# ashiq24/UNO

Hardware: AMD Instinct MI355X
Metric: UNO training samples/s (421^2 Darcy) (higher is better)
Workload: dtype f32; 1 GPU; Darcy 2D 421x421, UNO_9(3,64,pad=5) 64ch, batch 16/GPU, train step (fwd+loss+bwd+allreduce+Adam); global_batch=16, parallelism=dp1

## Files before the change

### include/uno_spectral.h

```cpp
#ifndef UNO_SPECTRAL_H
#define UNO_SPECTRAL_H

#ifdef __cplusplus
extern "C" {
#endif

#define UNO_SPECTRAL_ABI_VERSION 14

int uno_abi_version(void);
void* uno_upload_table(const void* host, long long bytes);

const char* uno_last_error(void);

long long uno_spectral_conv2d_fwd_ws_bytes(int B, int Ci, int Co, int m1, int m2);
long long uno_spectral_conv2d_bwd_ws_bytes(int B, int Ci, int Co, int m1, int m2);

int uno_spectral_conv2d_forward(const float* x, const float* w1, const float* w2, float* y,
                                float* xtrunc, void* ws, int B, int Ci, int Co, int H, int W,
                                int Ho, int Wo, int m1, int m2, void* stream);

int uno_spectral_conv2d_backward(const float* gy, const float* xtrunc, const float* w1,
                                 const float* w2, float* gx, float* gw1, float* gw2, void* ws,
                                 int B, int Ci, int Co, int H, int W, int Ho, int Wo, int m1,
                                 int m2, void* stream);

int uno_spectral_conv2d_forward_bf16(const void* x, const float* w1, const float* w2, void* y,
                                     float* xtrunc, void* ws, int B, int Ci, int Co, int H, int W,
                                     int Ho, int Wo, int m1, int m2, void* stream);
int uno_spectral_conv2d_backward_bf16(const void* gy, const float* xtrunc, const float* w1,
                                      const float* w2, void* gx, float* gw1, float* gw2, void* ws,
                                      int B, int Ci, int Co, int H, int W, int Ho, int Wo, int m1,
                                      int m2, void* stream);

long long uno_fft_resample3d_ws_bytes(int n_vol, int D1, int M1, int J1, int J2, int m3);
int uno_fft_resample3d(const float* x, float* y, void* ws, int n_vol, int D1, int D2, int D3, int M1, int M2, int M3,
                       int J1, const int* f1_in, const int* f1_out, int J2, const int* f2_in, const int* f2_out, int m3,
                       float scale, int herm_in, int herm_out, void* stream);

int uno_fft_resample3d_acc(const float* x, float* y, float* y_act, void* ws, int n_vol, int D1, int D2, int D3, int M1, int M2, int M3,
                           int J1, const int* f1_in, const int* f1_out, int J2, const int* f2_in, const int* f2_out, int m3,
                           float scale, int herm_in, int herm_out, void* stream);

long long uno_fft_resample3d_any_ws_bytes(int n_vol, int D1, int M1, int J1, int J2, int m3);
int uno_fft_resample3d_any(const float* x, float* y, void* ws, int n_vol, int D1, int D2, int D3, int M1, int M2, int M3,
                           int J1, const int* f1_in, const int* f1_out, int J2, const int* f2_in, const int* f2_out, int m3,
                           float scale, int herm_in, int herm_out, void* stream);

int uno_fft_resample3d_any_acc(const float* x, float* y, float* y_act, void* ws, int n_vol, int D1, int D2, int D3, int M1, int M2, int M3,
                               int J1, const int* f1_in, const int* f1_out, int J2, const int* f2_in, const int* f2_out, int m3,
                               float scale, int herm_in, int herm_out, void* stream);

long long uno_spectral_conv3d_fwd_ws_bytes(int B, int Ci, int Co, int H, int Ho, int m1, int m2, int m3);
long long uno_spectral_conv3d_bwd_ws_bytes(int B, int Ci, int Co, int H, int Ho, int m1, int m2, int m3);
int uno_spectral_conv3d_forward(const float* x, const float* const* w, float* y, float* xtrunc, void* ws,
                                int B, int Ci, int Co, int H, int W, int T, int Ho, int Wo, int To,
                                int m1, int m2, int m3, void* stream);
int uno_spectral_conv3d_backward(const float* gy, const float* xtrunc, const float* const* w, float* gx,
                                 float* const* gw, void* ws, int B, int Ci, int Co, int H, int W, int T,
                                 int Ho, int Wo, int To, int m1, int m2, int m3, void* stream);

int uno_cdft_axis(const float* in, float* out, int inverse, int n_img, int H, int m1, int m2, int m3,
                  float scale, int mask_overlap, void* stream);


int uno_dft2d_forward(const float* images, float* spec, int n_img, int H, int W, int m1, int m2,
                      float scale, int hermitian_cols, int mask_overlap, void* stream);

int uno_dft2d_inverse(const float* spec, float* images, int n_img, int H, int W, int m1, int m2,
                      float scale, int hermitian_cols, int mask_overlap, void* stream);

int uno_reserve_cus(int n);

int uno_sweep_alternation(int enable);

int uno_dft2d_inverse_add_applies(int n_img, int H, int W, int m1, int m2, int Hs, int Ws);
int uno_dft2d_inverse_add(const float* spec, float* images, int n_img, int H, int W, int m1, int m2, float scale, int hermitian_cols,
                          int mask_overlap, const float* addend, int Hs, int Ws, const int* tile_p0, const float* row_op,
                          const int* col_v0, const float* col_op, void* stream);

int uno_dft2d_forward_bf16(const void* images, float* spec, int n_img, int H, int W, int m1, int m2,
                           float scale, int hermitian_cols, int mask_overlap, void* stream);
int uno_dft2d_inverse_bf16(const float* spec, void* images, int n_img, int H, int W, int m1, int m2,
                           float scale, int hermitian_cols, int mask_overlap, void* stream);

int uno_dft2d_forward_grouped(const float* images, float* spec, int n_img, int H, int W, int m1, int m2, float scale,
                              int hermitian_cols, int mask_overlap, int group, int stride, int offset, void* stream);
int uno_dft2d_inverse_grouped(const float* spec, float* images, int n_img, int H, int W, int m1, int m2, float scale,
                              int hermitian_cols, int mask_overlap, int group, int stride, int offset, void* stream);

int uno_mode_mix(const float* in, const float* const* w, float* out, int op, int B, int Ci, int Co,
                 int ncorner, int modes_per_corner, void* stream);

int uno_mode_wgrad(const float* xtrunc, const float* go, float* const* gw, int B, int Ci, int Co,
                   int ncorner, int modes_per_corner, void* stream);
int uno_mode_backward(const float* xtrunc, const float* go, const float* const* w, float* gx_spec, float* const* gw, int B, int Ci,
                      int Co, int ncorner, int modes_per_corner, int accumulate, void* stream);
int uno_mode_wgrad_acc(const float* xtrunc, const float* go, float* const* gw, int B, int Ci, int Co, int ncorner,
                       int modes_per_corner, int accumulate, void* stream);
int uno_spectral_conv2d_backward_acc(const void* gy, const float* xtrunc, const void* w1, const void* w2, void* gx,
                                     float* gw1, float* gw2, void* ws, int B, int Ci, int Co, int H, int W, int Ho, int Wo,
                                     int m1, int m2, int io_format, int accumulate_gw, void* stream);

int uno_resample2d(const float* in, float* out, float* tmp, int n_img, int H, int W, int Ho, int Wo,
                   const int* startH, const float* wtH, int KH, const int* startW, const float* wtW, int KW,
                   const int* tile_p0, const float* tile_w, int NP, int accumulate, void* stream);

int uno_channel_mix(const float* x, const float* w, const float* bias, float* y, int B, int Ci, int Co,
                    long long P, int transpose_w, int accumulate, int act_in, const float* dgelu_of, void* stream);

long long uno_channel_wgrad_ws_bytes(int B, int Ci, int Co, long long P);
int uno_channel_wgrad(const float* gy, const float* x, float* gw, float* gb, void* ws, int B, int Ci, int Co,
                      long long P, int act_x, void* stream);

int uno_channel_mix2(const float* x1, const float* x2, int C1, const float* w, const float* bias, float* y1, float* y2, int Co1,
                     float* y_act, int B, int Ci, int Co, long long P, int transpose_w, int accumulate, int act_in,
                     const float* dgelu_of, const float* proj_w, const float* proj_b, float* proj_out, void* stream);
int uno_channel_wgrad2(const float* gy, const float* x1, const float* x2, int C1, float* gw, float* gb, void* ws, int B, int Ci,
                       int Co, long long P, int act_x, int accumulate, void* stream);
int uno_channel_wgrad_finish(const void* parts, float* gw, float* gb, int Ci, int Co, long long nparts, int accumulate, void* stream);

int uno_gelu_project_forward(const float* pre, const float* w, const float* bias, float* out, int B, int C, long long P,
                             void* stream);
long long uno_gelu_project_bwd_ws_bytes(int B, int C, long long P);
int uno_gelu_project_backward(const float* pre, const float* w, const float* gout, float* gpre, float* gw, float* gb,
                              void* ws, int B, int C, long long P, void* stream);

int uno_gelu_project2_forward(const float* pre, const float* s, const float* w, const float* bias, float* out, int B, int C1, int C2,
                              long long P, int act2, void* stream);
long long uno_gelu_project2_bwd_ws_bytes(int B, int C1, int C2, long long P);
int uno_gelu_project2_backward(const float* pre, const float* s, const float* w, const float* gout, float* gpre, float* gs, float* gw,
                               float* gb, void* ws, int B, int C1, int C2, long long P, int act2, void* stream);

long long uno_rel_l2_steps_ws_bytes(int B, long long P, int T);
int uno_rel_l2_steps(const float* pred, const float* target, float* sums, float* rel, float* totals, void* ws, int B, long long P, int T,
                     void* stream);

long long uno_rollout_ws_bytes(int B, long long P, int T);
int uno_rollout_advance(float* window, const float* frame, const float* target, float* pred, void* ws, int B, int C, int T_in, long long P,
                        int T, int t, int shift, void* stream);
int uno_rollout_finish(const void* ws, float* sums, float* rel, float* totals, int B, long long P, int T, void* stream);

int uno_rollout_lift(const float* given, const float* pred, const float* feat, const float* w, const float* bias, float* h, int B, int T_in,
                     int F, int Cm, long long P, int T, int t, void* stream);
long long uno_rollout_lift_bwd_ws_bytes(int B, int T_in, int F, int Cm, long long P, int T);
int uno_rollout_lift_backward(const float* gh, const float* given, const float* pred, const float* target, const float* feat, const float* w,
                              const float* sums, const float* gL, float* gpred, float* gframe, void* parts, int B, int T_in, int F, int Cm,
                              long long P, int T, int t, void* stream);
int uno_rollout_loss_seed(const float* pred, const float* target, const float* sums, const float* gL, float* gframe, int B, long long P, int T,
                          void* stream);

int uno_channel_mix2_win(const float* x1, const float* x2, int C1, const float* w, const float* bias, float* y1, float* y2, int Co1,
                         float* y_act, int B, int Ci, int Co, int rows, int cols, int pitch, long long plane, int transpose_w,
                         int accumulate, int act_in, const float* dgelu_of, const float* proj_w, const float* proj_b, float* proj_out,
                         void* stream);
int uno_channel_wgrad2_win(const float* gy, const float* x1, const float* x2, int C1, float* gw, float* gb, void* ws, int B, int Ci,
                           int Co, int rows, int cols, int pitch, long long plane, int act_x, int accumulate, void* stream);
int uno_gelu_project_backward_win(const float* pre, const float* w, const float* gout, float* gpre, float* gw, float* gb, void* ws,
                                  int B, int C, int rows, int cols, int pitch, long long plane, void* stream);
int uno_project_backward_applies(int B, int C1, int Ci, int Co, int rows, int cols, int pitch, long long plane);
long long uno_project_backward_ws_bytes(int B, int Ci, int Co, long long P);
int uno_project_backward(const float* x1, const float* x2, int C1, const float* w, const float* pre, const float* w2, const float* gout,
                         float* g1, float* g2, float* gw, float* gb, float* gw2, float* gb2, void* ws, int B, int Ci, int Co, int rows,
                         int cols, int pitch, long long plane, int act_in, int accumulate_w, void* stream);
int uno_clear_border(float* t, long long n_planes, int Hp, int Wp, int rows, int cols, void* stream);
int uno_channel_mix_act_padded(const float* x, const float* w, const float* bias, float* y, float* y_act, int B, int Ci, int Co, int H,
                               int W, int Hp, int Wp, int act_in, void* stream);
int uno_channel_mix_dgelu_padded(const float* x, const float* w, const float* bias, const float* g_padded, float* gz, int B, int Ci,
                                 int Co, int H, int W, int Hp, int Wp, int act_in, void* stream);
int uno_lift_forward(const float* x, const float* w1, const float* b1, const float* w0, const float* b0, float* act, int B, int Cin,
                     int Cm, int Co, int H, int W, int Hp, int Wp, void* stream);
long long uno_lift_bwd_ws_bytes(int B, int Cin, int Cm, int Co, int H, int W);
int uno_lift_backward(const float* x, const float* w1, const float* b1, const float* w0, const float* b0, const float* g_act, float* gw1,
                      float* gb1, float* gw0, float* gb0, void* ws, int B, int Cin, int Cm, int Co, int H, int W, int Hp, int Wp,
                      void* stream);
int uno_lift_backward_takes_second(int B, int Cin, int Cm, int Co, int H, int W, int Hp, int Wp);
int uno_lift_backward2(const float* x, const float* w1, const float* b1, const float* w0, const float* b0, const float* g_act,
                       const float* g_act2, float* gw1, float* gb1, float* gw0, float* gb0, void* ws, int B, int Cin, int Cm, int Co,
                       int H, int W, int Hp, int Wp, void* stream);

int uno_gelu_pad(const float* s, const float* gy, float* out, int n_img, int H, int W, int Hp, int Wp, int backward,
                 void* stream);

int uno_instnorm_forward(const float* x, const float* gamma, const float* beta, float* y, float* mean, float* rstd, long long rows,
                         int C, long long N, float eps, int gelu, void* stream);
int uno_instnorm_backward(const float* x, const float* gy, const float* gamma, const float* beta, const float* mean,
                          const float* rstd, float* gx, float* s1, float* s2, long long rows, int C, long long N, int gelu,
                          void* stream);

int uno_adam_step(float* p, const float* g, float* m, float* v, long long n, int is_complex, double lr, double beta1,
                  double beta2, double eps, double weight_decay, int step, void* stream);

int uno_adam_step_multi(int n_tensors, float* const* p, const float* const* g, float* const* m, float* const* v,
                        const long long* n, const int* is_complex, double lr, double beta1, double beta2, double eps,
                        double weight_decay, int step, void* stream);

int uno_adam_step_multi_dev(int n_tensors, float* const* p, const float* const* g, float* const* m, float* const* v,
                            const long long* n, const int* is_complex, double lr, double beta1, double beta2, double eps,
                            double weight_decay, int* step_counter, float* scalars, const double* hyper, void* stream);

int uno_spectral_conv2d_forward_mixed(const void* x_bf16, const void* w1_f16, const void* w2_f16, void* y_bf16,
                                      float* xtrunc, void* ws, int B, int Ci, int Co, int H, int W, int Ho, int Wo,
                                      int modes1, int modes2, void* stream);
int uno_spectral_conv2d_backward_mixed(const void* gy_bf16, const float* xtrunc, const void* w1_f16, const void* w2_f16,
                                       void* gx_bf16, float* gw1, float* gw2, void* ws, int B, int Ci, int Co, int H, int W,
                                       int Ho, int Wo, int modes1, int modes2, void* stream);
int uno_mode_mix_f16w(const float* in, const void* const* w_f16, float* out, int op, int B, int Ci, int Co, int ncorner,
                      int modes_per_corner, void* stream);
int uno_dft2d_forward_grouped_bf16(const void* images, float* spec, int n_img, int H, int W, int m1, int m2, float scale,
                                   int hermitian_cols, int mask_overlap, int group, int stride, int offset, void* stream);
int uno_dft2d_inverse_grouped_bf16(const float* spec, void* images, int n_img, int H, int W, int m1, int m2, float scale,
                                   int hermitian_cols, int mask_overlap, int group, int stride, int offset, void* stream);
int uno_resample2d_bf16(const void* in, void* out, float* tmp, int n_img, int H, int W, int Ho, int Wo, const int* startH,
                        const float* wtH, int KH, const int* startW, const float* wtW, int KW, const int* tile_p0,
                        const float* tile_w, int NP, int accumulate, void* stream);
int uno_channel_mix_bf16(const void* x, const float* w, const float* bias, void* y, int B, int Ci, int Co, long long P,
                         int transpose_w, int accumulate, int act_in, const void* dgelu_of, void* stream);
int uno_channel_wgrad_bf16(const void* gy, const void* x, float* gw, float* gb, void* ws, int B, int Ci, int Co, long long P,
                           int act_x, void* stream);
int uno_channel_mix2_bf16(const void* x1, const void* x2, int C1, const float* w, const float* bias, void* y1, void* y2, int Co1,
                          void* y_act, int B, int Ci, int Co, long long P, int transpose_w, int accumulate, int act_in,
                          const void* dgelu_of, const float* proj_w, const float* proj_b, void* proj_out, void* stream);
int uno_channel_wgrad2_bf16(const void* gy, const void* x1, const void* x2, int C1, float* gw, float* gb, void* ws, int B, int Ci,
                            int Co, long long P, int act_x, int accumulate, void* stream);
int uno_gelu_project_forward_bf16(const void* pre, const float* w, const float* bias, void* out, int B, int C, long long P,
                                  void* stream);
int uno_gelu_project_backward_bf16(const void* pre, const float* w, const void* gout, void* gpre, float* gw, float* gb,
                                   void* ws, int B, int C, long long P, void* stream);
int uno_gelu_pad_bf16(const void* s, const void* gy, void* out, int n_img, int H, int W, int Hp, int Wp, int backward,
                      void* stream);
int uno_instnorm_forward_bf16(const void* x, const float* gamma, const float* beta, void* y, float* mean, float* rstd,
                              long long rows, int C, long long N, float eps, int gelu, void* stream);
int uno_instnorm_backward_bf16(const void* x, const void* gy, const float* gamma, const float* beta, const float* mean,
                               const float* rstd, void* gx, float* s1, float* s2, long long rows, int C, long long N,
                               int gelu, void* stream);

long long uno_dft2d_any_ws_bytes(int n_img, int H, int W, int m1, int m2);
int uno_scratch_provide(void* ptr, long long bytes);
long long uno_channel_mix_ws_bytes(int Ci, int Co, long long P, int bf16);

int uno_transpose_batched(const float* in, float* out, int B, long long R, int C, long long ld_in, long long sb_in,
                          long long ld_out, long long sb_out, void* stream);

int uno_profile_begin(int max_records);
int uno_profile_end(void);
int uno_profile_get(int index, char* name, int name_len, double* ms, double* bytes);

#ifdef __cplusplus
}
#endif
#endif
```

### uno_amd/_native.py

```python
from __future__ import annotations

import ctypes as C
import os
import threading

import torch

_HERE = os.path.dirname(os.path.abspath(__file__))
LIB_PATH = os.path.join(_HERE, "lib", "libuno_spectral.so")
ABI_VERSION = 14

_lib = None
_lock = threading.Lock()

_fp = C.c_void_p
_i = C.c_int
_SIGNATURES = {
    "uno_abi_version": (C.c_int, []),
    "uno_last_error": (C.c_char_p, []),
    "uno_dft2d_any_ws_bytes": (C.c_longlong, [_i] * 5),
    "uno_scratch_provide": (C.c_int, [_fp, C.c_longlong]),
    "uno_spectral_conv2d_fwd_ws_bytes": (C.c_longlong, [_i] * 5),
    "uno_spectral_conv2d_bwd_ws_bytes": (C.c_longlong, [_i] * 5),
    "uno_spectral_conv2d_forward": (C.c_int, [_fp] * 6 + [_i] * 9 + [_fp]),
    "uno_spectral_conv2d_backward": (C.c_int, [_fp] * 8 + [_i] * 9 + [_fp]),
    "uno_spectral_conv2d_forward_bf16": (C.c_int, [_fp] * 6 + [_i] * 9 + [_fp]),
    "uno_spectral_conv2d_backward_bf16": (C.c_int, [_fp] * 8 + [_i] * 9 + [_fp]),
    "uno_fft_resample3d_ws_bytes": (C.c_longlong, [_i] * 6),
    "uno_fft_resample3d": (C.c_int, [_fp] * 3 + [_i] * 8 + [_fp, _fp, _i, _fp, _fp, _i, C.c_float, _i, _i, _fp]),
    "uno_fft_resample3d_acc": (C.c_int, [_fp] * 4 + [_i] * 8 + [_fp, _fp, _i, _fp, _fp, _i, C.c_float, _i, _i, _fp]),
    "uno_fft_resample3d_any_ws_bytes": (C.c_longlong, [_i] * 6),
    "uno_fft_resample3d_any": (C.c_int, [_fp] * 3 + [_i] * 8 + [_fp, _fp, _i, _fp, _fp, _i, C.c_float, _i, _i, _fp]),
    "uno_fft_resample3d_any_acc": (C.c_int, [_fp] * 4 + [_i] * 8 + [_fp, _fp, _i, _fp, _fp, _i, C.c_float, _i, _i, _fp]),
    "uno_dft2d_forward": (C.c_int, [_fp, _fp] + [_i] * 5 + [C.c_float, _i, _i, _fp]),
    "uno_dft2d_forward_bf16": (C.c_int, [_fp, _fp] + [_i] * 5 + [C.c_float, _i, _i, _fp]),
    "uno_dft2d_inverse_bf16": (C.c_int, [_fp, _fp] + [_i] * 5 + [C.c_float, _i, _i, _fp]),
    "uno_dft2d_inverse": (C.c_int, [_fp, _fp] + [_i] * 5 + [C.c_float, _i, _i, _fp]),
    "uno_reserve_cus": (C.c_int, [_i]),
    "uno_sweep_alternation": (C.c_int, [_i]),
    "uno_dft2d_inverse_add_applies": (C.c_int, [_i] * 7),
    "uno_dft2d_inverse_add": (C.c_int, [_fp, _fp] + [_i] * 5 + [C.c_float, _i, _i, _fp, _i, _i, _fp, _fp, _fp, _fp, _fp]),
    "uno_dft2d_forward_grouped": (C.c_int, [_fp, _fp] + [_i] * 5 + [C.c_float] + [_i] * 5 + [_fp]),
    "uno_dft2d_inverse_grouped": (C.c_int, [_fp, _fp] + [_i] * 5 + [C.c_float] + [_i] * 5 + [_fp]),
    "uno_mode_mix": (C.c_int, [_fp, C.POINTER(_fp), _fp] + [_i] * 6 + [_fp]),
    "uno_mode_wgrad": (C.c_int, [_fp, _fp, C.POINTER(_fp)] + [_i] * 5 + [_fp]),
    "uno_mode_backward": (C.c_int, [_fp, _fp, C.POINTER(_fp), _fp, C.POINTER(_fp)] + [_i] * 6 + [_fp]),
    "uno_spectral_conv3d_fwd_ws_bytes": (C.c_longlong, [_i] * 8),
    "uno_spectral_conv3d_bwd_ws_bytes": (C.c_longlong, [_i] * 8),
    "uno_spectral_conv3d_forward": (C.c_int, [_fp, C.POINTER(_fp), _fp, _fp, _fp] + [_i] * 12 + [_fp]),
    "uno_spectral_conv3d_backward": (C.c_int, [_fp, _fp, C.POINTER(_fp), _fp, C.POINTER(_fp), _fp] + [_i] * 12 + [_fp]),
    "uno_cdft_axis": (C.c_int, [_fp, _fp] + [_i] * 6 + [C.c_float, _i, _fp]),
    "uno_resample2d": (C.c_int, [_fp, _fp, _fp] + [_i] * 5 + [_fp, _fp, _i, _fp, _fp, _i, _fp, _fp, _i, _i, _fp]),
    "uno_channel_mix": (C.c_int, [_fp, _fp, _fp, _fp, _i, _i, _i, C.c_longlong, _i, _i, _i, _fp, _fp]),
    "uno_channel_wgrad_ws_bytes": (C.c_longlong, [_i, _i, _i, C.c_longlong]),
    "uno_channel_wgrad": (C.c_int, [_fp, _fp, _fp, _fp, _fp, _i, _i, _i, C.c_longlong, _i, _fp]),
    "uno_channel_mix2": (C.c_int, [_fp, _fp, _i, _fp, _fp, _fp, _fp, _i, _fp, _i, _i, _i, C.c_longlong, _i, _i, _i, _fp, _fp, _fp, _fp, _fp]),
    "uno_channel_wgrad2": (C.c_int, [_fp, _fp, _fp, _i, _fp, _fp, _fp, _i, _i, _i, C.c_longlong, _i, _i, _fp]),
    "uno_channel_mix2_win": (C.c_int, [_fp, _fp, _i, _fp, _fp, _fp, _fp, _i, _fp, _i, _i, _i, _i, _i, _i, C.c_longlong, _i, _i, _i, _fp, _fp, _fp, _fp, _fp]),
    "uno_channel_mix_ws_bytes": (C.c_longlong, [_i, _i, C.c_longlong, _i]),
    "uno_clear_border": (C.c_int, [_fp, C.c_longlong, _i, _i, _i, _i, _fp]),
    "uno_channel_mix_act_padded": (C.c_int, [_fp, _fp, _fp, _fp, _fp, _i, _i, _i, _i, _i, _i, _i, _i, _fp]),
    "uno_lift_forward": (C.c_int, [_fp] * 6 + [_i] * 8 + [_fp]),
    "uno_lift_bwd_ws_bytes": (C.c_longlong, [_i] * 6),
    "uno_lift_backward": (C.c_int, [_fp] * 11 + [_i] * 8 + [_fp]),
    "uno_lift_backward2": (C.c_int, [_fp] * 12 + [_i] * 8 + [_fp]),
    "uno_lift_backward_takes_second": (C.c_int, [_i] * 8),
    "uno_channel_mix_dgelu_padded": (C.c_int, [_fp, _fp, _fp, _fp, _fp, _i, _i, _i, _i, _i, _i, _i, _i, _fp]),
    "uno_channel_wgrad2_win": (C.c_int, [_fp, _fp, _fp, _i, _fp, _fp, _fp, _i, _i, _i, _i, _i, _i, C.c_longlong, _i, _i, _fp]),
    "uno_gelu_project_backward_win": (C.c_int, [_fp] * 7 + [_i, _i, _i, _i, _i, C.c_longlong, _fp]),
    "uno_channel_wgrad_finish": (C.c_int, [_fp, _fp, _fp, _i, _i, C.c_longlong, _i, _fp]),
    "uno_mode_wgrad_acc": (C.c_int, [_fp, _fp, C.POINTER(_fp)] + [_i] * 6 + [_fp]),
    "uno_spectral_conv2d_backward_acc": (C.c_int, [_fp] * 8 + [_i] * 11 + [_fp]),
    "uno_upload_table": (C.c_void_p, [_fp, C.c_longlong]),
    "uno_project_backward_applies": (C.c_int, [_i] * 7 + [C.c_longlong]),
    "uno_project_backward_ws_bytes": (C.c_longlong, [_i, _i, _i, C.c_longlong]),
    "uno_project_backward": (C.c_int, [_fp, _fp, _i] + [_fp] * 11 + [_i] * 6 + [C.c_longlong, _i, _i, _fp]),
    "uno_gelu_project_forward": (C.c_int, [_fp, _fp, _fp, _fp, _i, _i, C.c_longlong, _fp]),
    "uno_gelu_project_bwd_ws_bytes": (C.c_longlong, [_i, _i, C.c_longlong]),
    "uno_gelu_project_backward": (C.c_int, [_fp] * 7 + [_i, _i, C.c_longlong, _fp]),
    "uno_gelu_project2_forward": (C.c_int, [_fp] * 5 + [_i, _i, _i, C.c_longlong, _i, _fp]),
    "uno_gelu_project2_bwd_ws_bytes": (C.c_longlong, [_i, _i, _i, C.c_longlong]),
    "uno_gelu_project2_backward": (C.c_int, [_fp] * 9 + [_i, _i, _i, C.c_longlong, _i, _fp]),
    "uno_rel_l2_steps_ws_bytes": (C.c_longlong, [_i, C.c_longlong, _i]),
    "uno_rel_l2_steps": (C.c_int, [_fp] * 6 + [_i, C.c_longlong, _i, _fp]),
    "uno_rollout_ws_bytes": (C.c_longlong, [_i, C.c_longlong, _i]),
    "uno_rollout_advance": (C.c_int, [_fp] * 5 + [_i, _i, _i, C.c_longlong, _i, _i, _i, _fp]),
    "uno_rollout_finish": (C.c_int, [_fp] * 4 + [_i, C.c_longlong, _i, _fp]),
    "uno_rollout_lift": (C.c_int, [_fp] * 6 + [_i, _i, _i, _i, C.c_longlong, _i, _i, _fp]),
    "uno_rollout_lift_bwd_ws_bytes": (C.c_longlong, [_i, _i, _i, _i, C.c_longlong, _i]),
    "uno_rollout_lift_backward": (C.c_int, [_fp] * 11 + [_i, _i, _i, _i, C.c_longlong, _i, _i, _fp]),
    "uno_rollout_loss_seed": (C.c_int, [_fp] * 5 + [_i, C.c_longlong, _i, _fp]),
    "uno_gelu_pad": (C.c_int, [_fp, _fp, _fp] + [_i] * 6 + [_fp]),
    "uno_transpose_batched": (C.c_int, [_fp, _fp, _i, C.c_longlong, _i] + [C.c_longlong] * 4 + [_fp]),
    "uno_instnorm_forward": (C.c_int, [_fp] * 6 + [C.c_longlong, _i, C.c_longlong, C.c_float, _i, _fp]),
    "uno_instnorm_backward": (C.c_int, [_fp] * 9 + [C.c_longlong, _i, C.c_longlong, _i, _fp]),
    "uno_adam_step": (C.c_int, [_fp, _fp, _fp, _fp, C.c_longlong, _i] + [C.c_double] * 5 + [_i, _fp]),
    "uno_adam_step_multi": (C.c_int, [_i, C.POINTER(_fp), C.POINTER(_fp), C.POINTER(_fp), C.POINTER(_fp), C.POINTER(C.c_longlong),
                                      C.POINTER(_i)] + [C.c_double] * 5 + [_i, _fp]),
    "uno_adam_step_multi_dev": (C.c_int, [_i, C.POINTER(_fp), C.POINTER(_fp), C.POINTER(_fp), C.POINTER(_fp), C.POINTER(C.c_longlong),
                                          C.POINTER(_i)] + [C.c_double] * 5 + [_fp, _fp, _fp, _fp]),
    "uno_spectral_conv2d_forward_mixed": (C.c_int, [_fp] * 6 + [_i] * 9 + [_fp]),
    "uno_spectral_conv2d_backward_mixed": (C.c_int, [_fp] * 8 + [_i] * 9 + [_fp]),
    "uno_mode_mix_f16w": (C.c_int, [_fp, C.POINTER(_fp), _fp] + [_i] * 6 + [_fp]),
    "uno_dft2d_forward_grouped_bf16": (C.c_int, [_fp, _fp] + [_i] * 5 + [C.c_float] + [_i] * 5 + [_fp]),
    "uno_dft2d_inverse_grouped_bf16": (C.c_int, [_fp, _fp] + [_i] * 5 + [C.c_float] + [_i] * 5 + [_fp]),
    "uno_resample2d_bf16": (C.c_int, [_fp, _fp, _fp] + [_i] * 5 + [_fp, _fp, _i, _fp, _fp, _i, _fp, _fp, _i, _i, _fp]),
    "uno_channel_mix_bf16": (C.c_int, [_fp, _fp, _fp, _fp, _i, _i, _i, C.c_longlong, _i, _i, _i, _fp, _fp]),
    "uno_channel_wgrad_bf16": (C.c_int, [_fp, _fp, _fp, _fp, _fp, _i, _i, _i, C.c_longlong, _i, _fp]),
    "uno_channel_mix2_bf16": (C.c_int, [_fp, _fp, _i, _fp, _fp, _fp, _fp, _i, _fp, _i, _i, _i, C.c_longlong, _i, _i, _i, _fp, _fp, _fp, _fp, _fp]),
    "uno_channel_wgrad2_bf16": (C.c_int, [_fp, _fp, _fp, _i, _fp, _fp, _fp, _i, _i, _i, C.c_longlong, _i, _i, _fp]),
    "uno_gelu_project_forward_bf16": (C.c_int, [_fp, _fp, _fp, _fp, _i, _i, C.c_longlong, _fp]),
    "uno_gelu_project_backward_bf16": (C.c_int, [_fp] * 7 + [_i, _i, C.c_longlong, _fp]),
    "uno_gelu_pad_bf16": (C.c_int, [_fp, _fp, _fp] + [_i] * 6 + [_fp]),
    "uno_instnorm_forward_bf16": (C.c_int, [_fp] * 6 + [C.c_longlong, _i, C.c_longlong, C.c_float, _i, _fp]),
    "uno_instnorm_backward_bf16": (C.c_int, [_fp] * 9 + [C.c_longlong, _i, C.c_longlong, _i, _fp]),
    "uno_profile_begin": (C.c_int, [_i]),
    "uno_profile_end": (C.c_int, []),
    "uno_profile_get": (C.c_int, [_i, C.c_char_p, _i, C.POINTER(C.c_double), C.POINTER(C.c_double)]),
}
EXPORTED_SYMBOLS = tuple(_SIGNATURES)


def lib():
    global _lib
    if _lib is None:
        with _lock:
            if _lib is None:
                if not os.path.exists(LIB_PATH):
                    raise RuntimeError(
                        f"uno_amd: native library {LIB_PATH} is missing - build it with "
                        "`python -m uno_amd.build` (hipcc, gfx950); there is no CPU fallback")
                h = C.CDLL(LIB_PATH)
                for name, (res, args) in _SIGNATURES.items():
                    fn = getattr(h, name)
                    fn.restype = res
                    fn.argtypes = args
                if h.uno_abi_version() != ABI_VERSION:
                    raise RuntimeError(f"uno_amd: ABI mismatch, library {h.uno_abi_version()} != binding {ABI_VERSION}")
                _lib = h
    return _lib


def _check(rc: int, what: str):
    if rc != 0:
        msg = lib().uno_last_error().decode(errors="replace")
        raise RuntimeError(f"{what} failed (code {rc}): {msg}")


def _ptr(t: torch.Tensor):
    return C.c_void_p(t.data_ptr())


def _opt(t):
    return _ptr(t) if t is not None else C.c_void_p(0)


def _count(lead) -> int:
    n = 1
    for d in lead:
        n *= d
    return n


def _stream(t: torch.Tensor):
    return C.c_void_p(torch.cuda.current_stream(t.device).cuda_stream)


class _scratch:

    def __init__(self, device, nbytes):
        self.bytes, self.device, self.buf = nbytes, device, None

    def __enter__(self):
        if self.bytes > 0:
            self.buf = torch.empty(self.bytes, dtype=torch.uint8, device=self.device)
            _check(lib().uno_scratch_provide(_ptr(self.buf), self.bytes), "uno_scratch_provide")
        return self

    def __exit__(self, *exc):
        if self.bytes > 0:
            lib().uno_scratch_provide(None, 0)
        return False


class _any_mode_scratch(_scratch):

    def __init__(self, device, *needs):
        L = lib()
        _scratch.__init__(self, device, max((int(L.uno_dft2d_any_ws_bytes(*[int(v) for v in n])) for n in needs), default=0))


class _mix_scratch(_scratch):

    def __init__(self, device, Ci, Co, P, bf16):
        _scratch.__init__(self, device, int(lib().uno_channel_mix_ws_bytes(int(Ci), int(Co), int(P), 1 if bf16 else 0)))


def _require(t: torch.Tensor, dtype, name: str, dense: bool = True):
    if not t.is_cuda:
        raise RuntimeError(f"uno_amd: {name} must live on a HIP device (got {t.device})"
                           + ("; the spectral convolution runs only on the MI355X kernels" if dense else ""))
    if t.dtype != dtype:
        raise RuntimeError(f"uno_amd: {name} must be {dtype} (got {t.dtype})")
    if dense and not t.is_contiguous():
        raise RuntimeError(f"uno_amd: {name} must be contiguous")


def _entry(name: str, bf16: bool):
    return getattr(lib(), name + "_bf16" if bf16 else name)


def _act_dtype(t, name):
    bf16 = t.dtype == torch.bfloat16
    _require(t, torch.bfloat16 if bf16 else torch.float32, name)
    return bf16


def _weights_half(w1, w2, bf16):
    if w1.dtype == torch.float16:
        if not bf16:
            raise RuntimeError("uno_amd: half-precision weight storage goes with bfloat16 activations")
        for w, name in ((w1, "weights1"), (w2, "weights2")):
            _require(w, torch.float16, name)
            if w.dim() != 5 or w.shape[-1] != 2:
                raise RuntimeError("uno_amd: half-precision weights are stored as (Ci, Co, m1, m2, 2) = (re, im)")
        return True
    _require(w1, torch.complex64, "weights1")
    _require(w2, torch.complex64, "weights2")
    return False


def _complex_grad_buffers(out, shape, n: int, device, accumulate: bool):
    if out is None:
        return [torch.empty(shape, dtype=torch.complex64, device=device) for _ in range(n)], False
    gws = list(out)
    for t in gws:
        _require(t, torch.complex64, "weight-gradient buffer")
        if tuple(t.shape) != tuple(shape):
            raise RuntimeError("uno_amd: weight-gradient buffer has the wrong shape")
    return gws, accumulate


def _real_grad_buffers(out_w, out_b, Ci: int, Co: int, need_bias: bool, device, accumulate: bool):
    if out_w is None:
        gw = torch.empty((Co, Ci), dtype=torch.float32, device=device)
        return gw, (torch.empty((Co,), dtype=torch.float32, device=device) if need_bias else None), False
    gw, gb = out_w, (out_b if need_bias else None)
    _require(gw, torch.float32, "weight-gradient buffer")
    if gw.numel() != Co * Ci or (need_bias and (gb is None or gb.numel() != Co)):
        raise RuntimeError("uno_amd: gradient buffers do not match the layer")
    if gb is not None:
        _require(gb, torch.float32, "bias-gradient buffer")
    return gw, gb, accumulate


def spectral_conv2d_forward(x, w1, w2, Ho: int, Wo: int, xt_out=None):
    bf16 = _act_dtype(x, "x")
    wh = _weights_half(w1, w2, bf16)
    B, Ci, H, W = x.shape
    Ci2, Co, m1, m2 = w1.shape[:4]
    if Ci2 != Ci or tuple(w2.shape) != tuple(w1.shape):
        raise RuntimeError(f"uno_amd: weight shapes {tuple(w1.shape)} / {tuple(w2.shape)} do not match input channels {Ci}")
    L = lib()
    with torch.cuda.device(x.device):
        y = torch.empty((B, Co, Ho, Wo), dtype=x.dtype, device=x.device)
        if xt_out is None:
            xt = torch.empty((B, Ci, 2 * m1, m2), dtype=torch.complex64, device=x.device)
        else:
            xt = xt_out
            _require(xt, torch.complex64, "xtrunc buffer")
            if tuple(xt.shape) != (B, Ci, 2 * m1, m2):
                raise RuntimeError("uno_amd: xtrunc buffer has the wrong shape")
        ws = torch.empty(max(1, L.uno_spectral_conv2d_fwd_ws_bytes(B, Ci, Co, m1, m2)), dtype=torch.uint8, device=x.device)
        fn = L.uno_spectral_conv2d_forward_mixed if wh else _entry("uno_spectral_conv2d_forward", bf16)
        with _any_mode_scratch(x.device, (B * Ci, H, W, m1, m2), (B * Co, Ho, Wo, m1, m2)):
            rc = fn(_ptr(x), _ptr(w1), _ptr(w2), _ptr(y), _ptr(xt), _ptr(ws), B, Ci, Co, H, W, Ho, Wo, m1, m2, _stream(x))
    _check(rc, "uno_spectral_conv2d_forward")
    return y, xt


def spectral_conv2d_backward(gy, xt, w1, w2, H: int, W: int, need_gx=True, need_gw=True, gw_out=None, accumulate_gw=False):
    bf16 = _act_dtype(gy, "grad_output")
    _require(xt, torch.complex64, "xtrunc")
    wh = _weights_half(w1, w2, bf16)
    B, Co, Ho, Wo = gy.shape
    Ci, Co2, m1, m2 = w1.shape[:4]
    if Co2 != Co:
        raise RuntimeError("uno_amd: grad_output channels do not match the weights")
    L = lib()
    with torch.cuda.device(gy.device):
        gx = torch.empty((B, Ci, H, W), dtype=gy.dtype, device=gy.device) if need_gx else None
        gw1, gw2, accumulate_gw = None, None, accumulate_gw and need_gw
        if need_gw:
            (gw1, gw2), accumulate_gw = _complex_grad_buffers(gw_out, (Ci, Co, m1, m2), 2, gy.device, accumulate_gw)
        ws = torch.empty(max(1, L.uno_spectral_conv2d_bwd_ws_bytes(B, Ci, Co, m1, m2)), dtype=torch.uint8, device=gy.device)
        with _any_mode_scratch(gy.device, (B * Co, Ho, Wo, m1, m2), (B * Ci, H, W, m1, m2)):
            rc = L.uno_spectral_conv2d_backward_acc(_ptr(gy), _ptr(xt), _ptr(w1), _ptr(w2), _opt(gx), _opt(gw1), _opt(gw2),
                                                    _ptr(ws), B, Ci, Co, H, W, Ho, Wo, m1, m2, 2 if wh else (1 if bf16 else 0),
                                                    1 if accumulate_gw else 0, _stream(gy))
    _check(rc, "uno_spectral_conv2d_backward")
    return gx, gw1, gw2


def _fft_resample3d(any_grid: bool, x, out_size, f1, f2, m3, scale, adjoint, out, act):
    name = "uno_fft_resample3d_any" if any_grid else "uno_fft_resample3d"
    _require(x, torch.float32, "x")
    *lead, D1, D2, D3 = x.shape
    M1, M2, M3 = (int(v) for v in out_size)
    n = _count(lead)
    for t in (*f1, *f2):
        if t.dtype != torch.int32 or not t.is_cuda or not t.is_contiguous():
            raise RuntimeError("uno_amd: frequency tables must be contiguous int32 device tensors")
    J1, J2 = f1[0].numel(), f2[0].numel()
    if any_grid and (f1[1].numel() != J1 or f2[1].numel() != J2):
        raise RuntimeError("uno_amd: the forward and inverse frequency tables of an axis must have the same length")
    L = lib()
    with torch.cuda.device(x.device):
        ws = torch.empty(max(1, getattr(L, name + "_ws_bytes")(n, D1, M1, J1, J2, int(m3))), dtype=torch.uint8, device=x.device)
        if out is not None:
            _require(out, torch.float32, "out")
            if tuple(out.shape) != (*lead, M1, M2, M3) or not out.is_contiguous():
                raise RuntimeError(f"uno_amd: out must be a contiguous {(*lead, M1, M2, M3)} tensor")
            ya = torch.empty_like(out) if act else None
            fn, dst, res = getattr(L, name + "_acc"), (_ptr(out), _opt(ya)), ((out, ya) if act else out)
        else:
            res = torch.empty((*lead, M1, M2, M3), dtype=torch.float32, device=x.device)
            fn, dst = getattr(L, name), (_ptr(res),)
        rc = fn(_ptr(x), *dst, _ptr(ws), n, D1, D2, D3, M1, M2, M3, J1, _ptr(f1[0]), _ptr(f1[1]), J2, _ptr(f2[0]), _ptr(f2[1]),
                int(m3), float(scale), int(adjoint), int(not adjoint), _stream(x))
    _check(rc, name + ("_acc" if out is not None else ""))
    return res


def fft_resample3d(x, out_size, f1, f2, m3: int, scale: float, adjoint: bool, out=None, act=False):
    return _fft_resample3d(False, x, out_size, f1, f2, m3, scale, adjoint, out, act)


def fft_resample3d_any(x, out_size, f1, f2, m3: int, scale: float, adjoint: bool, out=None, act=False):
    return _fft_resample3d(True, x, out_size, f1, f2, m3, scale, adjoint, out, act)


def dft2d_forward(images, m1, m2, scale=1.0, hermitian_cols=False, mask_overlap=False, out=None, channel_offset=0):
    bf16 = _act_dtype(images, "images")
    *lead, H, W = images.shape
    n = _count(lead)
    if out is None:
        spec = torch.empty((*lead, 2 * m1, m2), dtype=torch.complex64, device=images.device)
        with torch.cuda.device(images.device):
            fn = _entry("uno_dft2d_forward", bf16)
            with _any_mode_scratch(images.device, (n, H, W, m1, m2)):
                rc = fn(_ptr(images), _ptr(spec), n, H, W, m1, m2, float(scale), int(hermitian_cols), int(mask_overlap), _stream(images))
        _check(rc, "uno_dft2d_forward")
        return spec
    _require(out, torch.complex64, "out")
    if images.dim() != 4 or out.dim() != 4 or out.shape[0] != images.shape[0] or tuple(out.shape[2:]) != (2 * m1, m2) \
            or channel_offset < 0 or channel_offset + images.shape[1] > out.shape[1]:
        raise RuntimeError("uno_amd: out must be (B, Ctot, 2*m1, m2) with room for the image channels at channel_offset")
    with torch.cuda.device(images.device):
        fn = _entry("uno_dft2d_forward_grouped", bf16)
        with _any_mode_scratch(images.device, (n, H, W, m1, m2)):
            rc = fn(_ptr(images), _ptr(out), n, H, W, m1, m2, float(scale), int(hermitian_cols),
                    int(mask_overlap), images.shape[1], out.shape[1], int(channel_offset), _stream(images))
    _check(rc, "uno_dft2d_forward_grouped")
    return out


def reserve_cus(n: int) -> int:
    return int(lib().uno_reserve_cus(int(n)))


def sweep_alternation(enable: bool) -> bool:
    return bool(lib().uno_sweep_alternation(1 if enable else 0))


def sweep_direction(mode: str, mask: int = 255) -> int:
    if mode not in ("alternate", "forward", "reversed") or not 0 <= int(mask) <= 255:
        raise ValueError(f"uno_amd: sweep_direction({mode!r}, {mask!r}): mode is alternate | forward | reversed, mask 0 .. 255")
    value = {"alternate": int(mask), "forward": 0, "reversed": 256 | int(mask)}[mode]
    if value == 1:
        raise ValueError("uno_amd: sweep_direction('alternate', 1): the C entry point reads 1 as 'every family' (255)")
    return int(lib().uno_sweep_alternation(value))


def dft2d_inverse_add_applies(n_img, H, W, m1, m2, Hs, Ws) -> bool:
    return bool(lib().uno_dft2d_inverse_add_applies(int(n_img), int(H), int(W), int(m1), int(m2), int(Hs), int(Ws)))


def dft2d_inverse(spec, H, W, scale=1.0, hermitian_cols=True, mask_overlap=True, channels=None, channel_offset=0,
                  dtype=torch.float32, addend=None):
    _require(spec, torch.complex64, "spec")
    *lead, r2, m2 = spec.shape
    m1 = r2 // 2
    if addend is not None:
        t, (p0, rowop, v0, colop) = addend
        _require(t, torch.float32, "addend")
        if channels is not None or dtype != torch.float32 or tuple(t.shape[:-2]) != tuple(lead):
            raise RuntimeError("uno_amd: dft2d_inverse(addend=) takes the plain float32 form with one addend image per spectrum")
        n = _count(lead)
        img = torch.empty((*lead, H, W), dtype=torch.float32, device=spec.device)
        with torch.cuda.device(spec.device):
            rc = lib().uno_dft2d_inverse_add(_ptr(spec), _ptr(img), n, H, W, m1, m2, float(scale), int(hermitian_cols), int(mask_overlap),
                                             _ptr(t), t.shape[-2], t.shape[-1], _ptr(p0), _ptr(rowop), _ptr(v0), _ptr(colop), _stream(spec))
        _check(rc, "uno_dft2d_inverse_add")
        return img
    if channels is None:
        n = _count(lead)
        if dtype not in (torch.float32, torch.bfloat16):
            raise RuntimeError("uno_amd: images are float32 or bfloat16")
        img = torch.empty((*lead, H, W), dtype=dtype, device=spec.device)
        with torch.cuda.device(spec.device):
            fn = _entry("uno_dft2d_inverse", dtype == torch.bfloat16)
            with _any_mode_scratch(spec.device, (n, H, W, m1, m2)):
                rc = fn(_ptr(spec), _ptr(img), n, H, W, m1, m2, float(scale), int(hermitian_cols), int(mask_overlap), _stream(spec))
        _check(rc, "uno_dft2d_inverse")
        return img
    if dtype not in (torch.float32, torch.bfloat16):
        raise RuntimeError("uno_amd: images are float32 or bfloat16")
    if spec.dim() != 4 or channel_offset < 0 or channels < 1 or channel_offset + channels > spec.shape[1]:
        raise RuntimeError("uno_amd: spec must be (B, Ctot, 2*m1, m2) holding the requested channel range")
    B = spec.shape[0]
    img = torch.empty((B, channels, H, W), dtype=dtype, device=spec.device)
    with torch.cuda.device(spec.device):
        fn = _entry("uno_dft2d_inverse_grouped", dtype == torch.bfloat16)
        with _any_mode_scratch(spec.device, (B * channels, H, W, m1, m2)):
            rc = fn(_ptr(spec), _ptr(img), B * channels, H, W, m1, m2, float(scale), int(hermitian_cols),
                    int(mask_overlap), int(channels), spec.shape[1], int(channel_offset), _stream(spec))
    _check(rc, "uno_dft2d_inverse_grouped")
    return img


def _ptr_array(ts):
    return (C.c_void_p * len(ts))(*[t.data_ptr() for t in ts])


def mode_mix(inp, weights, op: int):
    _require(inp, torch.complex64, "spectrum")
    half = weights[0].dtype == torch.float16
    for w in weights:
        _require(w, torch.float16 if half else torch.complex64, "weights")
    B = inp.shape[0]
    Ci, Co = weights[0].shape[:2]
    nc = len(weights)
    Mc = weights[0][0, 0].numel() // (2 if half else 1)
    cout = Co if op == 0 else Ci
    out = torch.empty((B, cout, *inp.shape[2:]), dtype=torch.complex64, device=inp.device)
    with torch.cuda.device(inp.device):
        fn = lib().uno_mode_mix_f16w if half else lib().uno_mode_mix
        rc = fn(_ptr(inp), _ptr_array(weights), _ptr(out), op, B, Ci, Co, nc, Mc, _stream(inp))
    _check(rc, "uno_mode_mix")
    return out


def mode_wgrad(xt, go, weight_shape, ncorner: int, out=None, accumulate: bool = False):
    _require(xt, torch.complex64, "xtrunc")
    _require(go, torch.complex64, "grad spectrum")
    B, Ci = xt.shape[:2]
    Co = go.shape[1]
    gws, accumulate = _complex_grad_buffers(out, weight_shape, ncorner, xt.device, accumulate)
    Mc = gws[0][0, 0].numel()
    with torch.cuda.device(xt.device):
        rc = lib().uno_mode_wgrad_acc(_ptr(xt), _ptr(go), _ptr_array(gws), B, Ci, Co, ncorner, Mc, 1 if accumulate else 0, _stream(xt))
    _check(rc, "uno_mode_wgrad")
    return gws


def mode_backward(xt, go, weights, out=None, accumulate: bool = False):
    _require(xt, torch.complex64, "xtrunc")
    _require(go, torch.complex64, "grad spectrum")
    for w in weights:
        _require(w, torch.complex64, "weights")
    B, Ci = xt.shape[:2]
    Co = go.shape[1]
    nc = len(weights)
    Mc = weights[0][0, 0].numel()
    gws, accumulate = _complex_grad_buffers(out, weights[0].shape, nc, xt.device, accumulate)
    gX = torch.empty((B, Ci, nc * Mc), dtype=torch.complex64, device=xt.device)
    with torch.cuda.device(xt.device):
        rc = lib().uno_mode_backward(_ptr(xt), _ptr(go), _ptr_array(list(weights)), _ptr(gX), _ptr_array(gws), B, Ci, Co, nc, Mc,
                                     1 if accumulate else 0, _stream(xt))
    _check(rc, "uno_mode_backward")
    return gX, gws


def spectral_conv3d_forward(x, ws_, Ho: int, Wo: int, To: int):
    _require(x, torch.float32, "x")
    if len(ws_) != 4:
        raise RuntimeError("uno_amd: the 3-D spectral convolution takes four weight tensors")
    for w in ws_:
        _require(w, torch.complex64, "weights")
        if tuple(w.shape) != tuple(ws_[0].shape):
            raise RuntimeError("uno_amd: weights1..4 must have one shape")
    B, Ci, H, W, T = x.shape
    Ci2, Co, m1, m2, m3 = ws_[0].shape
    if Ci2 != Ci:
        raise RuntimeError(f"uno_amd: weight shape {tuple(ws_[0].shape)} does not match input channels {Ci}")
    L = lib()
    with torch.cuda.device(x.device):
        y = torch.empty((B, Co, Ho, Wo, To), dtype=torch.float32, device=x.device)
        xt = torch.empty((B, Ci, 4, m1, m2, m3), dtype=torch.complex64, device=x.device)
        scratch = torch.empty(max(1, L.uno_spectral_conv3d_fwd_ws_bytes(B, Ci, Co, H, Ho, m1, m2, m3)), dtype=torch.uint8,
                              device=x.device)
        with _any_mode_scratch(x.device, (B * Ci * H, W, T, m2, m3), (B * Co * Ho, Wo, To, m2, m3)):
            rc = L.uno_spectral_conv3d_forward(_ptr(x), _ptr_array(ws_), _ptr(y), _ptr(xt), _ptr(scratch), B, Ci, Co,
                                               H, W, T, Ho, Wo, To, m1, m2, m3, _stream(x))
    _check(rc, "uno_spectral_conv3d_forward")
    return y, xt


def spectral_conv3d_backward(gy, xt, ws_, H: int, W: int, T: int, need_gx=True, need_gw=True):
    _require(gy, torch.float32, "grad_output")
    _require(xt, torch.complex64, "xtrunc")
    for w in ws_:
        _require(w, torch.complex64, "weights")
    B, Co, Ho, Wo, To = gy.shape
    Ci, Co2, m1, m2, m3 = ws_[0].shape
    if Co2 != Co:
        raise RuntimeError("uno_amd: grad_output channels do not match the weights")
    L = lib()
    with torch.cuda.device(gy.device):
        gx = torch.empty((B, Ci, H, W, T), dtype=torch.float32, device=gy.device) if need_gx else None
        gws = [torch.empty_like(w) for w in ws_] if need_gw else None
        scratch = torch.empty(max(1, L.uno_spectral_conv3d_bwd_ws_bytes(B, Ci, Co, H, Ho, m1, m2, m3)), dtype=torch.uint8,
                              device=gy.device)
        with _any_mode_scratch(gy.device, (B * Co * Ho, Wo, To, m2, m3), (B * Ci * H, W, T, m2, m3)):
            rc = L.uno_spectral_conv3d_backward(_ptr(gy), _ptr(xt), _ptr_array(ws_), _opt(gx),
                                                _ptr_array(gws) if need_gw else None, _ptr(scratch), B, Ci, Co,
                                                H, W, T, Ho, Wo, To, m1, m2, m3, _stream(gy))
    _check(rc, "uno_spectral_conv3d_backward")
    return gx, gws


def resample2d(x, Ho: int, Wo: int, tabH, tabW, tilesH=None, out=None):
    bf16 = _act_dtype(x, "x")
    *lead, H, W = x.shape
    n = _count(lead)
    sH, wH = tabH
    sW, wW = tabW
    accumulate = out is not None
    if accumulate:
        _require(out, x.dtype, "out")
        if tuple(out.shape) != (*lead, Ho, Wo):
            raise RuntimeError(f"uno_amd: out has shape {tuple(out.shape)}, expected {(*lead, Ho, Wo)}")
    else:
        out = torch.empty((*lead, Ho, Wo), dtype=x.dtype, device=x.device)
    with torch.cuda.device(x.device):
        tmp = torch.empty(max(1, n * min(Ho * W, H * Wo)), dtype=torch.float32, device=x.device)
        if tilesH is not None:
            tp0, tw = tilesH
            targs = (_ptr(tp0), _ptr(tw), tw.shape[1])
        else:
            targs = (C.c_void_p(0), C.c_void_p(0), 0)
        fn = _entry("uno_resample2d", bf16)
        rc = fn(_ptr(x), _ptr(out), _ptr(tmp), n, H, W, Ho, Wo, _ptr(sH), _ptr(wH), wH.shape[1],
                _ptr(sW), _ptr(wW), wW.shape[1], *targs, 1 if accumulate else 0, _stream(x))
    _check(rc, "uno_resample2d")
    return out


def _window_fits(rows: int, cols: int, pitch: int, plane: int) -> bool:
    return not (rows < 1 or cols % 4 or cols < 260 or pitch < cols or (rows - 1) * pitch + cols > plane or rows * cols >= 1 << 24)


def _window_args(window, plane: int, bf16: bool):
    rows, cols, pitch = (int(v) for v in window)
    if bf16:
        raise RuntimeError("uno_amd: pixel windows are float32 only")
    if not _window_fits(rows, cols, pitch, plane):
        raise RuntimeError(f"uno_amd: window rows={rows} cols={cols} pitch={pitch} does not fit a plane of {plane} elements "
                           "(cols: a multiple of 4, 260 <= cols <= pitch; rows * cols < 2^24)")
    return rows, cols, pitch


def channel_mix(x, w, bias=None, transpose_w: bool = False, out=None, act_in: bool = False, dgelu_of=None, dgelu_total: bool = False,
                window=None):
    if window is not None:
        return channel_mix2(x, None, w, bias, transpose_w=transpose_w, out=out, act_in=act_in, dgelu_of=dgelu_of,
                            accumulate=(2 if (dgelu_total and dgelu_of is not None) else 1) if out is not None else 0, window=window)
    bf16 = _act_dtype(x, "x")
    _require(w, torch.float32, "weight")
    if bias is not None:
        _require(bias, torch.float32, "bias")
    B, Ci, P = x.shape
    Co = w.shape[1] if transpose_w else w.shape[0]
    if (w.shape[0] if transpose_w else w.shape[1]) != Ci:
        raise RuntimeError(f"uno_amd: weight {tuple(w.shape)} does not match {Ci} input channels")
    accumulate = out is not None
    if accumulate:
        _require(out, x.dtype, "out")
        if tuple(out.shape) != (B, Co, P):
            raise RuntimeError(f"uno_amd: out has shape {tuple(out.shape)}, expected {(B, Co, P)}")
        y = out
    else:
        y = torch.empty((B, Co, P), dtype=x.dtype, device=x.device)
    with torch.cuda.device(x.device), _mix_scratch(x.device, Ci, Co, P, bf16):
        if dgelu_of is not None:
            _require(dgelu_of, x.dtype, "dgelu_of")
            if tuple(dgelu_of.shape) != (B, Co, P):
                raise RuntimeError(f"uno_amd: dgelu_of has shape {tuple(dgelu_of.shape)}, expected {(B, Co, P)}")
        rc = _entry("uno_channel_mix", bf16)(_ptr(x), _ptr(w), _opt(bias), _ptr(y), B, Ci, Co, P, 1 if transpose_w else 0,
                                             (2 if (dgelu_total and dgelu_of is not None) else 1) if accumulate else 0,
                                             1 if act_in else 0, _opt(dgelu_of), _stream(x))
    _check(rc, "uno_channel_mix")
    return y


def clear_border(t, rows: int, cols: int):
    _require(t, torch.float32, "tensor")
    Hp, Wp = t.shape[-2:]
    n = t.numel() // max(1, Hp * Wp)
    with torch.cuda.device(t.device):
        rc = lib().uno_clear_border(_ptr(t), n, Hp, Wp, int(rows), int(cols), _stream(t))
    _check(rc, "uno_clear_border")
    return t


def channel_mix_act_padded_ok(x, Hp: int, Wp: int) -> bool:
    H, W = x.shape[-2:]
    return x.dtype == torch.float32 and 260 <= W <= Wp and H <= Hp and H * W < (1 << 24)


def channel_mix_act_padded(x, w, bias, Hp: int, Wp: int, act_in: bool = False, keep_y: bool = True):
    _require(x, torch.float32, "x")
    _require(w, torch.float32, "weight")
    if bias is not None:
        _require(bias, torch.float32, "bias")
    B, Ci, H, W = x.shape
    Co = w.shape[0]
    if w.shape[1] != Ci:
        raise RuntimeError(f"uno_amd: weight {tuple(w.shape)} does not match {Ci} input channels")
    y = torch.empty((B, Co, H, W), dtype=x.dtype, device=x.device) if keep_y else None
    act = torch.empty((B, Co, Hp, Wp), dtype=x.dtype, device=x.device)
    with torch.cuda.device(x.device):
        rc = lib().uno_channel_mix_act_padded(_ptr(x), _ptr(w), _opt(bias), _opt(y), _ptr(act),
                                              B, Ci, Co, H, W, int(Hp), int(Wp), 1 if act_in else 0, _stream(x))
    _check(rc, "uno_channel_mix_act_padded")
    return y, act


def lift_ok(x, w1, w0, Hp: int, Wp: int) -> bool:
    if x.dim() != 4 or x.dtype != torch.float32:
        return False
    H, W = x.shape[-2:]
    return (1 <= x.shape[1] <= 3 and w1.shape[0] in (16, 32) and w1.shape[1] == x.shape[1] and w0.shape[1] == w1.shape[0]
            and 260 <= W <= Wp and H <= Hp and H * W < (1 << 24))


def lift_forward(x, w1, b1, w0, b0, Hp: int, Wp: int):
    for t, n in ((x, "x"), (w1, "weight 1"), (w0, "weight 0")) + tuple((t, "bias") for t in (b1, b0) if t is not None):
        _require(t, torch.float32, n)
    B, Cin, H, W = x.shape
    Cm, Co = w1.shape[0], w0.shape[0]
    act = torch.empty((B, Co, Hp, Wp), dtype=x.dtype, device=x.device)
    with torch.cuda.device(x.device):
        rc = lib().uno_lift_forward(_ptr(x), _ptr(w1), _opt(b1), _ptr(w0), _opt(b0),
                                    _ptr(act), B, Cin, Cm, Co, H, W, int(Hp), int(Wp), _stream(x))
    _check(rc, "uno_lift_forward")
    return act


def lift_backward_takes_second(x, w1, w0, Hp: int, Wp: int) -> bool:
    B, Cin, H, W = x.shape
    return bool(lib().uno_lift_backward_takes_second(B, Cin, w1.shape[0], w0.shape[0], H, W, int(Hp), int(Wp)))


def lift_backward(x, w1, b1, w0, b0, g_act, g_act2=None):
    _require(g_act, torch.float32, "grad_output")
    B, Cin, H, W = x.shape
    Cm, Co = w1.shape[0], w0.shape[0]
    Hp, Wp = g_act.shape[-2:]
    if tuple(g_act.shape[:2]) != (B, Co):
        raise RuntimeError("uno_amd: grad_output does not match the lift")
    if g_act2 is not None:
        _require(g_act2, torch.float32, "second grad_output")
        if tuple(g_act2.shape) != tuple(g_act.shape):
            raise RuntimeError("uno_amd: the two gradients of the lift's output disagree in shape")
    dev = x.device
    gw1 = torch.empty((Cm, Cin), dtype=torch.float32, device=dev)
    gw0 = torch.empty((Co, Cm), dtype=torch.float32, device=dev)
    gb1 = torch.empty((Cm,), dtype=torch.float32, device=dev) if b1 is not None else None
    gb0 = torch.empty((Co,), dtype=torch.float32, device=dev) if b0 is not None else None
    with torch.cuda.device(dev):
        ws = torch.empty(max(1, lib().uno_lift_bwd_ws_bytes(B, Cin, Cm, Co, H, W)), dtype=torch.uint8, device=dev)
        rc = lib().uno_lift_backward2(_ptr(x), _ptr(w1), _opt(b1), _ptr(w0), _opt(b0),
                                     _ptr(g_act), _opt(g_act2), _ptr(gw1), _opt(gb1), _ptr(gw0),
                                     _opt(gb0), _ptr(ws), B, Cin, Cm, Co, H, W, int(Hp), int(Wp), _stream(x))
    _check(rc, "uno_lift_backward")
    return gw1, gb1, gw0, gb0


def channel_mix_dgelu_padded(x, w, bias, g_padded, act_in: bool = False):
# ... 641 lines not shown
```

### uno_amd/block2d.py

```python
import torch
import torch.nn.functional as F
from torch.autograd.function import once_differentiable

from . import _native
from ._param_grads import _grad_targets, _note_use, _stack_arrived, _stack_grad_slot, _stack_take, _stack_wanted
from .pointwise import _mix2_forward, _mix2_input_grads, _plain, _wgrad_into
from .resample import resample_adjoint, resample_forward, upsample_add_tables


def _half_weights(w1, w2):
    out = []
    capturing = w1.is_cuda and torch.cuda.is_current_stream_capturing()
    with torch.no_grad():
        for w in (w1, w2):
            cached = None if capturing else getattr(w, "_uno_half", None)
            if cached is None or cached[0] != w._version or cached[1].device != w.device or cached[2] != w.data_ptr():
                cached = (w._version, torch.view_as_real(w.detach()).half().contiguous(), w.data_ptr())
                if not capturing:
                    try:
                        w._uno_half = cached
                    except (AttributeError, RuntimeError):
                        pass
            out.append(cached[1])
    return out[0], out[1]


def _xt_slot(stack):
    return None if stack is None else stack.xt


def _xt_dest(stack, B, Ci, m1, m2, device):
    slot = _xt_slot(stack)
    return torch.empty((B, Ci, 2 * m1, m2), dtype=torch.complex64, device=device) if slot is None else slot


def _block_prologue(ctx, iw, x, Ci, w1, w2, cw, cb, Ho, Wo, half_weights):
    B, _, H, W = x.shape
    ctx.stack = _stack_take(w1, (B, Ci, 2 * w1.shape[2], w1.shape[3]), x.device, _stack_wanted(ctx, iw, x, half_weights))
    w1, w2 = _plain(w1), _plain(w2)
    if half_weights:
        w1, w2 = _half_weights(w1, w2)
    cwm = _plain(cw).reshape(cw.shape[0], Ci)
    cb = None if cb is None else _plain(cb)
    same = (H, W) == (Ho, Wo)
    return w1, w2, cwm, cb, same, same or Ho * Wo < H * W


def _pointwise_input_grads(g_src, w, C1, gx1, gx2, geom, dgelu_of=None, dgelu_total=False, g_act=None):
    H, W, Ho, Wo, same, mix_last = geom
    B = g_src.shape[0]
    direct = same or not mix_last

    def dest(gx):
        return gx.view(B, gx.shape[1], -1) if direct else None

    g1, g2 = g_act, None
    if gx1 is not None and gx2 is not None:
        g1, g2 = _mix2_input_grads(g_src, w, C1, out1=dest(gx1), out2=dest(gx2))
    else:
        if gx1 is not None and g1 is None:
            g1 = _native.channel_mix(g_src, w if C1 == w.shape[1] else w[:, :C1].contiguous(), None, transpose_w=True, out=dest(gx1),
                                     dgelu_of=dgelu_of, dgelu_total=dgelu_total)
        if gx2 is not None:
            g2 = _native.channel_mix(g_src, w[:, C1:].contiguous(), None, transpose_w=True, out=dest(gx2))
    if not direct:
        for g, gx in ((g1, gx1), (g2, gx2)):
            if gx is not None:
                resample_adjoint(g.view(B, gx.shape[1], Ho, Wo), H, W, out=gx)


class _SpectralConv2dFn(torch.autograd.Function):

    @staticmethod
    def forward(ctx, x, w1, w2, Ho, Wo, half_weights=False):
        ctx.params = (w1, w2)
        x = _plain(x)
        ctx.stack = _stack_take(w1, (x.shape[0], x.shape[1], 2 * w1.shape[2], w1.shape[3]), x.device, _stack_wanted(ctx, 1, x, half_weights))
        w1, w2 = _plain(w1), _plain(w2)
        if half_weights:
            w1, w2 = _half_weights(w1, w2)
        y, xt = _native.spectral_conv2d_forward(x, w1, w2, int(Ho), int(Wo), xt_out=_xt_slot(ctx.stack))
        ctx.save_for_backward(xt, w1, w2)
        ctx.in_hw = (x.shape[-2], x.shape[-1])
        return y

    @staticmethod
    @once_differentiable
    def backward(ctx, gy):
        xt, w1, w2 = ctx.saved_tensors
        gx, gw1, gw2, _ = _spectral_backward(_plain(gy), xt, w1, w2, ctx.in_hw[0], ctx.in_hw[1], ctx.needs_input_grad[0],
                                          ctx.needs_input_grad[1] or ctx.needs_input_grad[2],
                                          ctx.needs_input_grad[1] and ctx.needs_input_grad[2], ctx.params, ctx.stack)
        return gx, gw1, gw2, None, None, None


FUSE_UPSAMPLE_ADD = True


def _fused_addend(t, H, W, m1, m2, adjoint):
    if not FUSE_UPSAMPLE_ADD or t.dtype != torch.float32 or t.dim() != 4 or not t.is_cuda:
        return None
    Hs, Ws = t.shape[-2], t.shape[-1]
    if Hs * Ws >= H * W or not _native.dft2d_inverse_add_applies(t.shape[0] * t.shape[1], H, W, m1, m2, Hs, Ws):
        return None
    tabs = upsample_add_tables(Hs, Ws, H, W, str(t.device), bool(adjoint))
    return None if tabs is None else (t, tabs)


def _stage_wgrad(stack, gslot, xt, gO, w1, w2, leaves, both_gw, need_gx):
    if gslot is not None:
        return (None, *_stack_arrived(stack, leaves, w1.shape, both_gw))
    tg = _grad_targets(leaves) if both_gw else None
    _note_use(leaves[0])
    out, acc = (tg.dest, tg.accumulate) if tg else (None, False)
    gX = None
    if need_gx and w1.dtype == torch.complex64:
        gX, (gw1, gw2) = _native.mode_backward(xt, gO, [w1, w2], out=out, accumulate=acc)
        gX = gX.view(xt.shape)
    else:
        gw1, gw2 = _native.mode_wgrad(xt, gO, tuple(w1.shape[:4]), 2, out=out, accumulate=acc)
    if tg:
        gw1, gw2 = tg.returned
    return gX, gw1, gw2


def _spectral_backward(gs, xt, w1, w2, H, W, need_gx, need_gw, both_gw, leaves, stack, join=None, addend=None):
    B, Co = gs.shape[:2]
    Ci, _, m1, m2 = w1.shape[:4]
    gslot = _stack_grad_slot(stack, Co) if (stack is not None and need_gw) else None
    merging = join is not None and need_gx and bool(join.spectra)
    if addend is not None and not need_gx:
        raise RuntimeError("uno_amd: an addend for the input gradient needs the input gradient")
    if gslot is None and not merging and addend is None and not (need_gx and need_gw and w1.dtype == torch.complex64):
        tg = _grad_targets(leaves) if (need_gw and both_gw) else None
        if need_gw:
            _note_use(leaves[0])
        gx, gw1, gw2 = _native.spectral_conv2d_backward(gs, xt, w1, w2, H, W, need_gx=need_gx, need_gw=need_gw,
                                                        gw_out=tg.dest if tg else None, accumulate_gw=bool(tg and tg.accumulate))
        if tg:
            gw1, gw2 = tg.returned
        return gx, gw1, gw2, False
    gO = _native.dft2d_forward(gs, m1, m2, 1.0, True, True, out=gslot)
    gX, gw1, gw2 = _stage_wgrad(stack, gslot, xt, gO, w1, w2, leaves, both_gw, need_gx) if need_gw else (None, None, None)
    gx = None
    if need_gx:
        if gX is None:
            gX = _native.mode_mix(gO.view(B, Co, 2, m1 * m2), [w1, w2], 1).view(B, Ci, 2 * m1, m2)
        if merging:
            gX = join.merge(gX, (H, W))
        gx = _native.dft2d_inverse(gX, H, W, 1.0 / (H * W), False, False, dtype=gs.dtype, addend=addend)
    return gx, gw1, gw2, gslot is not None


class _OperatorBlock2dFn(torch.autograd.Function):

    @staticmethod
    def forward(ctx, x, w1, w2, cw, cb, Ho, Wo, half_weights=False, fuse_gelu=False, join=None, out_join=None):
        ctx.leaves = (w1, w2, cw, cb)
        ctx.join = None
        if join is not None:
            join.reset()
            if ctx.needs_input_grad[0]:
                join.owner = True
                ctx.join = join
        x = _plain(x)
        B, Ci, H, W = x.shape
        Co = cw.shape[0]
        w1, w2, cwm, cb, same, mix_last = _block_prologue(ctx, 1, x, Ci, w1, w2, cw, cb, Ho, Wo, half_weights)
        t = fused = None
        if not mix_last and not half_weights and x.dtype == torch.float32:
            t = _native.channel_mix(x.view(B, Ci, -1), cwm, cb).view(B, Co, H, W)
            fused = _fused_addend(t, Ho, Wo, w1.shape[2], w1.shape[3], False)
        if fused is not None:
            m1, m2 = w1.shape[2], w1.shape[3]
            xt = _xt_dest(ctx.stack, B, Ci, m1, m2, x.device)
            _native.dft2d_forward(x, m1, m2, 1.0 / (H * W), out=xt, channel_offset=0)
            O = _native.mode_mix(xt.view(B, Ci, 2, m1 * m2), [w1, w2], 0)
            s = _native.dft2d_inverse(O.view(B, Co, 2 * m1, m2), Ho, Wo, 1.0, True, True, addend=fused)
        else:
            pre_act = None
            if mix_last and not same:
                pre_act = resample_forward(x, Ho, Wo)
            s, xt = _native.spectral_conv2d_forward(x, w1, w2, Ho, Wo, xt_out=_xt_slot(ctx.stack))
        out = s
        if fused is not None:
            act = x
            if fuse_gelu:
                out = F.gelu(s)
        elif mix_last:
            act = x if same else pre_act
            if fuse_gelu:
                _, out = _native.channel_mix2(act.view(B, Ci, -1), None, cwm, cb, out=s.view(B, Co, -1), accumulate=True, y_act=True)
                out = out.view(B, Co, Ho, Wo)
            else:
                _native.channel_mix(act.view(B, Ci, -1), cwm, cb, out=s.view(B, Co, -1))
        else:
            act = x
            if t is None:
                t = _native.channel_mix(x.view(B, Ci, -1), cwm, cb).view(B, Co, H, W)
            resample_forward(t, Ho, Wo, out=s)
            if fuse_gelu:
                out = F.gelu(s)
        ctx.save_for_backward(xt, w1, w2, cwm, act, s if fuse_gelu else None)
        ctx.geom = (H, W, same, mix_last, cb is not None, tuple(cw.shape))
        ctx.out_join = None
        if fuse_gelu and out_join is not None:
            out_join.pre, out_join.dgelu_applied = s, False
            ctx.out_join = out_join
        return out

    @staticmethod
    @once_differentiable
    def backward(ctx, gs):
        xt, w1, w2, cwm, act, pre = ctx.saved_tensors
        H, W, same, mix_last, has_bias, cw_shape = ctx.geom
        gs = _plain(gs)
        if pre is not None:
            oj = ctx.out_join
            if oj is not None and oj.dgelu_applied and oj.pre is not None and oj.pre.data_ptr() == pre.data_ptr():
                oj.dgelu_applied = False
            else:
                gs = torch.ops.aten.gelu_backward(gs, pre)
            if oj is not None:
                oj.pre = None
        B, Co, Ho, Wo = gs.shape
        Ci = cwm.shape[1]
        need_gx = ctx.needs_input_grad[0]
        need_gw = ctx.needs_input_grad[1] or ctx.needs_input_grad[2]
        need_gc = ctx.needs_input_grad[3] or (has_bias and ctx.needs_input_grad[4])
        join = ctx.join
        lw1, lw2, lcw, lcb = ctx.leaves
        g_act = addend = g_t = None
        if not mix_last:
            g_t = resample_adjoint(gs, H, W).view(B, Co, -1)
        if mix_last and not same and need_gx and gs.dtype == torch.float32:
            g_act = _native.channel_mix(gs.view(B, Co, -1), cwm, None, transpose_w=True).view(B, Ci, Ho, Wo)
            addend = _fused_addend(g_act, H, W, w1.shape[2], w1.shape[3], True)
        gx, gw1, gw2, stacked = _spectral_backward(gs, xt, w1, w2, H, W, need_gx, need_gw, ctx.needs_input_grad[1] and ctx.needs_input_grad[2],
                                                   (lw1, lw2), ctx.stack, join, addend)
        pstack = ctx.stack if stacked else None
        gcw = gcb = None
        xpre = join.pre if (join is not None and need_gx) else None
        own_last = xpre is not None and not join.pending
        dg_view = xpre.view(B, Ci, -1) if own_last else None
        direct = same or not mix_last
        g_src = gs.view(B, Co, -1) if mix_last else g_t
        if need_gx and (direct or addend is None):
            _pointwise_input_grads(g_src, cwm, Ci, gx, None, (H, W, Ho, Wo, same, mix_last), dgelu_of=dg_view if direct else None,
                                   dgelu_total=own_last and direct, g_act=g_act)
        dg_done = own_last and direct
        if need_gc:
            gcw, gcb = _wgrad_into((lcw, lcb), g_src, act.view(B, Ci, -1), None, ctx.needs_input_grad[3],
                                   has_bias and ctx.needs_input_grad[4], stack=pstack)
            gcw = None if gcw is None else gcw.view(cw_shape)
        if join is not None:
            if need_gx:
                dg_done = join.apply(gx, xpre if not dg_done else None) or dg_done
                if xpre is not None:
                    if not dg_done:
                        gx = torch.ops.aten.gelu_backward(gx, xpre)
                    join.dgelu_applied = True
            join.reset()
        return gx, gw1, gw2, gcw, gcb, None, None, None, None, None, None


class _OperatorBlock2dCatFn(torch.autograd.Function):

    @staticmethod
    def forward(ctx, x1, x2, w1, w2, cw, cb, Ho, Wo, half_weights=False, defer=None):
        ctx.leaves = (w1, w2, cw, cb)
        ctx.defer = defer if (defer is not None and defer.owner and ctx.needs_input_grad[1]) else None
        x1, x2 = _plain(x1), _plain(x2)
        B, C1, H, W = x1.shape
        C2 = x2.shape[1]
        Ci, Co, m1, m2 = w1.shape
        w1, w2, cwm, cb, same, mix_last = _block_prologue(ctx, 2, x1, Ci, w1, w2, cw, cb, Ho, Wo, half_weights)
        xt = _xt_dest(ctx.stack, B, Ci, m1, m2, x1.device)
        _native.dft2d_forward(x1, m1, m2, 1.0 / (H * W), out=xt, channel_offset=0)
        _native.dft2d_forward(x2, m1, m2, 1.0 / (H * W), out=xt, channel_offset=C1)
        O = _native.mode_mix(xt.view(B, Ci, 2, m1 * m2), [w1, w2], 0)
        t = fused = None
        if not mix_last and not half_weights and x1.dtype == torch.float32:
            t = _mix2_forward(x1.view(B, C1, -1), x2.view(B, C2, -1), cwm, cb).view(B, Co, H, W)
            fused = _fused_addend(t, Ho, Wo, m1, m2, False)
        s = _native.dft2d_inverse(O.view(B, Co, 2 * m1, m2), Ho, Wo, 1.0, True, True, dtype=x1.dtype, addend=fused)
        if fused is not None:
            a1, a2 = x1, x2
        elif mix_last:
            a1 = x1 if same else resample_forward(x1, Ho, Wo)
            a2 = x2 if same else resample_forward(x2, Ho, Wo)
            _mix2_forward(a1.view(B, C1, -1), a2.view(B, C2, -1), cwm, cb, out=s.view(B, Co, -1), accumulate=True)
        else:
            a1, a2 = x1, x2
            if t is None:
                t = _mix2_forward(x1.view(B, C1, -1), x2.view(B, C2, -1), cwm, cb).view(B, Co, H, W)
            resample_forward(t, Ho, Wo, out=s)
        ctx.save_for_backward(xt, w1, w2, cwm, a1, a2)
        ctx.geom = (H, W, same, mix_last, cb is not None, tuple(cw.shape))
        return s

    @staticmethod
    @once_differentiable
    def backward(ctx, gs):
        xt, w1, w2, cwm, a1, a2 = ctx.saved_tensors
        H, W, same, mix_last, has_bias, cw_shape = ctx.geom
        gs = _plain(gs)
        B, Co, Ho, Wo = gs.shape
        Ci, _, m1, m2 = w1.shape[:4]
        C1, C2 = a1.shape[1], a2.shape[1]
        need1, need2 = ctx.needs_input_grad[0], ctx.needs_input_grad[1]
        need_gw = ctx.needs_input_grad[2] or ctx.needs_input_grad[3]
        need_gc = ctx.needs_input_grad[4] or (has_bias and ctx.needs_input_grad[5])
        lw1, lw2, lcw, lcb = ctx.leaves
        both_gw = ctx.needs_input_grad[2] and ctx.needs_input_grad[3]
        gslot = _stack_grad_slot(ctx.stack, Co) if (ctx.stack is not None and need_gw) else None
        g_src = gs.view(B, Co, -1) if mix_last else resample_adjoint(gs, H, W).view(B, Co, -1)
        gO = _native.dft2d_forward(gs, m1, m2, 1.0, True, True, out=gslot)
        gXp, gw1, gw2 = _stage_wgrad(ctx.stack, gslot, xt, gO, w1, w2, (lw1, lw2), both_gw, need1 or need2) if need_gw else (None, None, None)
        gx1 = gx2 = None
        defer = ctx.defer if (need2 and ctx.defer is not None and ctx.defer.owner) else None
        if need1 or need2:
            gX = gXp if gXp is not None else _native.mode_mix(gO.view(B, Co, 2, m1 * m2), [w1, w2], 1).view(B, Ci, 2 * m1, m2)
            if need1:
                gx1 = _native.dft2d_inverse(gX, H, W, 1.0 / (H * W), False, False, channels=C1, channel_offset=0, dtype=gs.dtype)
            if defer is not None:
                defer.spectra.append((gX[:, C1:].contiguous(), (H, W)))
            elif need2:
                gx2 = _native.dft2d_inverse(gX, H, W, 1.0 / (H * W), False, False, channels=C2, channel_offset=C1, dtype=gs.dtype)
        gcw = gcb = None
        geom = (H, W, Ho, Wo, same, mix_last)
        if defer is not None:
            cw2 = cwm[:, C1:].contiguous()

            def x2_part(out, dg=None):
                _pointwise_input_grads(g_src, cw2, C2, out, None, geom, dgelu_of=None if dg is None else dg.view(B, C2, -1),
                                       dgelu_total=dg is not None)
            defer.pending.append((x2_part, same or not mix_last))
            _pointwise_input_grads(g_src, cwm, C1, gx1, None, geom)
        else:
            _pointwise_input_grads(g_src, cwm, C1, gx1, gx2, geom)
        if need_gc:
            gcw, gcb = _wgrad_into((lcw, lcb), g_src, a1.view(B, C1, -1), a2.view(B, C2, -1), ctx.needs_input_grad[4],
                                   has_bias and ctx.needs_input_grad[5])
            gcw = None if gcw is None else gcw.view(cw_shape)
        if ctx.defer is not None and gx2 is not None:
            gx2 = ctx.defer.late(gx2)
        return gx1, gx2, gw1, gw2, gcw, gcb, None, None, None, None


def spectral_conv2d(x, weights1, weights2, dim1, dim2):
    return _SpectralConv2dFn.apply(x, weights1, weights2, dim1, dim2)


def spectral_conv2d_mixed(x, weights1, weights2, dim1, dim2):
    if x.dtype != torch.bfloat16:
        raise RuntimeError(f"spectral_conv2d_mixed: input must be bfloat16 (got {x.dtype})")
    for w in (weights1, weights2):
        if w.dtype == torch.float16 and w.shape[-1] != 2:
            raise RuntimeError("spectral_conv2d_mixed: half-precision weights are stored as (..., 2) = (re, im)")
    if weights1.dtype == torch.float16:
        return _SpectralConv2dHalfFn.apply(x, weights1, weights2, dim1, dim2)
    return _SpectralConv2dFn.apply(x, weights1, weights2, dim1, dim2)


class _SpectralConv2dHalfFn(torch.autograd.Function):

    @staticmethod
    def forward(ctx, x, w1h, w2h, Ho, Wo):
        x, w1h, w2h = _plain(x), _plain(w1h), _plain(w2h)
        y, xt = _native.spectral_conv2d_forward(x, w1h, w2h, int(Ho), int(Wo))
        ctx.save_for_backward(xt, w1h, w2h)
        ctx.in_hw = (x.shape[-2], x.shape[-1])
        return y

    @staticmethod
    @once_differentiable
    def backward(ctx, gy):
        xt, w1h, w2h = ctx.saved_tensors
        need_gx = ctx.needs_input_grad[0]
        need_gw = ctx.needs_input_grad[1] or ctx.needs_input_grad[2]
        gx, gw1, gw2 = _native.spectral_conv2d_backward(_plain(gy), xt, w1h, w2h, ctx.in_hw[0], ctx.in_hw[1],
                                                        need_gx=need_gx, need_gw=need_gw)
        if need_gw:
            gw1, gw2 = torch.view_as_real(gw1).half(), torch.view_as_real(gw2).half()
        return gx, gw1, gw2, None, None
```

### uno_amd/build.py

```python
from __future__ import annotations

import argparse
import concurrent.futures as cf
import hashlib
import os
import shutil
import subprocess
import sys

HERE = os.path.dirname(os.path.abspath(__file__))
CSRC = os.path.join(HERE, "csrc")
LIBDIR = os.path.join(HERE, "lib")
LIB = os.path.join(LIBDIR, "libuno_spectral.so")
STAMP = os.path.join(LIBDIR, "libuno_spectral.stamp")
SOURCES = ["capi.hip", "capi_spectral.hip", "capi_pointwise.hip", "dft2d_fwd.hip", "dft2d_fwd_r4.hip", "dft2d_inv.hip", "dft2d_inv_b.hip", "dft2d_inv_c.hip", "dft2d_inv_add.hip", "dft2d_plane.hip", "dft2d_b16.hip", "mode_gemm.hip", "cdft_axis.hip", "dft3d_volume.hip", "dft_generic.hip", "resample3d_any.hip", "resample2d.hip", "channel_mix.hip", "channel_wgrad.hip", "adam.hip", "pointwise_fused.hip", "instnorm.hip", "lift_bwd.hip", "rel_l2_steps.hip", "rollout.hip", "rollout_train.hip"]
HEADERS = ["uno_common.h", "channel_mix_common.h", "dft2d_fwd_common.h", "dft2d_fwd_kernel.h", "dft2d_fwd_ft_kernel.h", "dft2d_fwd_ht_kernel.h", "dft2d_inv_kernel.h", "dft2d_inv_add_kernel.h", os.path.join("..", "..", "include", "uno_spectral.h")]
ARCH = "gfx950"
FLAGS = ["-O3", "-std=c++17", "-fPIC", f"--offload-arch={ARCH}", "-fno-gpu-rdc", "-Wall", "-Wno-unused-function"]
EXTRA_FLAGS = {"mode_gemm.hip": ["-mllvm", "-amdgpu-mfma-vgpr-form"], "dft2d_inv_add.hip": ["-mllvm", "-amdgpu-mfma-vgpr-form"]}


def _hipcc() -> str:
    for cand in (os.environ.get("HIPCC"), shutil.which("hipcc"), "/opt/rocm/bin/hipcc"):
        if cand and os.path.exists(cand):
            return cand
    raise RuntimeError("hipcc not found (set HIPCC or install ROCm)")


def _digest() -> str:
    h = hashlib.sha256()
    for f in SOURCES + HEADERS:
        with open(os.path.join(CSRC, f), "rb") as fh:
            h.update(fh.read())
    h.update(" ".join(FLAGS).encode())
    h.update(repr(sorted(EXTRA_FLAGS.items())).encode())
    return h.hexdigest()


def build(force: bool = False, verbose: bool = False) -> str:
    os.makedirs(LIBDIR, exist_ok=True)
    digest = _digest()
    if not force and os.path.exists(LIB) and os.path.exists(STAMP) and open(STAMP).read().strip() == digest:
        return LIB
    hipcc = _hipcc()
    objdir = os.path.join(LIBDIR, "obj")
    os.makedirs(objdir, exist_ok=True)

    def compile_one(src):
        obj = os.path.join(objdir, os.path.splitext(src)[0] + ".o")
        cmd = [hipcc, *FLAGS, *EXTRA_FLAGS.get(src, []), "-c", os.path.join(CSRC, src), "-o", obj]
        if verbose:
            print(" ".join(cmd), flush=True)
        r = subprocess.run(cmd, capture_output=True, text=True)
        if r.returncode != 0:
            raise RuntimeError(f"hipcc failed on {src}:\n{r.stdout}\n{r.stderr}")
        if verbose and r.stderr.strip():
            print(r.stderr)
        return obj

    jobs = min(len(SOURCES), os.cpu_count() or 1, int(os.environ.get("MAX_JOBS", 16)))
    with cf.ThreadPoolExecutor(max_workers=max(1, jobs)) as ex:
        objs = list(ex.map(compile_one, SOURCES))
    cmd = [hipcc, "-shared", "-fPIC", f"--offload-arch={ARCH}", "-fno-gpu-rdc", *objs, "-o", LIB]
    r = subprocess.run(cmd, capture_output=True, text=True)
    if r.returncode != 0:
        raise RuntimeError(f"link failed:\n{r.stdout}\n{r.stderr}")
    with open(STAMP, "w") as fh:
        fh.write(digest)
    return LIB


if __name__ == "__main__":
    ap = argparse.ArgumentParser()
    ap.add_argument("--force", action="store_true")
    ap.add_argument("--verbose", action="store_true")
    a = ap.parse_args()
    print(build(a.force, a.verbose))
```

### uno_amd/csrc/capi_spectral.hip

```cpp
#include "../../include/uno_spectral.h"
#include "uno_common.h"

#include <cstdlib>
#include <map>
#include <mutex>

namespace uno {

static int check_modes2d(const char* who, int H, int W, int Ho, int Wo, int m1, int m2) {
    if (H < 1 || W < 1 || Ho < 1 || Wo < 1) { set_error("%s: empty grid %dx%d -> %dx%d", who, H, W, Ho, Wo); return -1; }
    if (m1 < 1 || m1 > H || m1 > Ho) {
        set_error("%s: modes1=%d incompatible with grid rows %d -> %d (need 1 <= modes1 <= min rows)", who, m1, H, Ho);
        return -1;
    }
    if (m2 < 1 || m2 > W / 2 + 1 || m2 > Wo / 2 + 1) {
        set_error("%s: modes2=%d incompatible with grid cols %d -> %d (need modes2 <= cols/2+1)", who, m2, W, Wo);
        return -1;
    }
    return 0;
}

static int dft2d(bool inverse, const float* in, float* out, int n_img, int H, int W, int m1, int m2, float scale,
                 int herm, int mask, hipStream_t s, int sp_group = 0, int sp_stride = 0, int sp_offset = 0, int bf16 = 0) {
    const char* who = inverse ? "uno_dft2d_inverse" : "uno_dft2d_forward";
    if (n_img < 0) { set_error("%s: negative image count", who); return -1; }
    if (n_img > 0 && (!in || !out)) { set_error("%s: null pointer", who); return -1; }
    if (int rc = check_modes2d(who, H, W, H, W, m1, m2)) return rc;
    if (n_img == 0) return 0;
    Dft2dParams p;
    p.in = in; p.out = out; p.n_img = n_img; p.H = H; p.W = W; p.m1 = m1; p.m2 = m2;
    p.scale = scale; p.herm = herm ? 1 : 0; p.mask = mask ? 1 : 0; p.bf16 = bf16 ? 1 : 0;
    if (sp_group <= 0) { sp_group = n_img; sp_stride = 0; sp_offset = 0; }
    if (sp_offset < 0 || sp_stride < sp_offset + sp_group || n_img % sp_group) {
        if (!(sp_stride == 0 && sp_offset == 0 && sp_group == n_img)) {
            set_error("%s: bad spectrum grouping (group %d, stride %d, offset %d, images %d)", who, sp_group, sp_stride, sp_offset, n_img);
            return -1;
        }
    }
    p.sp_group = sp_group; p.sp_stride = sp_stride; p.sp_offset = sp_offset;
    p.twH = twiddle_table(H);
    p.twW = twiddle_table(W);
    if (!p.twH || !p.twW) return -6;
    if (m1 > 40 || m2 > 48) return launch_dft2d_generic(p, inverse, thread_scratch().ptr, thread_scratch().bytes, s);
    if (inverse ? dft2d_inv_plane_applies(p) : dft2d_fwd_plane_applies(p))
        return inverse ? launch_dft2d_inv_plane(p, s) : launch_dft2d_fwd_plane(p, s);
    if (dft2d_b16_applies(p)) {
        const int rc = inverse ? launch_dft2d_inv_b16(p, s) : launch_dft2d_fwd_b16(p, s);
        if (rc != -3) return rc;
    }
    return inverse ? launch_dft2d_inv(p, s) : launch_dft2d_fwd(p, s);
}

static int mode_gemm_params(ModeGemmParams& p, int op, const float2* act, const float2* const* w, const float2* go, float2* out_act,
                            float2* const* out_w, int B, int Ci, int Co, int nc, int Mc, hipStream_t s, int w_half, int accumulate) {
    if (B < 0 || Ci < 1 || Co < 1 || nc < 1 || nc > 4 || Mc < 1) {
        set_error("mode gemm: bad sizes B=%d Ci=%d Co=%d corners=%d modes=%d", B, Ci, Co, nc, Mc);
        return -1;
    }
    if (B == 0 && op != 2) return 1;
    const long long P = (long long)nc * Mc;
    p.ncorner = nc; p.Mc = Mc; p.accumulate = (op == 2 && accumulate) ? 1 : 0;
    p.A.half = 0; p.B.half = (op != 2 && w_half) ? 1 : 0;
    for (int c = 0; c < 4; ++c) { p.A.base[c] = nullptr; p.B.base[c] = nullptr; p.out[c] = nullptr; }
    if (op == 0) {
        p.M = B; p.N = Co; p.K = Ci;
        p.A.s0 = (long long)Ci * P; p.A.s1 = P; p.A.conj = 0;
        p.B.s0 = (long long)Co * Mc; p.B.s1 = Mc; p.B.conj = 0;
        p.o_sm = (long long)Co * P; p.o_sn = P;
        for (int c = 0; c < nc; ++c) { p.A.base[c] = act + (long long)c * Mc; p.B.base[c] = w[c]; p.out[c] = out_act + (long long)c * Mc; }
    } else if (op == 1) {
        p.M = B; p.N = Ci; p.K = Co;
        p.A.s0 = (long long)Co * P; p.A.s1 = P; p.A.conj = 0;
        p.B.s0 = Mc; p.B.s1 = (long long)Co * Mc; p.B.conj = 1;
        p.o_sm = (long long)Ci * P; p.o_sn = P;
        for (int c = 0; c < nc; ++c) { p.A.base[c] = act + (long long)c * Mc; p.B.base[c] = w[c]; p.out[c] = out_act + (long long)c * Mc; }
    } else {
        p.M = Ci; p.N = Co; p.K = B;
        p.A.s0 = P; p.A.s1 = (long long)Ci * P; p.A.conj = 1;
        p.B.s0 = (long long)Co * P; p.B.s1 = P; p.B.conj = 0;
        p.o_sm = (long long)Co * Mc; p.o_sn = Mc;
        for (int c = 0; c < nc; ++c) { p.A.base[c] = act + (long long)c * Mc; p.B.base[c] = go + (long long)c * Mc; p.out[c] = out_w[c]; }
        if (B == 0) {
            if (accumulate) return 1;
            for (int c = 0; c < nc; ++c)
                if (hipMemsetAsync(out_w[c], 0, sizeof(float2) * (size_t)Ci * Co * Mc, s) != hipSuccess) { set_error("memset failed"); return -5; }
            return 1;
        }
    }
    return 0;
}

static int mode_gemm(int op, const float2* act, const float2* const* w, const float2* go, float2* out_act,
                     float2* const* out_w, int B, int Ci, int Co, int nc, int Mc, hipStream_t s, int w_half = 0, int accumulate = 0) {
    ModeGemmParams p;
    const int rc = mode_gemm_params(p, op, act, w, go, out_act, out_w, B, Ci, Co, nc, Mc, s, w_half, accumulate);
    if (rc != 0) return rc < 0 ? rc : 0;
    return launch_mode_gemm(p, s);
}

static int mode_backward(const float2* xtrunc, const float2* go, const float2* const* w, float2* gx_spec, float2* const* gw, int B, int Ci,
                         int Co, int nc, int Mc, hipStream_t s, int accumulate) {
    ModeGemmParams pa, pb;
    const int ra = mode_gemm_params(pa, 1, go, w, nullptr, gx_spec, nullptr, B, Ci, Co, nc, Mc, s, 0, 0);
    if (ra < 0) return ra;
    const int rb = mode_gemm_params(pb, 2, xtrunc, nullptr, go, nullptr, gw, B, Ci, Co, nc, Mc, s, 0, accumulate);
    if (rb < 0) return rb;
    if (ra == 0 && rb == 0) return launch_mode_gemm_pair(pa, pb, s);
    if (rb == 0) if (int rc = launch_mode_gemm(pb, s)) return rc;
    if (ra == 0) return launch_mode_gemm(pa, s);
    return 0;
}

}

using namespace uno;


namespace {
struct SideStream {
    hipStream_t s = nullptr;
    hipEvent_t fork_ev = nullptr, join_ev = nullptr;
    std::mutex mu;
    bool ok = false;
};
SideStream* side_stream_of_current_device() {
    static std::mutex mu;
    static std::map<int, SideStream*> table;
    int dev = 0;
    if (hipGetDevice(&dev) != hipSuccess) return nullptr;
    std::lock_guard<std::mutex> g(mu);
    auto it = table.find(dev);
    if (it != table.end()) return it->second->ok ? it->second : nullptr;
    SideStream* ss = new SideStream();
    ss->ok = hipStreamCreateWithFlags(&ss->s, hipStreamNonBlocking) == hipSuccess &&
             hipEventCreateWithFlags(&ss->fork_ev, hipEventDisableTiming) == hipSuccess &&
             hipEventCreateWithFlags(&ss->join_ev, hipEventDisableTiming) == hipSuccess;
    table[dev] = ss;
    return ss->ok ? ss : nullptr;
}
}

extern "C" {

long long uno_dft2d_any_ws_bytes(int n_img, int H, int W, int m1, int m2) {
    (void)W;
    if (n_img <= 0 || H <= 0 || m2 <= 0) return 0;
    return (m1 > 40 || m2 > 48) ? 8LL * n_img * H * m2 : 0;
}

long long uno_spectral_conv2d_fwd_ws_bytes(int B, int Ci, int Co, int m1, int m2) {
    (void)Ci;
    return 8LL * B * Co * 2 * m1 * m2;
}

long long uno_spectral_conv2d_bwd_ws_bytes(int B, int Ci, int Co, int m1, int m2) {
    return 8LL * B * (Ci + Co) * 2 * m1 * m2;
}

int uno_dft2d_forward(const float* images, float* spec, int n_img, int H, int W, int m1, int m2, float scale,
                      int hermitian_cols, int mask_overlap, void* stream) {
    return dft2d(false, images, spec, n_img, H, W, m1, m2, scale, hermitian_cols, mask_overlap, (hipStream_t)stream);
}

int uno_dft2d_inverse(const float* spec, float* images, int n_img, int H, int W, int m1, int m2, float scale,
                      int hermitian_cols, int mask_overlap, void* stream) {
    return dft2d(true, spec, images, n_img, H, W, m1, m2, scale, hermitian_cols, mask_overlap, (hipStream_t)stream);
}

int uno_dft2d_inverse_add_applies(int n_img, int H, int W, int m1, int m2, int Hs, int Ws) {
    if (n_img < 1 || H < 1 || W < 1 || m1 < 1 || m2 < 1 || Hs < 1 || Ws < 1 || m1 > H || m2 > W / 2 + 1 || m1 > 40 || m2 > 48) return 0;
    Dft2dParams p;
    p.n_img = n_img; p.H = H; p.W = W; p.m1 = m1; p.m2 = m2; p.herm = 1; p.mask = 1;
    p.sp_group = n_img; p.sp_stride = 0;
    p.add_Hs = Hs; p.add_Ws = Ws;
    if (dft2d_inv_plane_applies(p)) return 0;
    return dft2d_inv_add_applies(p) ? 1 : 0;
}

int uno_dft2d_inverse_add(const float* spec, float* images, int n_img, int H, int W, int m1, int m2, float scale, int hermitian_cols,
                          int mask_overlap, const float* addend, int Hs, int Ws, const int* tile_p0, const float* row_op,
                          const int* col_v0, const float* col_op, void* stream) {
    const char* who = "uno_dft2d_inverse_add";
    if (n_img < 0) { set_error("%s: negative image count", who); return -1; }
    if (n_img > 0 && (!spec || !images || !addend || !tile_p0 || !row_op || !col_v0 || !col_op)) { set_error("%s: null pointer", who); return -1; }
    if (int rc = check_modes2d(who, H, W, H, W, m1, m2)) return rc;
    if (Hs < 1 || Ws < 12 || (long long)Hs * Ws * 4 > 0x7fffffffLL) { set_error("%s: bad addend grid %dx%d", who, Hs, Ws); return -1; }
    if (n_img == 0) return 0;
    if (!uno_dft2d_inverse_add_applies(n_img, H, W, m1, m2, Hs, Ws)) {
        set_error("%s: the fused form does not apply to %d images of %dx%d, modes (%d, %d) (query uno_dft2d_inverse_add_applies)", who, n_img, H, W, m1, m2);
        return -3;
    }
    Dft2dParams p;
    p.in = spec; p.out = images; p.n_img = n_img; p.H = H; p.W = W; p.m1 = m1; p.m2 = m2;
    p.scale = scale; p.herm = hermitian_cols ? 1 : 0; p.mask = mask_overlap ? 1 : 0;
    p.sp_group = n_img; p.sp_stride = 0;
    p.twH = twiddle_table(H);
    p.twW = twiddle_table(W);
    if (!p.twH || !p.twW) return -6;
    p.add_src = addend; p.add_Hs = Hs; p.add_Ws = Ws; p.add_p0 = tile_p0; p.add_rowop = row_op; p.add_v0 = col_v0; p.add_colop = col_op;
#ifdef UNO_K3A_DEV
    { static const int dev_exp = getenv("UNO_K3A_STAGGER") ? atoi(getenv("UNO_K3A_STAGGER")) : 0; p.exp = dev_exp; }
#endif
    return launch_dft2d_inv_add(p, (hipStream_t)stream);
}

int uno_dft2d_forward_bf16(const void* images, float* spec, int n_img, int H, int W, int m1, int m2, float scale,
                           int hermitian_cols, int mask_overlap, void* stream) {
    return dft2d(false, static_cast<const float*>(images), spec, n_img, H, W, m1, m2, scale, hermitian_cols, mask_overlap,
                 (hipStream_t)stream, 0, 0, 0, 1);
}

int uno_dft2d_inverse_bf16(const float* spec, void* images, int n_img, int H, int W, int m1, int m2, float scale,
                           int hermitian_cols, int mask_overlap, void* stream) {
    return dft2d(true, spec, static_cast<float*>(images), n_img, H, W, m1, m2, scale, hermitian_cols, mask_overlap,
                 (hipStream_t)stream, 0, 0, 0, 1);
}

int uno_dft2d_forward_grouped(const float* images, float* spec, int n_img, int H, int W, int m1, int m2, float scale,
                              int hermitian_cols, int mask_overlap, int group, int stride, int offset, void* stream) {
    if (group < 1) { set_error("uno_dft2d_forward_grouped: group must be positive"); return -1; }
    return dft2d(false, images, spec, n_img, H, W, m1, m2, scale, hermitian_cols, mask_overlap, (hipStream_t)stream, group, stride, offset);
}

int uno_dft2d_forward_grouped_bf16(const void* images, float* spec, int n_img, int H, int W, int m1, int m2, float scale,
                                   int hermitian_cols, int mask_overlap, int group, int stride, int offset, void* stream) {
    if (group < 1) { set_error("uno_dft2d_forward_grouped_bf16: group must be positive"); return -1; }
    return dft2d(false, static_cast<const float*>(images), spec, n_img, H, W, m1, m2, scale, hermitian_cols, mask_overlap,
                 (hipStream_t)stream, group, stride, offset, 1);
}

int uno_dft2d_inverse_grouped_bf16(const float* spec, void* images, int n_img, int H, int W, int m1, int m2, float scale,
                                   int hermitian_cols, int mask_overlap, int group, int stride, int offset, void* stream) {
    if (group < 1) { set_error("uno_dft2d_inverse_grouped_bf16: group must be positive"); return -1; }
    return dft2d(true, spec, static_cast<float*>(images), n_img, H, W, m1, m2, scale, hermitian_cols, mask_overlap,
                 (hipStream_t)stream, group, stride, offset, 1);
}

int uno_dft2d_inverse_grouped(const float* spec, float* images, int n_img, int H, int W, int m1, int m2, float scale,
                              int hermitian_cols, int mask_overlap, int group, int stride, int offset, void* stream) {
    if (group < 1) { set_error("uno_dft2d_inverse_grouped: group must be positive"); return -1; }
    return dft2d(true, spec, images, n_img, H, W, m1, m2, scale, hermitian_cols, mask_overlap, (hipStream_t)stream, group, stride, offset);
}

static int mode_mix_impl(const float* in, const float* const* w, float* out, int op, int B, int Ci, int Co, int ncorner,
                         int modes_per_corner, void* stream, int w_half) {
    if (!w || (B > 0 && (!in || !out))) { set_error("uno_mode_mix: null pointer"); return -1; }
    if (op != 0 && op != 1) { set_error("uno_mode_mix: op must be 0 or 1"); return -1; }
    if (ncorner < 1 || ncorner > 4) { set_error("uno_mode_mix: ncorner=%d out of range", ncorner); return -1; }
    for (int c = 0; c < ncorner; ++c)
        if (!w[c]) { set_error("uno_mode_mix: null weight pointer %d", c); return -1; }
    return mode_gemm(op, reinterpret_cast<const float2*>(in), reinterpret_cast<const float2* const*>(w), nullptr,
                     reinterpret_cast<float2*>(out), nullptr, B, Ci, Co, ncorner, modes_per_corner, (hipStream_t)stream, w_half);
}

int uno_mode_mix(const float* in, const float* const* w, float* out, int op, int B, int Ci, int Co, int ncorner,
                 int modes_per_corner, void* stream) {
    return mode_mix_impl(in, w, out, op, B, Ci, Co, ncorner, modes_per_corner, stream, 0);
}

int uno_mode_mix_f16w(const float* in, const void* const* w, float* out, int op, int B, int Ci, int Co, int ncorner,
                      int modes_per_corner, void* stream) {
    return mode_mix_impl(in, reinterpret_cast<const float* const*>(w), out, op, B, Ci, Co, ncorner, modes_per_corner, stream, 1);
}

static int mode_wgrad_impl(const float* xtrunc, const float* go, float* const* gw, int B, int Ci, int Co, int ncorner,
                           int modes_per_corner, int accumulate, void* stream) {
    if (!gw || (B > 0 && (!xtrunc || !go))) { set_error("uno_mode_wgrad: null pointer"); return -1; }
    if (ncorner < 1 || ncorner > 4) { set_error("uno_mode_wgrad: ncorner=%d out of range", ncorner); return -1; }
    for (int c = 0; c < ncorner; ++c)
        if (!gw[c]) { set_error("uno_mode_wgrad: null output pointer %d", c); return -1; }
    return mode_gemm(2, reinterpret_cast<const float2*>(xtrunc), nullptr, reinterpret_cast<const float2*>(go), nullptr,
                     reinterpret_cast<float2* const*>(gw), B, Ci, Co, ncorner, modes_per_corner, (hipStream_t)stream, 0, accumulate);
}

int uno_mode_wgrad(const float* xtrunc, const float* go, float* const* gw, int B, int Ci, int Co, int ncorner,
                   int modes_per_corner, void* stream) {
    return mode_wgrad_impl(xtrunc, go, gw, B, Ci, Co, ncorner, modes_per_corner, 0, stream);
}

int uno_mode_backward(const float* xtrunc, const float* go, const float* const* w, float* gx_spec, float* const* gw, int B, int Ci, int Co,
                      int ncorner, int modes_per_corner, int accumulate, void* stream) {
    if (!w || !gw || (B > 0 && (!xtrunc || !go || !gx_spec))) { set_error("uno_mode_backward: null pointer"); return -1; }
    if (ncorner < 1 || ncorner > 4) { set_error("uno_mode_backward: ncorner=%d out of range", ncorner); return -1; }
    for (int c = 0; c < ncorner; ++c)
        if (!w[c] || !gw[c]) { set_error("uno_mode_backward: null weight / gradient pointer %d", c); return -1; }
    return mode_backward(reinterpret_cast<const float2*>(xtrunc), reinterpret_cast<const float2*>(go), reinterpret_cast<const float2* const*>(w),
                         reinterpret_cast<float2*>(gx_spec), reinterpret_cast<float2* const*>(gw), B, Ci, Co, ncorner, modes_per_corner,
                         (hipStream_t)stream, accumulate);
}

int uno_mode_wgrad_acc(const float* xtrunc, const float* go, float* const* gw, int B, int Ci, int Co, int ncorner,
                       int modes_per_corner, int accumulate, void* stream) {
    return mode_wgrad_impl(xtrunc, go, gw, B, Ci, Co, ncorner, modes_per_corner, accumulate, stream);
}

int uno_cdft_axis(const float* in, float* out, int inverse, int n_img, int H, int m1, int m2, int m3, float scale,
                  int mask_overlap, void* stream) {
    if (n_img < 0 || H < 1 || m1 < 1 || m1 > H || m2 < 1 || m3 < 1) {
        set_error("uno_cdft_axis: bad sizes n_img=%d H=%d modes=(%d,%d,%d)", n_img, H, m1, m2, m3);
        return -1;
    }
    if (n_img == 0) return 0;
    if (!in || !out) { set_error("uno_cdft_axis: null pointer"); return -1; }
    CdftParams p;
    p.in = in; p.out = out; p.n_img = n_img; p.H = H; p.C = 2 * m2 * m3; p.m1 = m1; p.m2 = m2; p.m3 = m3;
    p.scale = scale; p.mask = mask_overlap ? 1 : 0;
    p.tw = twiddle_table(H);
    if (!p.tw) return -6;
    if (m1 > 40) return launch_cdft_generic(p, inverse != 0, (hipStream_t)stream);
    return launch_cdft(p, inverse != 0, (hipStream_t)stream);
}

long long uno_fft_resample3d_ws_bytes(int n_vol, int D1, int M1, int J1, int J2, int m3) {
    const long long C = (long long)J2 * m3;
    return 8LL * n_vol * ((long long)D1 * C + (long long)M1 * C + (long long)J1 * C);
}

static int fft_resample3d_impl(const float* x, float* y, void* ws, int n_vol, int D1, int D2, int D3, int M1, int M2, int M3,
                               int J1, const int* f1_in, const int* f1_out, int J2, const int* f2_in, const int* f2_out, int m3,
                               float scale, int herm_in, int herm_out, int accumulate, float* act_out, void* stream) {
    const char* who = "uno_fft_resample3d";
    if (n_vol < 0 || D1 < 1 || D2 < 1 || D3 < 1 || M1 < 1 || M2 < 1 || M3 < 1) { set_error("%s: bad sizes", who); return -1; }
    if (J1 < 2 || (J1 & 1) || J2 < 2 || (J2 & 1) || J1 > 80 || J2 > 48 || m3 < 1 || m3 > D3 / 2 + 1 || m3 > M3 / 2 + 1) {
        set_error("%s: row counts must be even (J1=%d <= 80, J2=%d <= 48) and 1 <= modes3=%d <= n/2+1", who, J1, J2, m3);
        return -1;
    }
    if (n_vol == 0) return 0;
    if (!x || !y || !ws || !f1_in || !f1_out || !f2_in || !f2_out) { set_error("%s: null pointer", who); return -1; }
    hipStream_t s = (hipStream_t)stream;
    const long long C = (long long)J2 * m3;
    float* Z1 = static_cast<float*>(ws);
    float* Z2 = Z1 + 2LL * n_vol * D1 * C;
    float* S = Z2 + 2LL * n_vol * M1 * C;
    Dft2dParams p;
    p.n_img = n_vol * D1; p.H = D2; p.W = D3; p.m1 = J2 / 2; p.m2 = m3; p.herm = herm_in ? 1 : 0;
    p.sp_group = p.n_img; p.sp_stride = 0;
    p.in = x; p.out = Z1; p.rowfreq = f2_in;
    p.twH = twiddle_table(D2); p.twW = twiddle_table(D3);
    if (!p.twH || !p.twW) return -6;
    if (!dft2d_fwd_plane_applies(p)) { set_error("%s: input planes %d x %d (%d of them) are outside the plane-batched kernels' range", who, D2, D3, p.n_img); return -2; }
    if (int rc = launch_dft2d_fwd_plane(p, s)) return rc;
    CdftParams c;
    c.n_img = n_vol; c.C = (int)C; c.m1 = J1 / 2; c.m2 = J2 / 2; c.m3 = m3;
    c.in = Z1; c.out = S; c.H = D1; c.rowfreq = f1_in; c.tw = twiddle_table(D1);
    if (!c.tw) return -6;
    if (int rc = launch_cdft(c, false, s)) return rc;
    c.in = S; c.out = Z2; c.H = M1; c.rowfreq = f1_out; c.tw = twiddle_table(M1);
    if (!c.tw) return -6;
    if (int rc = launch_cdft(c, true, s)) return rc;
    p.n_img = n_vol * M1; p.H = M2; p.W = M3; p.scale = scale; p.herm = herm_out ? 1 : 0;
    p.sp_group = p.n_img;
    p.in = Z2; p.out = y; p.rowfreq = f2_out;
    p.twH = twiddle_table(M2); p.twW = twiddle_table(M3);
    if (!p.twH || !p.twW) return -6;
    if (!dft2d_inv_plane_applies(p)) { set_error("%s: output planes %d x %d (%d of them) are outside the plane-batched kernels' range", who, M2, M3, p.n_img); return -2; }
    p.accumulate = accumulate ? 1 : 0; p.act_out = act_out;
    return launch_dft2d_inv_plane(p, s);
}

int uno_fft_resample3d(const float* x, float* y, void* ws, int n_vol, int D1, int D2, int D3, int M1, int M2, int M3,
                       int J1, const int* f1_in, const int* f1_out, int J2, const int* f2_in, const int* f2_out, int m3,
                       float scale, int herm_in, int herm_out, void* stream) {
    return fft_resample3d_impl(x, y, ws, n_vol, D1, D2, D3, M1, M2, M3, J1, f1_in, f1_out, J2, f2_in, f2_out, m3, scale, herm_in, herm_out,
                               0, nullptr, stream);
}

int uno_fft_resample3d_acc(const float* x, float* y, float* y_act, void* ws, int n_vol, int D1, int D2, int D3, int M1, int M2, int M3,
                           int J1, const int* f1_in, const int* f1_out, int J2, const int* f2_in, const int* f2_out, int m3,
                           float scale, int herm_in, int herm_out, void* stream) {
    return fft_resample3d_impl(x, y, ws, n_vol, D1, D2, D3, M1, M2, M3, J1, f1_in, f1_out, J2, f2_in, f2_out, m3, scale, herm_in, herm_out,
                               1, y_act, stream);
}

long long uno_fft_resample3d_any_ws_bytes(int n_vol, int D1, int M1, int J1, int J2, int m3) {
    (void)J1;
    return 8LL * n_vol * ((long long)D1 + M1) * J2 * m3;
}

static int fft_resample3d_any_impl(const char* who, const float* x, float* y, float* y_act, int accumulate, void* ws, int n_vol, int D1,
                                   int D2, int D3, int M1, int M2, int M3, int J1, const int* f1_in, const int* f1_out, int J2,
                                   const int* f2_in, const int* f2_out, int m3, float scale, int herm_in, int herm_out, void* stream) {
    const int dims[6] = {D1, D2, D3, M1, M2, M3};
    for (int d : dims)
        if (d < 2 || d > 128) {
            set_error("%s: grid (%d,%d,%d) -> (%d,%d,%d): every axis length must be in 2 ... 128", who, D1, D2, D3, M1, M2, M3);
            return -1;
        }
    if (J1 < 1 || J1 > 128 || J2 < 1 || J2 > 128) { set_error("%s: kept-row counts J1=%d, J2=%d must be in 1 ... 128", who, J1, J2); return -1; }
    if (m3 < 1 || m3 > D3 / 2 + 1 || m3 > M3 / 2 + 1) {
        set_error("%s: need 1 <= modes3=%d <= n/2+1 on the last axis %d -> %d", who, m3, D3, M3);
        return -1;
    }
    if (n_vol < 0 || (long long)n_vol * 128 > 0x7fffffffLL) { set_error("%s: bad volume count %d (0 ... 2^24 - 1)", who, n_vol); return -1; }
    if (accumulate) {
        if (y_act && y_act == y) { set_error("%s: y_act must not alias y", who); return -1; }
        if (x && x == y) { set_error("%s: x must not alias y", who); return -1; }
        if (x && x == y_act) { set_error("%s: x must not alias y_act", who); return -1; }
    }
    if (n_vol == 0) return 0;
    if (!x || !y || !ws || !f1_in || !f1_out || !f2_in || !f2_out) { set_error("%s: null pointer", who); return -1; }
    return launch_resample3d_any(x, y, y_act, accumulate, ws, n_vol, D1, D2, D3, M1, M2, M3, J1, f1_in, f1_out, J2, f2_in, f2_out, m3, scale,
                                 herm_in, herm_out, (hipStream_t)stream);
}

int uno_fft_resample3d_any(const float* x, float* y, void* ws, int n_vol, int D1, int D2, int D3, int M1, int M2, int M3,
                           int J1, const int* f1_in, const int* f1_out, int J2, const int* f2_in, const int* f2_out, int m3,
                           float scale, int herm_in, int herm_out, void* stream) {
    return fft_resample3d_any_impl("uno_fft_resample3d_any", x, y, nullptr, 0, ws, n_vol, D1, D2, D3, M1, M2, M3, J1, f1_in, f1_out, J2, f2_in,
                                   f2_out, m3, scale, herm_in, herm_out, stream);
}

int uno_fft_resample3d_any_acc(const float* x, float* y, float* y_act, void* ws, int n_vol, int D1, int D2, int D3, int M1, int M2, int M3,
                               int J1, const int* f1_in, const int* f1_out, int J2, const int* f2_in, const int* f2_out, int m3,
                               float scale, int herm_in, int herm_out, void* stream) {
    return fft_resample3d_any_impl("uno_fft_resample3d_any_acc", x, y, y_act, 1, ws, n_vol, D1, D2, D3, M1, M2, M3, J1, f1_in, f1_out, J2,
                                   f2_in, f2_out, m3, scale, herm_in, herm_out, stream);
}

static int check_modes3d(const char* who, int H, int W, int T, int Ho, int Wo, int To, int m1, int m2, int m3) {
    if (H < 1 || W < 1 || T < 1 || Ho < 1 || Wo < 1 || To < 1) { set_error("%s: empty grid", who); return -1; }
    if (m1 < 1 || m1 > H || m1 > Ho) { set_error("%s: modes1=%d incompatible with axis %d -> %d", who, m1, H, Ho); return -1; }
    if (m2 < 1 || m2 > W || m2 > Wo) { set_error("%s: modes2=%d incompatible with axis %d -> %d", who, m2, W, Wo); return -1; }
    if (m3 < 1 || m3 > T / 2 + 1 || m3 > To / 2 + 1) {
        set_error("%s: modes3=%d incompatible with axis %d -> %d (need modes3 <= n/2+1)", who, m3, T, To);
        return -1;
    }
    return 0;
}

static int fwd_transform3d(const float* x, float* spec, float* Z, int n_vol, int D1, int D2, int D3, int m1, int m2, int m3, float scale,
                           int adjoint, hipStream_t s) {
    if (vol3d_fwd_applies(n_vol, D1, D2, D3, m1, m2, m3)) {
        Vol3dParams v;
        v.in = x; v.out = spec; v.n_vol = n_vol; v.D1 = D1; v.D2 = D2; v.D3 = D3; v.m1 = m1; v.m2 = m2; v.m3 = m3;
        v.scale = scale; v.herm = adjoint;
        v.tw1 = twiddle_table(2 * D1); v.tw2 = twiddle_table(2 * D2); v.tw3 = twiddle_table(D3);
        if (!v.tw1 || !v.tw2 || !v.tw3) return -6;
        return launch_dft3d_fwd_volume(v, s);
    }
    if (int rc = dft2d(false, x, Z, n_vol * D1, D2, D3, m2, m3, scale, adjoint, adjoint, s)) return rc;
    return uno_cdft_axis(Z, spec, 0, n_vol, D1, m1, m2, m3, 1.0f, adjoint, (void*)s);
}

static int inv_transform3d(const float* spec, float* y, float* Z, int n_vol, int D1, int D2, int D3, int m1, int m2, int m3, float scale,
                           int weighted, hipStream_t s) {
    if (vol3d_inv_applies(n_vol, D1, D2, D3, m1, m2, m3)) {
        Vol3dParams v;
        v.in = spec; v.out = y; v.n_vol = n_vol; v.D1 = D1; v.D2 = D2; v.D3 = D3; v.m1 = m1; v.m2 = m2; v.m3 = m3;
        v.scale = scale; v.herm = weighted;
        v.tw1 = twiddle_table(2 * D1); v.tw2 = twiddle_table(2 * D2); v.tw3 = twiddle_table(D3);
        if (!v.tw1 || !v.tw2 || !v.tw3) return -6;
        return launch_dft3d_inv_volume(v, s);
    }
    if (int rc = uno_cdft_axis(spec, Z, 1, n_vol, D1, m1, m2, m3, 1.0f, weighted, (void*)s)) return rc;
    return dft2d(true, Z, y, n_vol * D1, D2, D3, m2, m3, scale, weighted, weighted, s);
}

long long uno_spectral_conv3d_fwd_ws_bytes(int B, int Ci, int Co, int H, int Ho, int m1, int m2, int m3) {
    const long long C = 2LL * m2 * m3;
    return 8LL * B * ((long long)Ci * H * C + (long long)Co * Ho * C + 4LL * Co * m1 * m2 * m3);
}

long long uno_spectral_conv3d_bwd_ws_bytes(int B, int Ci, int Co, int H, int Ho, int m1, int m2, int m3) {
    const long long C = 2LL * m2 * m3;
    return 8LL * B * ((long long)Ci * H * C + (long long)Co * Ho * C + 4LL * (Ci + Co) * m1 * m2 * m3);
}

int uno_spectral_conv3d_forward(const float* x, const float* const* w, float* y, float* xtrunc, void* ws, int B, int Ci,
                                int Co, int H, int W, int T, int Ho, int Wo, int To, int m1, int m2, int m3, void* stream) {
    const char* who = "uno_spectral_conv3d_forward";
    if (B < 0 || Ci < 1 || Co < 1) { set_error("%s: bad sizes B=%d Ci=%d Co=%d", who, B, Ci, Co); return -1; }
    if (int rc = check_modes3d(who, H, W, T, Ho, Wo, To, m1, m2, m3)) return rc;
    if (B == 0) return 0;
    if (!x || !w || !y || !xtrunc || !ws) { set_error("%s: null pointer", who); return -1; }
    hipStream_t s = (hipStream_t)stream;
    const long long C = 2LL * m2 * m3, Mc = (long long)m1 * m2 * m3;
    float* Z1 = static_cast<float*>(ws);
    float* Z2 = Z1 + 2LL * B * Ci * H * C;
    float* O5 = Z2 + 2LL * B * Co * Ho * C;
    const float inv_n = 1.0f / ((float)H * (float)W * (float)T);
    if (int rc = fwd_transform3d(x, xtrunc, Z1, B * Ci, H, W, T, m1, m2, m3, inv_n, 0, s)) return rc;
    if (int rc = uno_mode_mix(xtrunc, w, O5, 0, B, Ci, Co, 4, (int)Mc, stream)) return rc;
    return inv_transform3d(O5, y, Z2, B * Co, Ho, Wo, To, m1, m2, m3, 1.0f, 1, s);
}

int uno_spectral_conv3d_backward(const float* gy, const float* xtrunc, const float* const* w, float* gx, float* const* gw,
                                 void* ws, int B, int Ci, int Co, int H, int W, int T, int Ho, int Wo, int To, int m1,
                                 int m2, int m3, void* stream) {
    const char* who = "uno_spectral_conv3d_backward";
    if (B < 0 || Ci < 1 || Co < 1) { set_error("%s: bad sizes B=%d Ci=%d Co=%d", who, B, Ci, Co); return -1; }
    if (int rc = check_modes3d(who, H, W, T, Ho, Wo, To, m1, m2, m3)) return rc;
    hipStream_t s = (hipStream_t)stream;
    const long long C = 2LL * m2 * m3, Mc = (long long)m1 * m2 * m3;
    if (B == 0) {
        if (gw)
            for (int c = 0; c < 4; ++c)
                if (hipMemsetAsync(gw[c], 0, 8ULL * Ci * Co * Mc, s) != hipSuccess) { set_error("memset failed"); return -5; }
        return 0;
    }
    if (!gy || !xtrunc || !w || !ws) { set_error("%s: null pointer", who); return -1; }
    float* Z1 = static_cast<float*>(ws);
    float* Z2 = Z1 + 2LL * B * Ci * H * C;
    float* gO = Z2 + 2LL * B * Co * Ho * C;
    float* gX = gO + 2LL * B * Co * 4 * Mc;
    if (int rc = fwd_transform3d(gy, gO, Z2, B * Co, Ho, Wo, To, m1, m2, m3, 1.0f, 1, s)) return rc;
    if (gw)
// ... 118 lines not shown
```

### uno_amd/csrc/dft2d_fwd_ft_kernel.h

```cpp
#pragma once
#include "dft2d_fwd_common.h"

namespace uno {

constexpr size_t FT_LDS_BUDGET = 160 * 1024 - 2048;
constexpr int FT_AUX = 2;
constexpr int FT_MAXW = 160;

template <int NT, int MT, int R4>
__global__ __launch_bounds__(256) void dft2d_fwd_ft_kernel(Dft2dParams p) {
    constexpr int NTF = R4 > 0 ? NT - 1 : NT;
    constexpr int NQ = R4 > 0 ? R4 : 1;
    constexpr int NTFA = NTF > 0 ? NTF : 1;
    extern __shared__ __attribute__((aligned(16))) char smem[];
    const int H = p.H, W = p.W, m1 = p.m1, m2 = p.m2;
    const int tid = threadIdx.x;
    const int nthreads = blockDim.x;
    const int NWT = nthreads >> 6;
    const int NW = p.nw;
    const int wave = __builtin_amdgcn_readfirstlane(tid >> 6);
    const int lane = tid & 63;
    const int r16 = lane & 15;
    const int kk = lane >> 4;
    const unsigned H8 = 8u * H;
    UNO_FWD_COLUMN_PAIRS(W);
    const int nk = 4 * nfull + tailsteps;

    const int tile_stride = (16 * W + 32 + 3) & ~3;
    float* sTile = reinterpret_cast<float*>(smem);
    float2* sTabF = reinterpret_cast<float2*>(sTile + (size_t)NWT * tile_stride);
    const int nka = UNO_FWD_TABLE_STEPS(nfull);
    float2* sTab4 = sTabF + (size_t)nka * NTF * 64;
    float2* sTwH = sTab4 + (size_t)nka * R4 * 16;
    int* sTailW = reinterpret_cast<int*>(sTwH + H);

    const int slot = wave / NW, wsub = wave - slot * NW;
    const int image = sweep_x(p.rev) * (NWT / NW) + slot;
    const bool active = image < p.n_img;
    const int nrt = (H + 15) >> 4;
    float* buf = sTile + (size_t)wave * tile_stride;

    int a0;
    const __amdgpu_buffer_rsrc_t rsrc = image_rsrc(p.in, p.n_img, H, W, active ? image : 0, &a0);
    auto request_tile = [&](int rt) {
        const int toff = a0 + rt * 16 * W;
        const int rows = min(16, H - 16 * rt);
        const int total = (toff & 31) + rows * W;
        const int npiece = (total + 255) >> 8;
        const unsigned v0 = (unsigned)(((toff & ~31) + 4 * lane) * 4);
        for (int i = 0; i < npiece; ++i)
            if (256 * i + 4 * lane < total)
                __builtin_amdgcn_raw_ptr_buffer_load_lds(rsrc, (lds_ptr_t)(buf + 256 * i), 16, v0 + 1024u * (unsigned)i, 0, 0, FT_AUX);
    };
    if (active && wsub < nrt) request_tile(wsub);

    for (int n = tid; n < H; n += nthreads) sTwH[n] = p.twH[n];
    for (int e = tid; e < FWD_TAILMAX * 64; e += nthreads) { UNO_FWD_PUT_TAIL_COLUMNS(e); }
    UNO_FWD_BUILD_OPERAND_TABLES();
    __syncthreads();

    UNO_FWD_ACCUMULATORS(false, MT);

    const float2* tabF = sTabF + lane;
    const float2* tab4 = sTab4 + 4 * kk + (lane & 3);

    if (active) {
        for (int rt = wsub; rt < nrt; rt += NW) {
            const int toff = a0 + rt * 16 * W;
            const int phase = toff & 31;
            const int rows = min(16, H - 16 * rt);
            const float* row = buf + phase + r16 * W;
            asm volatile("s_waitcnt vmcnt(0)" ::: "memory");
            if (rows < 16) {
                for (int i = phase + rows * W + lane; i < phase + 16 * W; i += 64) buf[i] = 0.f;
            }

            f32x4 Tr[NT], Tn[NT];
            f32x4 Qr[NQ], Qn[NQ];
#pragma unroll
            for (int t = 0; t < NT; ++t) { Tr[t] = f32x4{0, 0, 0, 0}; Tn[t] = f32x4{0, 0, 0, 0}; }
#pragma unroll
            for (int g = 0; g < NQ; ++g) { Qr[g] = f32x4{0, 0, 0, 0}; Qn[g] = f32x4{0, 0, 0, 0}; }
#define UNO_FT_MFMA(E_, D_, TWF_, TW4_)                                                   \
    do {                                                                                  \
        _Pragma("unroll") for (int t = 0; t < NTF; ++t) {                                 \
            Tr[t] = mfma16((E_), (TWF_)[t].x, Tr[t]);                                     \
            Tn[t] = mfma16((D_), (TWF_)[t].y, Tn[t]);                                     \
        }                                                                                 \
        _Pragma("unroll") for (int g = 0; g < R4; ++g) {                                  \
            Qr[g] = mfma4((E_), (TW4_)[g].x, Qr[g]);                                   \
            Qn[g] = mfma4((D_), (TW4_)[g].y, Qn[g]);                                   \
        }                                                                                 \
    } while (0)

            struct RowOps { float xl[4], xr[4]; float2 twF[4][NTFA], tw4[4][NQ]; };
            RowOps opA, opB;
            const float* pl = row + 1 + 4 * kk;
            const float* pr = row + W - 4 - 4 * kk;
            auto load_ops = [&](RowOps& o, int c) {
                const int cn = min(c, max(nfull - 1, 0));
                const float2* tf = tabF + (size_t)(4 * c) * (NTF * 64);
                const float2* t4 = tab4 + (size_t)(4 * c) * (R4 * 16);
#pragma unroll
                for (int s = 0; s < 4; ++s) {
                    o.xl[s] = pl[16 * cn + s]; o.xr[s] = pr[-16 * cn + s];
#pragma unroll
                    for (int t = 0; t < NTF; ++t) o.twF[s][t] = tf[(s * NTF + t) * 64];
#pragma unroll
                    for (int g = 0; g < R4; ++g) o.tw4[s][g] = t4[(s * R4 + g) * 16];
                }
            };
            auto chunk = [&](RowOps& cur, RowOps& nxt, int c) {
                load_ops(nxt, c + 1);
                __builtin_amdgcn_sched_barrier(0);
#pragma unroll
                for (int s = 0; s < 4; ++s) {
                    const float E = cur.xl[s] + cur.xr[3 - s];
                    const float D = cur.xl[s] - cur.xr[3 - s];
                    UNO_FT_MFMA(E, D, cur.twF[s], cur.tw4[s]);
                }
                __builtin_amdgcn_sched_barrier(0);
            };
            load_ops(opA, 0);
            {
                int c = 0;
                for (; c + 2 <= nfull; c += 2) { chunk(opA, opB, c); chunk(opB, opA, c + 1); }
                if (c < nfull) { chunk(opA, opB, c); opA = opB; }
            }
            float2 (&twF)[4][NTFA] = opA.twF;
            float2 (&tw4)[4][NQ] = opA.tw4;
            {
                const float2* tf = tabF + (size_t)(4 * nfull) * (NTF * 64);
                const float2* t4 = tab4 + (size_t)(4 * nfull) * (R4 * 16);
                float TL[FWD_TAILMAX], TR[FWD_TAILMAX];
#pragma unroll
                for (int s = 0; s < FWD_TAILMAX; ++s) {
                    const int wl = sTailW[(s * 2 + 0) * 64 + lane], wr = sTailW[(s * 2 + 1) * 64 + lane];
                    const float vl = row[max(wl, 0)], vr = row[max(wr, 0)];
                    TL[s] = wl >= 0 ? vl : 0.f; TR[s] = wr >= 0 ? vr : 0.f;
                }
                float2 twF5[NTFA], tw45[NQ];
#pragma unroll
                for (int t = 0; t < NTF; ++t) twF5[t] = tf[(4 * NTF + t) * 64];
#pragma unroll
                for (int g = 0; g < R4; ++g) tw45[g] = t4[(4 * R4 + g) * 16];
#pragma unroll
                for (int s = 0; s < FWD_TAILMAX; ++s) {
                    if (s < tailsteps) {
                        const float E = TL[s] + TR[s];
                        const float D = TL[s] - TR[s];
                        if (s < 4) UNO_FT_MFMA(E, D, twF[s], tw4[s]);
                        else UNO_FT_MFMA(E, D, twF5, tw45);
                    }
                }
            }
#undef UNO_FT_MFMA
            if (rt + NW < nrt) {
                asm volatile("s_waitcnt lgkmcnt(0)" ::: "memory");
                request_tile(rt + NW);
            }

            UNO_FWD_REGROUP_4X4();
            UNO_FWD_STAGE_B(false, MT);
        }
    }

    if (NW > 1) __syncthreads();
    for (int stride = 2; stride >= 1; stride >>= 1) {
        if (stride >= NW) continue;
        UNO_FWD_REDUCE_STEP(Xr, Xi, MT, buf, sTile + (size_t)(wave - stride) * tile_stride, wsub, stride);
    }
    if (active && wsub == 0) UNO_FWD_STORE_SPECTRUM(false, MT, image);
}

static size_t fwd_ft_lds_bytes(const Dft2dParams& p, int NTF, int R4, int waves) {
    const size_t tile_stride = (size_t)((16 * p.W + 32 + 3) & ~3);
    return (size_t)waves * tile_stride * 4 + fwd_table_bytes(p.W, NTF, R4) + (size_t)p.H * 8 + FWD_TAILMAX * 2 * 64 * 4;
}

static bool fwd_ft_geometry(const Dft2dParams& p, int NT, int MT, int R4, FwdFtGeometry* out) {
    const int NTF = R4 > 0 ? NT - 1 : NT;
    if (p.bf16 || p.rowfreq || p.W % 8 == 0 || ((p.W - 1) >> 1) < 16) return false;
    if (p.W > FT_MAXW) return false;
    if ((size_t)MT * NT * 8 * 64 > (size_t)16 * p.W) return false;
    return fwd_tile_geometry(p, NTF, R4, FwdTileForm{4, FT_LDS_BUDGET, 3, fwd_ft_lds_bytes}, out);
}

template <int NT, int MT, int R4>
static int launch_fwd_ft(const Dft2dParams& p, const FwdFtGeometry& g, hipStream_t s) {
    char name[64];
    snprintf(name, sizeof(name), "uno::dft2d_fwd_ft_kernel<%d, %d, %d>", NT, MT, R4);
    return launch_fwd_tile<dft2d_fwd_ft_kernel<NT, MT, R4>>(name, p, g, next_sweep_reversed(SWEEP_K1), s);
}

}
```

### uno_amd/csrc/uno_common.h

```cpp
#pragma once
#include <hip/hip_runtime.h>
#include <stdint.h>

namespace uno {

typedef float f32x4 __attribute__((ext_vector_type(4)));

__device__ __forceinline__ f32x4 mfma16(float a, float b, f32x4 c) {
    return __builtin_amdgcn_mfma_f32_16x16x4f32(a, b, c, 0, 0, 0);
}

__device__ __forceinline__ float uno_erf(float x) {
    x = __builtin_fminf(__builtin_fmaxf(x, -4.f), 4.f);
    const float t = x * x;
    float p = -2.72614225801306e-10f;
    p = fmaf(p, t, 2.77068142495902e-08f);
    p = fmaf(p, t, -2.10102402082508e-06f);
    p = fmaf(p, t, -5.69250639462346e-05f);
    p = fmaf(p, t, -7.34990630326855e-04f);
    p = fmaf(p, t, -2.95459980854025e-03f);
    p = fmaf(p, t, -1.60960333262415e-02f);
    p *= x;
    float q = -1.45660718464996e-05f;
    q = fmaf(q, t, -2.13374055278905e-04f);
    q = fmaf(q, t, -1.68282697438203e-03f);
    q = fmaf(q, t, -7.37332916720468e-03f);
    q = fmaf(q, t, -1.42647390514189e-02f);
    float r = __builtin_amdgcn_rcpf(q);
    r = r * fmaf(-q, r, 2.f);
    return p * r;
}
__device__ __forceinline__ float uno_gelu(float x) { return 0.5f * x * (1.f + uno_erf(x * 0.70710678118654752440f)); }
__device__ __forceinline__ float uno_dgelu(float x) {
    const float cdf = 0.5f * (1.f + uno_erf(x * 0.70710678118654752440f));
    const float pdf = 0.39894228040143267794f * __expf(-0.5f * x * x);
    return fmaf(x, pdf, cdf);
}

struct PixelWindow { long long plane = 0; int cols = 0, pitch = 0; };
struct PixMap {
    int PS; int rl, skip; unsigned magic;
};
inline PixMap pix_map(const PixelWindow& w, long long P) {
    if (!w.cols) return PixMap{(int)P, 0, 0, 0u};
    return PixMap{(int)w.plane, w.cols, w.pitch - w.cols, (unsigned)(((1ULL << 40) + w.cols - 1) / (unsigned long long)w.cols)};
}
inline const char* pix_window_error(const PixelWindow& w, long long P) {
    if (!w.cols) return nullptr;
    if (w.cols % 4 || w.cols < 260 || w.pitch < w.cols) return "window: cols must be a multiple of 4, >= 260 and <= pitch";
    if (P % w.cols || P >= (1LL << 24)) return "window: the pixel count must be rows * cols, below 2^24";
    if (w.plane < (P / w.cols - 1) * (long long)w.pitch + w.cols || w.plane > 0x7fffffffLL) return "window: the plane does not hold rows * pitch elements";
    return nullptr;
}
struct PixRun {
    int base, bound, skip;
    __device__ __forceinline__ int operator()(int q) const { return q + base + (q >= bound ? skip : 0); }
};
__device__ __forceinline__ PixRun pix_run(const PixMap& m, int q0) {
    if (m.rl == 0) return PixRun{0, 0x7fffffff, 0};
    const int r = (int)(((unsigned long long)(unsigned)q0 * m.magic) >> 40);
    return PixRun{r * m.skip, (r + 1) * m.rl, m.skip};
}
__device__ __forceinline__ int pix_phys(const PixMap& m, int q) {
    if (m.rl == 0) return q;
    return q + (int)(((unsigned long long)(unsigned)q * m.magic) >> 40) * m.skip;
}

__device__ __forceinline__ unsigned wrap_add(unsigned idx, unsigned inc, unsigned lim) {
    unsigned t = idx + inc;
    return min(t, t - lim);
}
__device__ __forceinline__ unsigned wrap_sub(unsigned idx, unsigned dec, unsigned lim) {
    unsigned t = idx - dec;
    return min(t, t + lim);
}

struct __attribute__((packed, aligned(4))) f4u { float v[4]; };

struct __attribute__((packed, aligned(2))) h4u { unsigned short v[4]; };
template <bool BF16> struct IoElem { typedef float type; typedef f4u vec4; };
template <> struct IoElem<true> { typedef unsigned short type; typedef h4u vec4; };
__device__ __forceinline__ float io_widen(float v) { return v; }
__device__ __forceinline__ float io_widen(unsigned short v) { return __uint_as_float((unsigned)v << 16); }
typedef __bf16 bf16x2_t __attribute__((ext_vector_type(2)));
typedef float f32x2_t __attribute__((ext_vector_type(2)));
__device__ __forceinline__ unsigned bf16_pack2(float lo, float hi) {
    return __builtin_bit_cast(unsigned, __builtin_convertvector(f32x2_t{lo, hi}, bf16x2_t));
}
__device__ __forceinline__ unsigned short bf16_rne(float f) { return (unsigned short)(bf16_pack2(f, 0.f) & 0xffffu); }
struct __attribute__((packed, aligned(2))) h8u { unsigned w[4]; };
__device__ __forceinline__ void io_store4(float* dst, float a, float b, float c, float d) {
    *reinterpret_cast<f4u*>(dst) = f4u{{a, b, c, d}};
}
__device__ __forceinline__ void io_store4(unsigned short* dst, float a, float b, float c, float d) {
    struct __attribute__((packed, aligned(2))) h4w { unsigned w[2]; };
    *reinterpret_cast<h4w*>(dst) = h4w{{bf16_pack2(a, b), bf16_pack2(c, d)}};
}
__device__ __forceinline__ void io_store8(unsigned short* dst, const f32x4& a, const f32x4& b) {
    *reinterpret_cast<h8u*>(dst) = h8u{{bf16_pack2(a[0], a[1]), bf16_pack2(a[2], a[3]), bf16_pack2(b[0], b[1]), bf16_pack2(b[2], b[3])}};
}
__device__ __forceinline__ float4 io_ld4(const float* p) {
    const f4u v = *reinterpret_cast<const f4u*>(p);
    return make_float4(v.v[0], v.v[1], v.v[2], v.v[3]);
}
__device__ __forceinline__ float4 io_ld4(const unsigned short* p) {
    const h4u v = *reinterpret_cast<const h4u*>(p);
    return make_float4(io_widen(v.v[0]), io_widen(v.v[1]), io_widen(v.v[2]), io_widen(v.v[3]));
}
__device__ __forceinline__ void io_store1(float* dst, float a) { *dst = a; }
__device__ __forceinline__ void io_store1(unsigned short* dst, float a) { *dst = bf16_rne(a); }

__device__ __forceinline__ float2 lds_tw(const float2* tab, unsigned byte_off) {
    return *reinterpret_cast<const float2*>(reinterpret_cast<const char*>(tab) + byte_off);
}

__device__ __forceinline__ float herm_weight(int l, int N) {
    return (l == 0 || 2 * l == N) ? 1.0f : 2.0f;
}

__host__ __device__ __forceinline__ int corner_freq(int j, int m, int N) { return j < m ? j : N - 2 * m + j; }

__host__ __device__ __forceinline__ bool row_survives(int j, int m, int N) { return j >= m || j < N - m; }

inline int pick_waves_per_image(int n_row_tiles) {
    int best = 1, best_waste = 1 << 30;
    for (int nw = 4; nw >= 1; --nw) {
        if (nw > n_row_tiles) continue;
        const int per = (n_row_tiles + nw - 1) / nw;
        const int waste = (per * nw - n_row_tiles) * 12 / nw;
        if (waste < best_waste) { best_waste = waste; best = nw; }
    }
    return best;
}

__device__ __forceinline__ int sweep_x(int rev) { return rev ? (int)(gridDim.x - 1 - blockIdx.x) : (int)blockIdx.x; }
__device__ __forceinline__ int sweep_y(int rev) { return rev ? (int)(gridDim.y - 1 - blockIdx.y) : (int)blockIdx.y; }

struct Dft2dParams {
    const float* in = nullptr;
    float* out = nullptr;
    const float2* twH = nullptr;
    const float2* twW = nullptr;
    int n_img = 0, H = 0, W = 0, m1 = 0, m2 = 0;
    float scale = 1.f;
    int herm = 0;
    int mask = 0;
    int sp_group = 1, sp_stride = 1, sp_offset = 0;
    int bf16 = 0;
    const int* rowfreq = nullptr;
    int nw = 1;
    int exp = 0;
    int accumulate = 0;
    float* act_out = nullptr;
    int rev = 0;
    const float* add_src = nullptr;
    int add_Hs = 0, add_Ws = 0;
    const int* add_p0 = nullptr;
    const float* add_rowop = nullptr;
    const int* add_v0 = nullptr;
    const float* add_colop = nullptr;
};

__device__ __forceinline__ size_t spectrum_index(const Dft2dParams& p, int img) {
    return (size_t)(img / p.sp_group) * p.sp_stride + p.sp_offset + img % p.sp_group;
}

struct ModeOperand {
    const float2* base[4];
    long long s0, s1;
    int conj;
    int half;
};
struct ModeGemmParams {
    ModeOperand A, B;
    float2* out[4];
    long long o_sm, o_sn;
    int M, N, K, ncorner, Mc;
    int accumulate;
};

struct CdftParams {
    const float* in = nullptr;
    float* out = nullptr;
    const float2* tw = nullptr;
    int n_img = 0, H = 0, C = 0, m1 = 0, m2 = 0, m3 = 0;
    float scale = 1.f;
    int mask = 0;
    const int* rowfreq = nullptr;
};

struct Vol3dParams {
    const float* in = nullptr;
    float* out = nullptr;
    const float2* tw1 = nullptr;
    const float2* tw2 = nullptr;
    const float2* tw3 = nullptr;
    int n_vol = 0, D1 = 0, D2 = 0, D3 = 0, m1 = 0, m2 = 0, m3 = 0;
    float scale = 1.f;
    int herm = 0;
    const float* ctab = nullptr;
};

const float2* twiddle_table(int N);
void* upload_table(const void* host, size_t bytes);
float2 twiddle_value(long long n, int N);

inline bool ensure_dynamic_lds(const void* kernel, size_t bytes, int* slot) {
    if (bytes <= 64 * 1024) return true;
    int dev = 0;
    if (hipGetDevice(&dev) != hipSuccess || dev < 0 || dev >= 64) dev = 0;
    if ((size_t)__atomic_load_n(&slot[dev], __ATOMIC_RELAXED) >= bytes) return true;
    const int want = 160 * 1024;
    if (hipFuncSetAttribute(kernel, hipFuncAttributeMaxDynamicSharedMemorySize, want) != hipSuccess) return false;
    __atomic_store_n(&slot[dev], want, __ATOMIC_RELAXED);
    return true;
}
void set_error(const char* fmt, ...);
struct Scratch { void* ptr; size_t bytes; };
const Scratch& thread_scratch();
int reserved_cus();
int next_sweep_reversed(int family);
enum { SWEEP_K1 = 1, SWEEP_K3 = 2, SWEEP_K7 = 4, SWEEP_K8 = 8, SWEEP_K9 = 16, SWEEP_NORM = 32, SWEEP_PROJ = 64, SWEEP_LIFT = 128 };
inline int usable_cus(int device_cus) { const int r = reserved_cus(); return device_cus - r >= 8 ? device_cus - r : (device_cus < 8 ? device_cus : 8); }

struct ProfScope {
    int slot;
    hipStream_t stream;
    ProfScope(const char* name, double bytes, hipStream_t s);
    ~ProfScope();
};

int launch_dft2d_fwd(const Dft2dParams& p, hipStream_t s);
int launch_dft2d_inv(const Dft2dParams& p, hipStream_t s);
bool dft2d_inv_add_applies(const Dft2dParams& p);
int launch_dft2d_inv_add(const Dft2dParams& p, hipStream_t s);
bool dft2d_fwd_plane_applies(const Dft2dParams& p);
bool dft2d_inv_plane_applies(const Dft2dParams& p);
bool dft2d_b16_applies(const Dft2dParams& p);
int launch_dft2d_fwd_b16(const Dft2dParams& p, hipStream_t s);
int launch_dft2d_inv_b16(const Dft2dParams& p, hipStream_t s);
int launch_dft2d_fwd_plane(const Dft2dParams& p, hipStream_t s);
int launch_dft2d_inv_plane(const Dft2dParams& p, hipStream_t s);
bool vol3d_fwd_applies(int n_vol, int D1, int D2, int D3, int m1, int m2, int m3);
bool vol3d_inv_applies(int n_vol, int D1, int D2, int D3, int m1, int m2, int m3);
int launch_dft3d_fwd_volume(const Vol3dParams& p, hipStream_t s);
int launch_dft3d_inv_volume(const Vol3dParams& p, hipStream_t s);
int launch_mode_gemm(const ModeGemmParams& p, hipStream_t s);
int launch_mode_gemm_pair(const ModeGemmParams& input_grad, const ModeGemmParams& weight_grad, hipStream_t s);
int launch_cdft(const CdftParams& p, bool inverse, hipStream_t s);
int launch_dft2d_generic(const Dft2dParams& p, bool inverse, void* ws, size_t ws_bytes, hipStream_t s);
int launch_cdft_generic(const CdftParams& p, bool inverse, hipStream_t s);
int launch_resample3d_any(const float* x, float* y, float* y_act, int accumulate, void* ws, int n_vol, int D1, int D2, int D3, int M1, int M2, int M3, int J1,
                          const int* f1_in, const int* f1_out, int J2, const int* f2_in, const int* f2_out, int m3, float scale,
                          int herm_in, int herm_out, hipStream_t s);
int launch_resample2d(const void* in, void* out, float* tmp, int n_img, int H, int W, int Ho, int Wo, const int* startH,
                      const float* wtH, int KH, const int* startW, const float* wtW, int KW, const int* tile_p0,
                      const float* tile_w, int NP, int accumulate, int bf16, hipStream_t s);
struct ChannelMixArgs {
    const void* x; const void* x2; const float* w; const float* bias; void* y; void* y2; void* y_act; const void* dgelu_of;
    const float* proj_w; const float* proj_b; void* proj_out;
    int B, Ci, Co, C1, Co1; long long P; int transpose_w, accumulate, act_in, bf16;
    PixelWindow win;
    void* ws = nullptr; size_t ws_bytes = 0;
    const float* vh_x = nullptr; const float* vh_w = nullptr; const float* vh_b = nullptr; int vh_ci = 0, vh_mode = 0;
    const void* gmul = nullptr;
    const float* pb_w2 = nullptr; const float* pb_g = nullptr;
    int act_cols = 0, act_pitch = 0; long long act_plane = 0;
};
int launch_clear_border(float* t, long long n_planes, int Hp, int Wp, int rows, int cols, hipStream_t s);
int launch_channel_mix2(const ChannelMixArgs& a, hipStream_t s);
int launch_channel_mix(const void* x, const float* w, const float* bias, void* y, int B, int Ci, int Co, long long P,
                       int transpose_w, int accumulate, int act_in, const void* dgelu_of, int bf16, hipStream_t s, void* ws = nullptr,
                       size_t ws_bytes = 0);
long long channel_mix_ws_bytes(int Ci, int Co, long long P, int bf16);
int launch_adam_multi(int n_tensors, float* const* p, const float* const* g, float* const* m, float* const* v, const long long* n,
                      const int* is_complex, double lr, double beta1, double beta2, double eps, double wd, int step, hipStream_t s,
                      const float* dev_scalars = nullptr);
int launch_adam_advance(int* step, float* scalars, const double* hyper, double lr, double eps, double wd, double beta1, double beta2,
                        hipStream_t s);
int launch_adam(float* p, const float* g, float* m, float* v, long long n, int is_complex, double lr, double beta1, double beta2,
                double eps, double wd, int step, hipStream_t s);
struct GeluProjectSecond { const void* s = nullptr; void* gs = nullptr; int C1 = 0, act = 0; };
int launch_gelu_project_fwd(const void* pre, const float* w, const float* bias, void* out, int B, int C, long long P, int bf16, hipStream_t s,
                            const GeluProjectSecond* two = nullptr);
long long gelu_project_ws_floats(int B, int C, long long P);
int launch_gelu_project_bwd(const void* pre, const float* w, const void* gout, void* gpre, float* gw, float* gb, float* ws, int B,
                            int C, long long P, int bf16, hipStream_t s, const PixelWindow& win = PixelWindow(),
                            const GeluProjectSecond* two = nullptr);
int launch_gelu_pad(const void* s, const void* gy, void* out, int n_img, int H, int W, int Hp, int Wp, int backward, int bf16, hipStream_t st);
int launch_transpose_batched(const float* in, float* out, int B, long long R, int C, long long ld_in, long long sb_in, long long ld_out,
                             long long sb_out, hipStream_t st);
int launch_instnorm_fwd(const void* x, const float* gamma, const float* beta, void* y, float* mean, float* rstd, long long rows, int C,
                        long long N, float eps, int gelu, int bf16, hipStream_t s);
int launch_instnorm_bwd(const void* x, const void* gy, const float* gamma, const float* beta, const float* mean, const float* rstd,
                        void* gx, float* s1, float* s2, long long rows, int C, long long N, int gelu, int bf16, hipStream_t s);
long long channel_wgrad_ws_floats(int B, int Ci, int Co, long long P, int* nsplit_out);
int launch_channel_wgrad(const void* gy, const void* x, float* gw, float* gb, float* ws, int B, int Ci, int Co, long long P,
                         int act_x, int bf16, hipStream_t s);
struct WgradProjectedBack { const float* w2 = nullptr; const float* g = nullptr; float* gw2 = nullptr; float* gb2 = nullptr; };
bool channel_wgrad_pb_applies(int B, int Ci, int Co, int C1, long long P);
long long channel_wgrad_pb_ws_floats(int B, int Ci, int Co, long long P);
int launch_channel_wgrad2(const void* gy, const void* x, const void* x2, int C1, float* gw, float* gb, float* ws, int B, int Ci, int Co,
                          long long P, int act_x, int accumulate, int bf16, hipStream_t s, const PixelWindow& win = PixelWindow(),
                          const WgradProjectedBack& pb = WgradProjectedBack());
int launch_channel_wgrad_vh(const void* gy, const float* vh_x, const float* vh_w, const float* vh_b, int vh_ci, float* gw, float* gb, float* ws,
                            int B, int Ci, int Co, long long P, int act_x, hipStream_t s, int accumulate = 0);
bool lift_bwd_fused_applies(int Cin, int Cm, int Co, int W, long long P);
long long lift_bwd_fused_parts(int B, int H, int W);
int launch_lift_forward_fused(const float* x, const float* w1, const float* b1, const float* w0, const float* b0, float* act, int B, int Cin,
                              int H, int W, int Hp, int Wp, hipStream_t s);
int launch_lift_backward_fused(const float* x, const float* w1, const float* b1, const float* w0, const float* b0, const float* g, float* part,
                               float* part1, int B, int Cin, int H, int W, int Hp, int Wp, hipStream_t s, const float* g2 = nullptr);
int launch_channel_wgrad_finish(const float* parts, float* gw, float* gb, int Ci, int Co, long long nparts, int accumulate, hipStream_t s);
long long rel_l2_steps_chunks(long long P, int T, long long* chunk_pixels);
long long rel_l2_steps_ws_floats(int B, long long P, int T);
int launch_rel_l2_steps(const float* pred, const float* target, float* sums, float* rel, float* totals, float* ws, int B, long long P, int T,
                        hipStream_t s);
int launch_rel_l2_steps_finish(const float* ws, float* sums, float* rel, float* totals, int B, int T, long long nc, hipStream_t s);
long long rollout_chunks(long long P, long long* chunk_pixels);
long long rollout_ws_floats(int B, long long P, int T);
int launch_rollout_advance(float* window, const float* frame, const float* target, float* pred, float* ws, int B, int C, int T_in, long long P,
                           int T, int t, int shift, hipStream_t s);
long long rollout_lift_bwd_ws_floats(int B, int C, int Cm, long long P, int T);
int launch_rollout_lift(const float* given, const float* pred, const float* feat, const float* w, const float* bias, float* h, int B, int T_in,
                        int F, int Cm, long long P, int T, int t, hipStream_t s);
int launch_rollout_lift_backward(const float* gh, const float* given, const float* pred, const float* target, const float* feat, const float* w,
                                 const float* sums, const float* gL, float* gpred, float* gframe, float* parts, int B, int T_in, int F, int Cm,
                                 long long P, int T, int t, hipStream_t s);
int launch_rollout_loss_seed(const float* pred, const float* target, const float* sums, const float* gL, float* gframe, int B, long long P, int T,
                             hipStream_t s);

}
```

### uno_amd/resample.py

```python
from __future__ import annotations

import functools

import torch
import torch.nn.functional as F
from torch.autograd.function import once_differentiable

from . import _native


@functools.lru_cache(maxsize=None)
def _matrix(n_in: int, n_out: int, mode: str = "bicubic_aa") -> torch.Tensor:
    eye = torch.eye(n_in, dtype=torch.float32).view(1, n_in, n_in, 1).expand(1, n_in, n_in, 2).contiguous()
    if mode == "bicubic_aa":
        r = F.interpolate(eye, size=(n_out, 2), mode="bicubic", align_corners=True, antialias=True)
    elif mode == "linear":
        r = F.interpolate(eye, size=(n_out, 2), mode="bilinear", align_corners=True)
    else:
        raise ValueError(mode)
    return r[0, :, :, 0].t().contiguous()


def _band(mat: torch.Tensor):
    nz = mat != 0
    n_out, n_in = mat.shape
    first = torch.where(nz.any(1), nz.float().argmax(1), torch.zeros(n_out, dtype=torch.long))
    last = torch.where(nz.any(1), n_in - 1 - nz.flip(1).float().argmax(1), torch.zeros(n_out, dtype=torch.long))
    K = int((last - first + 1).max())
    cols = first[:, None] + torch.arange(K)[None, :]
    w = torch.where(cols < n_in, mat.gather(1, cols.clamp(max=n_in - 1)), torch.zeros((), dtype=mat.dtype))
    return first.to(torch.int32), w.to(torch.float32), K


TILE_ROWS = 16


def _row_tiles(mat: torch.Tensor):
    n_out, n_in = mat.shape
    first, w, K = _band(mat)
    ntiles = (n_out + TILE_ROWS - 1) // TILE_ROWS
    p0 = torch.zeros(ntiles, dtype=torch.int32)
    spans = []
    for k in range(ntiles):
        rows = range(TILE_ROWS * k, min(TILE_ROWS * (k + 1), n_out))
        lo = min(int(first[i]) for i in rows)
        hi = max(min(int(first[i]) + K, n_in) for i in rows)
        p0[k] = lo
        spans.append(hi - lo)
    NP = max(spans)
    tw = torch.zeros(ntiles, NP, TILE_ROWS, dtype=torch.float32)
    for k in range(ntiles):
        for r in range(TILE_ROWS):
            i = TILE_ROWS * k + r
            if i >= n_out:
                break
            lo = int(p0[k])
            seg = mat[i, lo:min(lo + NP, n_in)].to(torch.float32)
            tw[k, :seg.numel(), r] = seg
    return p0, tw


@functools.lru_cache(maxsize=None)
def _tables(n_in: int, n_out: int, device_str: str, mode: str = "bicubic_aa"):
    R = _matrix(n_in, n_out, mode)
    dev = torch.device(device_str)
    out = []
    for M in (R, R.t().contiguous()):
        s, w, _ = _band(M)
        p0, tw = _row_tiles(M)
        up = lambda t: _native.table_to_device(t.contiguous(), dev)
        out.append(((up(s), up(w)), (up(p0), up(tw))))
    return tuple(out)


ADD_KE = 3


def _add_operands(Rh: torch.Tensor, Rw: torch.Tensor):
    H, Hs = Rh.shape
    W, Ws = Rw.shape
    span = 4 * ADD_KE
    if Hs < 1 or Ws < span:
        return None
    lane = torch.arange(64)
    r16, kk = lane % 16, lane // 16

    def band(M, rows):
        rows = [r for r in rows if 0 <= r < M.shape[0]]
        if not rows:
            return 0, -1
        nz = (M[rows] != 0).any(0).nonzero().flatten()
        return (int(nz[0]), int(nz[-1])) if nz.numel() else (0, -1)

    nrt = (H + 15) // 16
    p0 = torch.zeros(nrt, dtype=torch.int32)
    rowop = torch.zeros(nrt, ADD_KE, 64, dtype=torch.float32)
    Rh_pad = torch.zeros(16 * nrt, Hs + span, dtype=torch.float32)
    Rh_pad[:H, :Hs] = Rh
    for rt in range(nrt):
        lo, hi = band(Rh, range(16 * rt, 16 * rt + 16))
        if hi - lo + 1 > span:
            return None
        p0[rt] = lo
        for e in range(ADD_KE):
            rowop[rt, e] = Rh_pad[16 * rt + r16, lo + ADD_KE * kk + e]
    nwt = ((W // 2) + 16) // 16
    v0 = torch.zeros(nwt, 2, dtype=torch.int32)
    colop = torch.zeros(nwt, 2, ADD_KE, 64, dtype=torch.float32)
    Rw_pad = torch.zeros(W + 1, Ws + span, dtype=torch.float32)
    Rw_pad[:W, :Ws] = Rw
    for wt in range(nwt):
        for side in range(2):
            cols = [16 * wt + i if side == 0 else W - 16 * wt - i for i in range(16)]
            lo, hi = band(Rw, cols)
            lo = max(min(lo, Ws - span), 0)
            if hi - lo + 1 > span:
                return None
            v0[wt, side] = lo
            w = torch.tensor([c if 0 <= c < W else W for c in cols])[r16]
            for ks in range(ADD_KE):
                colop[wt, side, ks] = Rw_pad[w, lo + ADD_KE * kk + ks]
    return p0, rowop.contiguous(), v0.contiguous(), colop.contiguous()


@functools.lru_cache(maxsize=None)
def upsample_add_tables(Hs: int, Ws: int, H: int, W: int, device_str: str, adjoint: bool = False, mode: str = "bicubic_aa"):
    if adjoint:
        Rh, Rw = _matrix(H, Hs, mode).t().contiguous(), _matrix(W, Ws, mode).t().contiguous()
    else:
        Rh, Rw = _matrix(Hs, H, mode), _matrix(Ws, W, mode)
    ops = _add_operands(Rh, Rw)
    if ops is None:
        return None
    dev = torch.device(device_str)
    return tuple(_native.table_to_device(t, dev) for t in ops)


def resample_forward(x: torch.Tensor, Ho: int, Wo: int, out: torch.Tensor | None = None) -> torch.Tensor:
    H, W = x.shape[-2:]
    (fh, th), _ = _tables(H, Ho, str(x.device))
    (fw, _), _ = _tables(W, Wo, str(x.device))
    return _native.resample2d(x, Ho, Wo, fh, fw, th, out=out)


def resample_adjoint(gy: torch.Tensor, H: int, W: int, out: torch.Tensor | None = None) -> torch.Tensor:
    Ho, Wo = gy.shape[-2:]
    _, (bh, th) = _tables(H, Ho, str(gy.device))
    _, (bw, _) = _tables(W, Wo, str(gy.device))
    return _native.resample2d(gy, H, W, bh, bw, th, out=out)


class _Resample2dFn(torch.autograd.Function):
    @staticmethod
    def forward(ctx, x, Ho, Wo):
        x = x.contiguous()
        ctx.in_hw = tuple(x.shape[-2:])
        return resample_forward(x, Ho, Wo)

    @staticmethod
    @once_differentiable
    def backward(ctx, gy):
        return resample_adjoint(gy.contiguous(), *ctx.in_hw), None, None


def resample2d_bicubic_aa(x: torch.Tensor, Ho: int, Wo: int) -> torch.Tensor:
    if x.shape[-2] == Ho and x.shape[-1] == Wo:
        return x
    return _Resample2dFn.apply(x, int(Ho), int(Wo))


def _apply3d(x: torch.Tensor, sizes, adjoint: bool) -> torch.Tensor:
    dev = str(x.device)
    B, C = x.shape[:2]
    (i1, i2, i3), (o1, o2, o3) = sizes
    k = 1 if adjoint else 0
    src, dst = ((o1, o2, o3), (i1, i2, i3)) if adjoint else ((i1, i2, i3), (o1, o2, o3))

    def tabs(n_in, n_out):
        return _tables(n_in, n_out, dev, "linear")[k]

    def last_two(t, d1):
        if (src[1], src[2]) == (dst[1], dst[2]):
            return t
        (bh, th), (bw, _) = tabs(i2, o2), tabs(i3, o3)
        return _native.resample2d(t.reshape(B * C * d1, src[1], src[2]), dst[1], dst[2], bh, bw, th).view(B, C, d1, dst[1], dst[2])

    def first(t, d2, d3):
        if src[0] == dst[0]:
            return t
        (bh, th) = tabs(i1, o1)
        (bw, _) = _tables(d2 * d3, d2 * d3, dev, "linear")[0]
        return _native.resample2d(t.reshape(B * C, src[0], d2 * d3), dst[0], d2 * d3, bh, bw, th).view(B, C, dst[0], d2, d3)

    if src[0] * dst[1] * dst[2] <= dst[0] * src[1] * src[2]:
        return first(last_two(x, src[0]), dst[1], dst[2])
    return last_two(first(x, src[1], src[2]), dst[0])


class _Trilinear3dFn(torch.autograd.Function):
    @staticmethod
    def forward(ctx, x, size):
        x = x.contiguous()
        ctx.sizes = (tuple(x.shape[2:]), tuple(size))
        return _apply3d(x, ctx.sizes, adjoint=False)

    @staticmethod
    @once_differentiable
    def backward(ctx, gy):
        return _apply3d(gy.contiguous(), ctx.sizes, adjoint=True), None


def resample3d_trilinear(x: torch.Tensor, size) -> torch.Tensor:
    size = tuple(int(v) for v in size)
    if tuple(x.shape[2:]) == size:
        return x
    if x.is_cuda and x.dtype == torch.float32 and x.dim() == 5 and min(x.shape[2:]) > 1 and min(size) > 1:
        return _Trilinear3dFn.apply(x, size)
    return F.interpolate(x, size=size, mode="trilinear", align_corners=True)
```

Baseline: 1496 samples/s.

## Fuse downsampling resample into forward DFT kernel

Adds a new forward-DFT kernel that, while streaming image tiles for the truncated 2D DFT, also computes a banded bicubic resample to a smaller grid. It is used in the block forward when mixing happens last and the grid shrinks, and in backward for the resample adjoint of the gradient. The goal is to avoid a separate resample kernel that re-reads the full-resolution tensor. In exchange it adds register- and LDS-heavy kernel complexity, a closure-based hook in the backward path, and shape-restricted applicability checks.

```diff
diff --git a/include/uno_spectral.h b/include/uno_spectral.h
--- a/include/uno_spectral.h
+++ b/include/uno_spectral.h
@@ -77,6 +77,11 @@
 int uno_dft2d_inverse_add(const float* spec, float* images, int n_img, int H, int W, int m1, int m2, float scale, int hermitian_cols,
                           int mask_overlap, const float* addend, int Hs, int Ws, const int* tile_p0, const float* row_op,
                           const int* col_v0, const float* col_op, void* stream);
+
+int uno_dft2d_forward_resample_applies(int n_img, int H, int W, int m1, int m2, int Ho, int Wo, int KW);
+int uno_dft2d_forward_resample(const float* images, float* spec, int n_img, int H, int W, int m1, int m2, float scale, int hermitian_cols,
+                               int mask_overlap, int group, int stride, int offset, float* resampled, int Ho, int Wo, const int* col_start,
+                               const float* col_wt, int KW, const int* row_tiles, const float* row_op, void* stream);
 
 int uno_dft2d_forward_bf16(const void* images, float* spec, int n_img, int H, int W, int m1, int m2,
                            float scale, int hermitian_cols, int mask_overlap, void* stream);
diff --git a/uno_amd/_native.py b/uno_amd/_native.py
--- a/uno_amd/_native.py
+++ b/uno_amd/_native.py
@@ -39,6 +39,8 @@
     "uno_reserve_cus": (C.c_int, [_i]),
     "uno_sweep_alternation": (C.c_int, [_i]),
     "uno_dft2d_inverse_add_applies": (C.c_int, [_i] * 7),
+    "uno_dft2d_forward_resample_applies": (C.c_int, [_i] * 8),
+    "uno_dft2d_forward_resample": (C.c_int, [_fp, _fp] + [_i] * 5 + [C.c_float] + [_i] * 5 + [_fp, _i, _i, _fp, _fp, _i, _fp, _fp, _fp]),
     "uno_dft2d_inverse_add": (C.c_int, [_fp, _fp] + [_i] * 5 + [C.c_float, _i, _i, _fp, _i, _i, _fp, _fp, _fp, _fp, _fp]),
     "uno_dft2d_forward_grouped": (C.c_int, [_fp, _fp] + [_i] * 5 + [C.c_float] + [_i] * 5 + [_fp]),
     "uno_dft2d_inverse_grouped": (C.c_int, [_fp, _fp] + [_i] * 5 + [C.c_float] + [_i] * 5 + [_fp]),
@@ -386,6 +388,33 @@
     return bool(lib().uno_dft2d_inverse_add_applies(int(n_img), int(H), int(W), int(m1), int(m2), int(Hs), int(Ws)))
 
 
+def dft2d_forward_resample_applies(n_img, H, W, m1, m2, Ho, Wo, KW) -> bool:
+    return bool(lib().uno_dft2d_forward_resample_applies(int(n_img), int(H), int(W), int(m1), int(m2), int(Ho), int(Wo), int(KW)))
+
+
+def dft2d_forward_resample(images, m1, m2, Ho, Wo, tables, scale=1.0, hermitian_cols=False, mask_overlap=False, out=None, channel_offset=0):
+    _require(images, torch.float32, "images")
+    col_start, col_wt, row_tiles, row_op = tables
+    *lead, H, W = images.shape
+    n = _count(lead)
+    group = stride = 0
+    if out is None:
+        spec = torch.empty((*lead, 2 * m1, m2), dtype=torch.complex64, device=images.device)
+    else:
+        _require(out, torch.complex64, "out")
+        if images.dim() != 4 or out.dim() != 4 or out.shape[0] != images.shape[0] or tuple(out.shape[2:]) != (2 * m1, m2) \
+                or channel_offset < 0 or channel_offset + images.shape[1] > out.shape[1]:
+            raise RuntimeError("uno_amd: out must be (B, Ctot, 2*m1, m2) with room for the image channels at channel_offset")
+        spec, group, stride = out, images.shape[1], out.shape[1]
+    res = torch.empty((*lead, Ho, Wo), dtype=torch.float32, device=images.device)
+    with torch.cuda.device(images.device):
+        rc = lib().uno_dft2d_forward_resample(_ptr(images), _ptr(spec), n, H, W, m1, m2, float(scale), int(hermitian_cols), int(mask_overlap),
+                                              int(group), int(stride), int(channel_offset), _ptr(res), int(Ho), int(Wo), _ptr(col_start),
+                                              _ptr(col_wt), int(col_wt.shape[1]), _ptr(row_tiles), _ptr(row_op), _stream(images))
+    _check(rc, "uno_dft2d_forward_resample")
+    return spec, res
+
+
 def dft2d_inverse(spec, H, W, scale=1.0, hermitian_cols=True, mask_overlap=True, channels=None, channel_offset=0,
                   dtype=torch.float32, addend=None):
     _require(spec, torch.complex64, "spec")
diff --git a/uno_amd/block2d.py b/uno_amd/block2d.py
--- a/uno_amd/block2d.py
+++ b/uno_amd/block2d.py
@@ -5,7 +5,7 @@
 from . import _native
 from ._param_grads import _grad_targets, _note_use, _stack_arrived, _stack_grad_slot, _stack_take, _stack_wanted
 from .pointwise import _mix2_forward, _mix2_input_grads, _plain, _wgrad_into
-from .resample import resample_adjoint, resample_forward, upsample_add_tables
+from .resample import fused_resample_tables, resample_adjoint, resample_forward, upsample_add_tables
 
 
 def _half_weights(w1, w2):
@@ -107,6 +107,22 @@
     return None if tabs is None else (t, tabs)
 
 
+FUSE_FORWARD_RESAMPLE = True
+
+
+def _fused_resample(x, m1, m2, Ho, Wo, adjoint):
+    if not FUSE_FORWARD_RESAMPLE or x.dtype != torch.float32 or x.dim() != 4 or not x.is_cuda:
+        return None
+    H, W = x.shape[-2], x.shape[-1]
+    n = x.shape[0] * x.shape[1]
+    if Ho * Wo >= H * W or not _native.dft2d_forward_resample_applies(n, H, W, m1, m2, Ho, Wo, 1):
+        return None
+    tabs = fused_resample_tables(H, W, Ho, Wo, str(x.device), bool(adjoint))
+    if tabs is None or not _native.dft2d_forward_resample_applies(n, H, W, m1, m2, Ho, Wo, tabs[1].shape[1]):
+        return None
+    return tabs
+
+
 def _stage_wgrad(stack, gslot, xt, gO, w1, w2, leaves, both_gw, need_gx):
     if gslot is not None:
         return (None, *_stack_arrived(stack, leaves, w1.shape, both_gw))
@@ -124,14 +140,14 @@
     return gX, gw1, gw2
 
 
-def _spectral_backward(gs, xt, w1, w2, H, W, need_gx, need_gw, both_gw, leaves, stack, join=None, addend=None):
+def _spectral_backward(gs, xt, w1, w2, H, W, need_gx, need_gw, both_gw, leaves, stack, join=None, addend=None, k1=None):
     B, Co = gs.shape[:2]
     Ci, _, m1, m2 = w1.shape[:4]
     gslot = _stack_grad_slot(stack, Co) if (stack is not None and need_gw) else None
     merging = join is not None and need_gx and bool(join.spectra)
     if addend is not None and not need_gx:
         raise RuntimeError("uno_amd: an addend for the input gradient needs the input gradient")
-    if gslot is None and not merging and addend is None and not (need_gx and need_gw and w1.dtype == torch.complex64):
+    if gslot is None and not merging and addend is None and k1 is None and not (need_gx and need_gw and w1.dtype == torch.complex64):
         tg = _grad_targets(leaves) if (need_gw and both_gw) else None
         if need_gw:
             _note_use(leaves[0])
@@ -140,7 +156,7 @@
         if tg:
             gw1, gw2 = tg.returned
         return gx, gw1, gw2, False
-    gO = _native.dft2d_forward(gs, m1, m2, 1.0, True, True, out=gslot)
+    gO = _native.dft2d_forward(gs, m1, m2, 1.0, True, True, out=gslot) if k1 is None else k1(gslot)
     gX, gw1, gw2 = _stage_wgrad(stack, gslot, xt, gO, w1, w2, leaves, both_gw, need_gx) if need_gw else (None, None, None)
     gx = None
     if need_gx:
@@ -177,6 +193,12 @@
             _native.dft2d_forward(x, m1, m2, 1.0 / (H * W), out=xt, channel_offset=0)
             O = _native.mode_mix(xt.view(B, Ci, 2, m1 * m2), [w1, w2], 0)
             s = _native.dft2d_inverse(O.view(B, Co, 2 * m1, m2), Ho, Wo, 1.0, True, True, addend=fused)
+        elif mix_last and not same and not half_weights and (rs := _fused_resample(x, w1.shape[2], w1.shape[3], Ho, Wo, False)) is not None:
+            m1, m2 = w1.shape[2], w1.shape[3]
+            xt = _xt_dest(ctx.stack, B, Ci, m1, m2, x.device)
+            _, pre_act = _native.dft2d_forward_resample(x, m1, m2, Ho, Wo, rs, 1.0 / (H * W), out=xt, channel_offset=0)
+            O = _native.mode_mix(xt.view(B, Ci, 2, m1 * m2), [w1, w2], 0)
+            s = _native.dft2d_inverse(O.view(B, Co, 2 * m1, m2), Ho, Wo, 1.0, True, True)
         else:
             pre_act = None
             if mix_last and not same:
@@ -230,14 +252,24 @@
         need_gc = ctx.needs_input_grad[3] or (has_bias and ctx.needs_input_grad[4])
         join = ctx.join
         lw1, lw2, lcw, lcb = ctx.leaves
-        g_act = addend = g_t = None
+        g_act = addend = g_t = k1 = None
         if not mix_last:
-            g_t = resample_adjoint(gs, H, W).view(B, Co, -1)
+            rs = _fused_resample(gs, w1.shape[2], w1.shape[3], H, W, True) if w1.dtype == torch.complex64 else None
+            if rs is None:
+                g_t = resample_adjoint(gs, H, W).view(B, Co, -1)
+            else:
+                both = []
+
+                def k1(out):
+                    both.extend(_native.dft2d_forward_resample(gs, w1.shape[2], w1.shape[3], H, W, rs, 1.0, True, True, out=out))
+                    return both[0]
         if mix_last and not same and need_gx and gs.dtype == torch.float32:
             g_act = _native.channel_mix(gs.view(B, Co, -1), cwm, None, transpose_w=True).view(B, Ci, Ho, Wo)
             addend = _fused_addend(g_act, H, W, w1.shape[2], w1.shape[3], True)
         gx, gw1, gw2, stacked = _spectral_backward(gs, xt, w1, w2, H, W, need_gx, need_gw, ctx.needs_input_grad[1] and ctx.needs_input_grad[2],
-                                                   (lw1, lw2), ctx.stack, join, addend)
+                                                   (lw1, lw2), ctx.stack, join, addend, k1)
+        if k1 is not None:
+            g_t = both[1].view(B, Co, -1)
         pstack = ctx.stack if stacked else None
         gcw = gcb = None
         xpre = join.pre if (join is not None and need_gx) else None
@@ -314,8 +346,13 @@
         lw1, lw2, lcw, lcb = ctx.leaves
         both_gw = ctx.needs_input_grad[2] and ctx.needs_input_grad[3]
         gslot = _stack_grad_slot(ctx.stack, Co) if (ctx.stack is not None and need_gw) else None
-        g_src = gs.view(B, Co, -1) if mix_last else resample_adjoint(gs, H, W).view(B, Co, -1)
-        gO = _native.dft2d_forward(gs, m1, m2, 1.0, True, True, out=gslot)
+        rs = _fused_resample(gs, m1, m2, H, W, True) if (not mix_last and w1.dtype == torch.complex64) else None
+        if rs is not None:
+            gO, g_src = _native.dft2d_forward_resample(gs, m1, m2, H, W, rs, 1.0, True, True, out=gslot)
+            g_src = g_src.view(B, Co, -1)
+        else:
+            g_src = gs.view(B, Co, -1) if mix_last else resample_adjoint(gs, H, W).view(B, Co, -1)
+            gO = _native.dft2d_forward(gs, m1, m2, 1.0, True, True, out=gslot)
         gXp, gw1, gw2 = _stage_wgrad(ctx.stack, gslot, xt, gO, w1, w2, (lw1, lw2), both_gw, need1 or need2) if need_gw else (None, None, None)
         gx1 = gx2 = None
         defer = ctx.defer if (need2 and ctx.defer is not None and ctx.defer.owner) else None
diff --git a/uno_amd/build.py b/uno_amd/build.py
--- a/uno_amd/build.py
+++ b/uno_amd/build.py
@@ -13,8 +13,8 @@
 LIBDIR = os.path.join(HERE, "lib")
 LIB = os.path.join(LIBDIR, "libuno_spectral.so")
 STAMP = os.path.join(LIBDIR, "libuno_spectral.stamp")
-SOURCES = ["capi.hip", "capi_spectral.hip", "capi_pointwise.hip", "dft2d_fwd.hip", "dft2d_fwd_r4.hip", "dft2d_inv.hip", "dft2d_inv_b.hip", "dft2d_inv_c.hip", "dft2d_inv_add.hip", "dft2d_plane.hip", "dft2d_b16.hip", "mode_gemm.hip", "cdft_axis.hip", "dft3d_volume.hip", "dft_generic.hip", "resample3d_any.hip", "resample2d.hip", "channel_mix.hip", "channel_wgrad.hip", "adam.hip", "pointwise_fused.hip", "instnorm.hip", "lift_bwd.hip", "rel_l2_steps.hip", "rollout.hip", "rollout_train.hip"]
-HEADERS = ["uno_common.h", "channel_mix_common.h", "dft2d_fwd_common.h", "dft2d_fwd_kernel.h", "dft2d_fwd_ft_kernel.h", "dft2d_fwd_ht_kernel.h", "dft2d_inv_kernel.h", "dft2d_inv_add_kernel.h", os.path.join("..", "..", "include", "uno_spectral.h")]
+SOURCES = ["capi.hip", "capi_spectral.hip", "capi_pointwise.hip", "dft2d_fwd.hip", "dft2d_fwd_r4.hip", "dft2d_fwd_fd.hip", "dft2d_inv.hip", "dft2d_inv_b.hip", "dft2d_inv_c.hip", "dft2d_inv_add.hip", "dft2d_plane.hip", "dft2d_b16.hip", "mode_gemm.hip", "cdft_axis.hip", "dft3d_volume.hip", "dft_generic.hip", "resample3d_any.hip", "resample2d.hip", "channel_mix.hip", "channel_wgrad.hip", "adam.hip", "pointwise_fused.hip", "instnorm.hip", "lift_bwd.hip", "rel_l2_steps.hip", "rollout.hip", "rollout_train.hip"]
+HEADERS = ["uno_common.h", "channel_mix_common.h", "dft2d_fwd_common.h", "dft2d_fwd_kernel.h", "dft2d_fwd_ft_kernel.h", "dft2d_fwd_ht_kernel.h", "dft2d_fwd_fd_kernel.h", "dft2d_inv_kernel.h", "dft2d_inv_add_kernel.h", os.path.join("..", "..", "include", "uno_spectral.h")]
 ARCH = "gfx950"
 FLAGS = ["-O3", "-std=c++17", "-fPIC", f"--offload-arch={ARCH}", "-fno-gpu-rdc", "-Wall", "-Wno-unused-function"]
 EXTRA_FLAGS = {"mode_gemm.hip": ["-mllvm", "-amdgpu-mfma-vgpr-form"], "dft2d_inv_add.hip": ["-mllvm", "-amdgpu-mfma-vgpr-form"]}
diff --git a/uno_amd/csrc/capi_spectral.hip b/uno_amd/csrc/capi_spectral.hip
--- a/uno_amd/csrc/capi_spectral.hip
+++ b/uno_amd/csrc/capi_spectral.hip
@@ -202,6 +202,48 @@
     { static const int dev_exp = getenv("UNO_K3A_STAGGER") ? atoi(getenv("UNO_K3A_STAGGER")) : 0; p.exp = dev_exp; }
 #endif
     return launch_dft2d_inv_add(p, (hipStream_t)stream);
+}
+
+static void fwd_resample_shape(Dft2dParams& p, int n_img, int H, int W, int m1, int m2, int Ho, int Wo, int KW) {
+    p.n_img = n_img; p.H = H; p.W = W; p.m1 = m1; p.m2 = m2;
+    p.fd_Ho = Ho; p.fd_Wo = Wo; p.fd_KW = KW;
+}
+
+int uno_dft2d_forward_resample_applies(int n_img, int H, int W, int m1, int m2, int Ho, int Wo, int KW) {
+    if (n_img < 1 || H < 1 || W < 1 || m1 < 1 || m2 < 1 || Ho < 1 || Wo < 1 || KW < 1 || m1 > H || m2 > W / 2 + 1 || m1 > 40 || m2 > 48) return 0;
+    Dft2dParams p;
+    fwd_resample_shape(p, n_img, H, W, m1, m2, Ho, Wo, KW);
+    return dft2d_fwd_fd_applies(p) ? 1 : 0;
+}
+
+int uno_dft2d_forward_resample(const float* images, float* spec, int n_img, int H, int W, int m1, int m2, float scale, int hermitian_cols,
+                               int mask_overlap, int group, int stride, int offset, float* resampled, int Ho, int Wo, const int* col_start,
+                               const float* col_wt, int KW, const int* row_tiles, const float* row_op, void* stream) {
+    const char* who = "uno_dft2d_forward_resample";
+    if (n_img < 0) { set_error("%s: negative image count", who); return -1; }
+    if (n_img > 0 && (!images || !spec || !resampled || !col_start || !col_wt || !row_tiles || !row_op)) { set_error("%s: null pointer", who); return -1; }
+    if (int rc = check_modes2d(who, H, W, H, W, m1, m2)) return rc;
+    if (Ho < 1 || Wo < 1 || KW < 1) { set_error("%s: bad output grid %dx%d or band (%d taps)", who, Ho, Wo, KW); return -1; }
+    if (n_img == 0) return 0;
+    if (group <= 0) { group = n_img; stride = 0; offset = 0; }
+    else if (offset < 0 || stride < offset + group || n_img % group) {
+        set_error("%s: bad spectrum grouping (group %d, stride %d, offset %d, images %d)", who, group, stride, offset, n_img);
+        return -1;
+    }
+    if (!uno_dft2d_forward_resample_applies(n_img, H, W, m1, m2, Ho, Wo, KW)) {
+        set_error("%s: the fused form does not apply to %d images of %dx%d -> %dx%d, modes (%d, %d), %d taps (query uno_dft2d_forward_resample_applies)",
+                  who, n_img, H, W, Ho, Wo, m1, m2, KW);
+        return -3;
+    }
+    Dft2dParams p;
+    fwd_resample_shape(p, n_img, H, W, m1, m2, Ho, Wo, KW);
+    p.in = images; p.out = spec; p.scale = scale; p.herm = hermitian_cols ? 1 : 0; p.mask = mask_overlap ? 1 : 0;
+    p.sp_group = group; p.sp_stride = stride; p.sp_offset = offset;
+    p.twH = twiddle_table(H);
+    p.twW = twiddle_table(W);
+    if (!p.twH || !p.twW) return -6;
+    p.fd_out = resampled; p.fd_startW = col_start; p.fd_wtW = col_wt; p.fd_tiles = row_tiles; p.fd_rowop = row_op;
+    return launch_dft2d_fwd_fd(p, (hipStream_t)stream);
 }
 
 int uno_dft2d_forward_bf16(const void* images, float* spec, int n_img, int H, int W, int m1, int m2, float scale,
diff --git a/uno_amd/csrc/dft2d_fwd_fd.hip b/uno_amd/csrc/dft2d_fwd_fd.hip
--- /dev/null
+++ b/uno_amd/csrc/dft2d_fwd_fd.hip
@@ -0,0 +1,28 @@
+#include "dft2d_fwd_fd_kernel.h"
+
+namespace uno {
+
+static bool fd_class(const Dft2dParams& p, int* NT, int* MT, int* R4) {
+    if (p.m1 < 1 || p.m2 < 1 || p.m1 > 40 || p.m2 > 48) return false;
+    *NT = (p.m2 + 15) / 16; *MT = (2 * p.m1 + 15) / 16;
+    const int rem = p.m2 - 16 * (*NT - 1);
+    if (rem > 8) return false;
+    *R4 = (rem + 3) / 4;
+    return (*NT == 2 && *MT == 3 && *R4 == 1) || (*NT == 1 && *MT == 1 && (*R4 == 1 || *R4 == 2));
+}
+
+bool dft2d_fwd_fd_applies(const Dft2dParams& p) {
+    int NT, MT, R4;
+    FwdFtGeometry g;
+    return fd_class(p, &NT, &MT, &R4) && fwd_fd_geometry(p, NT, MT, R4, &g);
+}
+
+int launch_dft2d_fwd_fd(const Dft2dParams& p, hipStream_t s) {
+    int NT, MT, R4;
+    FwdFtGeometry g;
+    if (!fd_class(p, &NT, &MT, &R4) || !fwd_fd_geometry(p, NT, MT, R4, &g)) { set_error("dft2d_fwd_fd: the form does not apply"); return -3; }
+    if (NT == 2) return launch_fwd_fd<2, 3, 1>(p, g, s);
+    return R4 == 1 ? launch_fwd_fd<1, 1, 1>(p, g, s) : launch_fwd_fd<1, 1, 2>(p, g, s);
+}
+
+}
diff --git a/uno_amd/csrc/dft2d_fwd_fd_kernel.h b/uno_amd/csrc/dft2d_fwd_fd_kernel.h
--- /dev/null
+++ b/uno_amd/csrc/dft2d_fwd_fd_kernel.h
@@ -0,0 +1,319 @@
+#pragma once
+#include "dft2d_fwd_common.h"
+#include "dft2d_fwd_ft_kernel.h"
+
+namespace uno {
+
+constexpr int FD_NC = 13;
+constexpr int FD_KT = 10;
+constexpr int FD_CE = 4;
+constexpr int FD_WR = (FD_NC * 16 + 63) / 64;
+#ifndef UNO_FD_KO
+#define UNO_FD_KO 0
+#endif
+constexpr int FD_MINW = 416, FD_MAXW = 447;
+
+template <int NT, int MT, int R4>
+__global__ __launch_bounds__(256) void dft2d_fwd_fd_kernel(Dft2dParams p) {
+    constexpr int NTF = R4 > 0 ? NT - 1 : NT;
+    constexpr int NQ = R4 > 0 ? R4 : 1;
+    constexpr int NTFA = NTF > 0 ? NTF : 1;
+    extern __shared__ __attribute__((aligned(16))) char smem[];
+    const int H = p.H, W = p.W, m1 = p.m1, m2 = p.m2;
+    const int Ho = p.fd_Ho, Wo = p.fd_Wo;
+    const int tid = threadIdx.x;
+    const int nthreads = blockDim.x;
+    const int NWT = nthreads >> 6;
+    const int wave = __builtin_amdgcn_readfirstlane(tid >> 6);
+    const int lane = tid & 63;
+    const int r16 = lane & 15;
+    const int kk = lane >> 4;
+    const unsigned H8 = 8u * H;
+    UNO_FWD_COLUMN_PAIRS(W);
+    const int nk = 4 * nfull + tailsteps;
+
+    const int tile_stride = (16 * W + 32 + 3) & ~3;
+    float* sTile = reinterpret_cast<float*>(smem);
+    float2* sTabF = reinterpret_cast<float2*>(sTile + (size_t)NWT * tile_stride);
+    const int nka = UNO_FWD_TABLE_STEPS(nfull);
+    float2* sTab4 = sTabF + (size_t)nka * NTF * 64;
+    float2* sTwH = sTab4 + (size_t)nka * R4 * 16;
+    int* sTailW = reinterpret_cast<int*>(sTwH + H);
+
+    const int image = sweep_x(p.rev) * NWT + wave;
+    const bool active = image < p.n_img;
+    const int nrt = (H + 15) >> 4;
+    float* buf = sTile + (size_t)wave * tile_stride;
+
+    int a0;
+    const __amdgpu_buffer_rsrc_t rsrc = image_rsrc(p.in, p.n_img, H, W, active ? image : 0, &a0);
+    auto request_tile = [&](int rt) {
+        const int toff = a0 + rt * 16 * W;
+        const int rows = min(16, H - 16 * rt);
+        const int total = (toff & 31) + rows * W;
+        const int npiece = (total + 255) >> 8;
+        const unsigned v0 = (unsigned)(((toff & ~31) + 4 * lane) * 4);
+        for (int i = 0; i < npiece; ++i)
+            if (256 * i + 4 * lane < total)
+                __builtin_amdgcn_raw_ptr_buffer_load_lds(rsrc, (lds_ptr_t)(buf + 256 * i), 16, v0 + 1024u * (unsigned)i, 0, 0, FT_AUX);
+    };
+    if (active) request_tile(0);
+
+    for (int n = tid; n < H; n += nthreads) sTwH[n] = p.twH[n];
+    for (int e = tid; e < FWD_TAILMAX * 64; e += nthreads) { UNO_FWD_PUT_TAIL_COLUMNS(e); }
+    UNO_FWD_BUILD_OPERAND_TABLES();
+
+    int sc[FD_CE];
+    float wc[FD_CE][FD_KT];
+    {
+        const int KW = p.fd_KW;
+#pragma unroll
+        for (int e = 0; e < FD_CE; ++e) {
+            const int j = min(64 * e + lane, Wo - 1);
+            const int s = p.fd_startW[j];
+            sc[e] = max(min(s - (lane >> 5), W - FD_KT), 0);
+            const int d = s - sc[e];
+#pragma unroll
+            for (int t = 0; t < FD_KT; ++t) {
+                const int u = t - d;
+                const bool in = u >= 0 && u < KW && s + u < W;
+                const float wv = p.fd_wtW[(size_t)j * KW + min(max(u, 0), KW - 1)];
+                wc[e][t] = in ? wv : 0.f;
+            }
+        }
+    }
+    __syncthreads();
+
+    UNO_FWD_ACCUMULATORS(false, MT);
+
+    const float2* tabF = sTabF + lane;
+    const float2* tab4 = sTab4 + 4 * kk + (lane & 3);
+
+    float C[FD_NC][FD_CE];
+#pragma unroll
+    for (int c = 0; c < FD_NC; ++c)
+#pragma unroll
+        for (int e = 0; e < FD_CE; ++e) C[c][e] = 0.f;
+
+    if (active) {
+        float* const oimg = p.fd_out + (size_t)image * Ho * Wo;
+        int pend_ibase = 0, pend_ncomp = 0;
+        auto flush_rows = [&]() {
+#pragma unroll
+            for (int c = 0; c < FD_NC; ++c) {
+                if (c < pend_ncomp && (unsigned)(pend_ibase + c) < (unsigned)Ho && !(UNO_FD_KO & 4)) {
+                    float* orow = oimg + (size_t)(pend_ibase + c) * Wo;
+#pragma unroll
+                    for (int e = 0; e < FD_CE; ++e)
+                        if (64 * e + lane < Wo) orow[64 * e + lane] = C[c][e];
+                }
+            }
+#pragma unroll
+            for (int n = 1; n < 16; n *= 2) {
+                if (pend_ncomp & n) {
+#pragma unroll
+                    for (int c = 0; c < FD_NC; ++c)
+#pragma unroll
+                        for (int e = 0; e < FD_CE; ++e) C[c][e] = (c + n < FD_NC) ? C[(c + n < FD_NC) ? c + n : 0][e] : 0.f;
+                }
+            }
+        };
+        for (int rt = 0; rt < nrt; ++rt) {
+            const int toff = a0 + rt * 16 * W;
+            const int phase = toff & 31;
+            const int rows = min(16, H - 16 * rt);
+            const float* row = buf + phase + r16 * W;
+            asm volatile("s_waitcnt vmcnt(0)" ::: "memory");
+            flush_rows();
+            if (rows < 16) {
+                for (int i = phase + rows * W + lane; i < phase + 16 * W; i += 64) buf[i] = 0.f;
+            }
+            const float* wd = p.fd_rowop + (size_t)rt * (FD_NC * 16);
+            float wv[FD_WR];
+#pragma unroll
+            for (int k = 0; k < FD_WR; ++k) wv[k] = wd[min(64 * k + lane, FD_NC * 16 - 1)];
+            int tinfo = p.fd_tiles[4 * rt + (lane & 3)];
+
+            f32x4 Tr[NT], Tn[NT];
+            f32x4 Qr[NQ], Qn[NQ];
+#pragma unroll
+            for (int t = 0; t < NT; ++t) { Tr[t] = f32x4{0, 0, 0, 0}; Tn[t] = f32x4{0, 0, 0, 0}; }
+#pragma unroll
+            for (int g = 0; g < NQ; ++g) { Qr[g] = f32x4{0, 0, 0, 0}; Qn[g] = f32x4{0, 0, 0, 0}; }
+#define UNO_FD_MFMA(E_, D_, TWF_, TW4_)                                                   \
+    do {                                                                                  \
+        _Pragma("unroll") for (int t = 0; t < NTF; ++t) {                                 \
+            Tr[t] = mfma16((E_), (TWF_)[t].x, Tr[t]);                                     \
+            Tn[t] = mfma16((D_), (TWF_)[t].y, Tn[t]);                                     \
+        }                                                                                 \
+        _Pragma("unroll") for (int g = 0; g < R4; ++g) {                                  \
+            Qr[g] = mfma4((E_), (TW4_)[g].x, Qr[g]);                                   \
+            Qn[g] = mfma4((D_), (TW4_)[g].y, Qn[g]);                                   \
+        }                                                                                 \
+    } while (0)
+
+            struct RowOps { float xl[4], xr[4]; float2 twF[4][NTFA], tw4[4][NQ]; };
+            RowOps opA, opB;
+            const float* pl = row + 1 + 4 * kk;
+            const float* pr = row + W - 4 - 4 * kk;
+            auto load_ops = [&](RowOps& o, int c) {
+                const int cn = min(c, max(nfull - 1, 0));
+                const float2* tf = tabF + (size_t)(4 * c) * (NTF * 64);
+                const float2* t4 = tab4 + (size_t)(4 * c) * (R4 * 16);
+#pragma unroll
+                for (int s = 0; s < 4; ++s) {
+                    o.xl[s] = pl[16 * cn + s]; o.xr[s] = pr[-16 * cn + s];
+#pragma unroll
+                    for (int t = 0; t < NTF; ++t) o.twF[s][t] = tf[(s * NTF + t) * 64];
+#pragma unroll
+                    for (int g = 0; g < R4; ++g) o.tw4[s][g] = t4[(s * R4 + g) * 16];
+                }
+            };
+            auto chunk = [&](RowOps& cur, RowOps& nxt, int c) {
+                load_ops(nxt, c + 1);
+                __builtin_amdgcn_sched_barrier(0);
+#pragma unroll
+                for (int s = 0; s < 4; ++s) {
+                    const float E = cur.xl[s] + cur.xr[3 - s];
+                    const float D = cur.xl[s] - cur.xr[3 - s];
+                    UNO_FD_MFMA(E, D, cur.twF[s], cur.tw4[s]);
+                }
+                __builtin_amdgcn_sched_barrier(0);
+            };
+            load_ops(opA, 0);
+            {
+                int c = 0;
+                for (; c + 2 <= nfull; c += 2) { chunk(opA, opB, c); chunk(opB, opA, c + 1); }
+                if (c < nfull) { chunk(opA, opB, c); opA = opB; }
+            }
+            float2 (&twF)[4][NTFA] = opA.twF;
+            float2 (&tw4)[4][NQ] = opA.tw4;
+            {
+                const float2* tf = tabF + (size_t)(4 * nfull) * (NTF * 64);
+                const float2* t4 = tab4 + (size_t)(4 * nfull) * (R4 * 16);
+                float TL[FWD_TAILMAX], TR[FWD_TAILMAX];
+#pragma unroll
+                for (int s = 0; s < FWD_TAILMAX; ++s) {
+                    const int wl = sTailW[(s * 2 + 0) * 64 + lane], wr = sTailW[(s * 2 + 1) * 64 + lane];
+                    const float vl = row[max(wl, 0)], vr = row[max(wr, 0)];
+                    TL[s] = wl >= 0 ? vl : 0.f; TR[s] = wr >= 0 ? vr : 0.f;
+                }
+                float2 twF5[NTFA], tw45[NQ];
+#pragma unroll
+                for (int t = 0; t < NTF; ++t) twF5[t] = tf[(4 * NTF + t) * 64];
+#pragma unroll
+                for (int g = 0; g < R4; ++g) tw45[g] = t4[(4 * R4 + g) * 16];
+#pragma unroll
+                for (int s = 0; s < FWD_TAILMAX; ++s) {
+                    if (s < tailsteps) {
+                        const float E = TL[s] + TR[s];
+                        const float D = TL[s] - TR[s];
+                        if (s < 4) UNO_FD_MFMA(E, D, twF[s], tw4[s]);
+                        else UNO_FD_MFMA(E, D, twF5, tw45);
+                    }
+                }
+            }
+#undef UNO_FD_MFMA
+
+            float Y[16][FD_CE];
+            {
+                const float* trow = buf + phase;
+                float xv[2][FD_CE][FD_KT];
+                auto read_row = [&](float (&x)[FD_CE][FD_KT], int r) {
+#pragma unroll
+                    for (int e = 0; e < FD_CE; ++e) {
+                        const float* q = trow + r * W + sc[e];
+#pragma unroll
+                        for (int t = 0; t < FD_KT; ++t) x[e][t] = q[t];
+                    }
+                };
+                if (!(UNO_FD_KO & 1)) read_row(xv[0], 0);
+#pragma unroll
+                for (int r = 0; r < 16; ++r) {
+                    if (UNO_FD_KO & 1) { for (int e = 0; e < FD_CE; ++e) Y[r][e] = 0.f; continue; }
+                    if (r + 1 < 16) read_row(xv[(r + 1) & 1], r + 1);
+                    __builtin_amdgcn_sched_barrier(0);
+#pragma unroll
+                    for (int e = 0; e < FD_CE; ++e) {
+                        float acc = 0.f;
+#pragma unroll
+                        for (int t = 0; t < FD_KT; ++t) acc = fmaf(wc[e][t], xv[r & 1][e][t], acc);
+                        asm volatile("" : "+v"(acc));
+                        Y[r][e] = acc;
+                    }
+                    __builtin_amdgcn_sched_barrier(0);
+                }
+            }
+#pragma unroll
+            for (int k = 0; k < FD_WR; ++k) asm volatile("" : "+v"(wv[k]));
+            asm volatile("" : "+v"(tinfo));
+            asm volatile("s_waitcnt lgkmcnt(0)" ::: "memory");
+            if (rt + 1 < nrt) request_tile(rt + 1);
+
+            const int ibase = __builtin_amdgcn_readlane(tinfo, 0);
+            const int ncomp = __builtin_amdgcn_readlane(tinfo, 1);
+            const unsigned mlo = (unsigned)__builtin_amdgcn_readlane(tinfo, 2);
+            const unsigned mhi = (unsigned)__builtin_amdgcn_readlane(tinfo, 3);
+#pragma unroll
+            for (int c = 0; c < FD_NC; ++c) {
+#pragma unroll
+                for (int q4 = 0; q4 < 4; ++q4) {
+                    const int b = 4 * c + q4;
+                    const unsigned bit = b < 32 ? (mlo >> (b & 31)) & 1u : (mhi >> ((b - 32) & 31)) & 1u;
+                    if (bit && !(UNO_FD_KO & 2)) {
+#pragma unroll
+                        for (int r = 4 * q4; r < 4 * q4 + 4; ++r) {
+                            const float w = __int_as_float(__builtin_amdgcn_readlane(__float_as_int(wv[(c * 16 + r) >> 6]), (c * 16 + r) & 63));
+#pragma unroll
+                            for (int e = 0; e < FD_CE; ++e) C[c][e] = fmaf(w, Y[r][e], C[c][e]);
+                        }
+                    }
+                }
+            }
+            pend_ibase = ibase;
+            pend_ncomp = ncomp;
+
+            UNO_FWD_REGROUP_4X4();
+            UNO_FWD_STAGE_B(false, MT);
+        }
+        flush_rows();
+    }
+
+    if (active) UNO_FWD_STORE_SPECTRUM(false, MT, image);
+}
+
+static bool fwd_fd_geometry(const Dft2dParams& p, int NT, int MT, int R4, FwdFtGeometry* out) {
+    (void)MT;
+    const int NTF = R4 > 0 ? NT - 1 : NT;
+    if (p.bf16 || p.rowfreq || p.W < FD_MINW || p.W > FD_MAXW) return false;
+    if (p.fd_Ho < 1 || p.fd_Wo < 1 || p.fd_Wo > 64 * FD_CE || p.fd_KW < 1 || p.fd_KW > FD_KT - 1) return false;
+    if ((long long)p.fd_Ho * p.fd_Wo > 0x7fffffffLL / 4) return false;
+    const int cus = ft_device_cu_count();
+    int g = 4;
+    while (g > 1 && (long long)(p.n_img + g - 1) / g < cus) --g;
+    while (g > 1 && fwd_ft_lds_bytes(p, NTF, R4, g) > FT_LDS_BUDGET) --g;
+    const size_t lds = fwd_ft_lds_bytes(p, NTF, R4, g);
+    if (lds > FT_LDS_BUDGET) return false;
+    *out = FwdFtGeometry{1, g, lds};
+    return true;
+}
+
+template <int NT, int MT, int R4>
+static int launch_fwd_fd(Dft2dParams p, const FwdFtGeometry& g, hipStream_t s) {
+    auto K = dft2d_fwd_fd_kernel<NT, MT, R4>;
+    static int lds_slot[64];
+    if (!ensure_dynamic_lds(reinterpret_cast<const void*>(K), g.lds, lds_slot)) { set_error("dft2d_fwd_fd: cannot raise dynamic LDS to %zu", g.lds); return -4; }
+    char name[64];
+    snprintf(name, sizeof(name), "uno::dft2d_fwd_fd_kernel<%d, %d, %d>", NT, MT, R4);
+    p.nw = 1;
+    p.rev = fwd_ft_sweep();
+    {
+        ProfScope prof(name, (double)p.n_img * ((double)p.H * p.W * 4.0 + (double)p.fd_Ho * p.fd_Wo * 4.0 + 2.0 * p.m1 * p.m2 * 8.0), s);
+        hipLaunchKernelGGL(K, dim3((p.n_img + g.g - 1) / g.g), dim3(64 * g.g), g.lds, s, p);
+    }
+    const hipError_t e = hipGetLastError();
+    if (e != hipSuccess) { set_error("dft2d_fwd_fd launch: %s", hipGetErrorString(e)); return -5; }
+    return 0;
+}
+
+}
diff --git a/uno_amd/csrc/dft2d_fwd_ft_kernel.h b/uno_amd/csrc/dft2d_fwd_ft_kernel.h
--- a/uno_amd/csrc/dft2d_fwd_ft_kernel.h
+++ b/uno_amd/csrc/dft2d_fwd_ft_kernel.h
@@ -186,11 +186,13 @@
     return fwd_tile_geometry(p, NTF, R4, FwdTileForm{4, FT_LDS_BUDGET, 3, fwd_ft_lds_bytes}, out);
 }
 
+static int fwd_ft_sweep() { return next_sweep_reversed(SWEEP_K1); }
+
 template <int NT, int MT, int R4>
 static int launch_fwd_ft(const Dft2dParams& p, const FwdFtGeometry& g, hipStream_t s) {
     char name[64];
     snprintf(name, sizeof(name), "uno::dft2d_fwd_ft_kernel<%d, %d, %d>", NT, MT, R4);
-    return launch_fwd_tile<dft2d_fwd_ft_kernel<NT, MT, R4>>(name, p, g, next_sweep_reversed(SWEEP_K1), s);
+    return launch_fwd_tile<dft2d_fwd_ft_kernel<NT, MT, R4>>(name, p, g, fwd_ft_sweep(), s);
 }
 
 }
diff --git a/uno_amd/csrc/uno_common.h b/uno_amd/csrc/uno_common.h
--- a/uno_amd/csrc/uno_common.h
+++ b/uno_amd/csrc/uno_common.h
@@ -159,6 +159,12 @@
     const float* add_rowop = nullptr;
     const int* add_v0 = nullptr;
     const float* add_colop = nullptr;
+    float* fd_out = nullptr;
+    int fd_Ho = 0, fd_Wo = 0, fd_KW = 0;
+    const int* fd_startW = nullptr;
+    const float* fd_wtW = nullptr;
+    const int* fd_tiles = nullptr;
+    const float* fd_rowop = nullptr;
 };
 
 __device__ __forceinline__ size_t spectrum_index(const Dft2dParams& p, int img) {
@@ -234,6 +240,8 @@
 int launch_dft2d_inv(const Dft2dParams& p, hipStream_t s);
 bool dft2d_inv_add_applies(const Dft2dParams& p);
 int launch_dft2d_inv_add(const Dft2dParams& p, hipStream_t s);
+bool dft2d_fwd_fd_applies(const Dft2dParams& p);
+int launch_dft2d_fwd_fd(const Dft2dParams& p, hipStream_t s);
 bool dft2d_fwd_plane_applies(const Dft2dParams& p);
 bool dft2d_inv_plane_applies(const Dft2dParams& p);
 bool dft2d_b16_applies(const Dft2dParams& p);
diff --git a/uno_amd/resample.py b/uno_amd/resample.py
--- a/uno_amd/resample.py
+++ b/uno_amd/resample.py
@@ -136,6 +136,51 @@
     return tuple(_native.table_to_device(t, dev) for t in ops)
 
 
+FD_NC = 13
+FD_KW = 9
+
+
+def _fd_row_tiles(A: torch.Tensor):
+    Ho, H = A.shape
+    nrt = (H + TILE_ROWS - 1) // TILE_ROWS
+    nz = A != 0
+    last = torch.where(nz.any(1), H - 1 - nz.flip(1).float().argmax(1), torch.zeros(Ho, dtype=torch.long))
+    done = torch.cummax(last, 0).values // TILE_ROWS
+    pad = torch.zeros(Ho + FD_NC, TILE_ROWS * nrt, dtype=torch.float32)
+    pad[:Ho, :H] = A
+    tiles = torch.zeros(nrt, 4, dtype=torch.int64)
+    op = torch.zeros(nrt, FD_NC, TILE_ROWS, dtype=torch.float32)
+    for rt in range(nrt):
+        i0 = int((done < rt).sum())
+        cols = slice(TILE_ROWS * rt, TILE_ROWS * (rt + 1))
+        if bool((pad[i0 + FD_NC:, cols] != 0).any()):
+            return None
+        op[rt] = pad[i0:i0 + FD_NC, cols]
+        ncomp = int((done == rt).sum()) if rt < nrt - 1 else Ho - i0
+        if ncomp > FD_NC:
+            return None
+        pieces = (op[rt].view(FD_NC, 4, 4) != 0).any(2).flatten()
+        mask = sum(1 << b for b in range(4 * FD_NC) if bool(pieces[b]))
+        lo, hi = mask & 0xffffffff, mask >> 32
+        tiles[rt] = torch.tensor([i0, ncomp, lo - (1 << 32) if lo >= 1 << 31 else lo, hi])
+    return tiles.to(torch.int32).contiguous(), op.contiguous()
+
+
+@functools.lru_cache(maxsize=None)
+def fused_resample_tables(H: int, W: int, Ho: int, Wo: int, device_str: str, adjoint: bool = False, mode: str = "bicubic_aa"):
+    if adjoint:
+        A, (bw, _) = _matrix(Ho, H, mode).t().contiguous(), _tables(Wo, W, device_str, mode)[1]
+    else:
+        A, (bw, _) = _matrix(H, Ho, mode), _tables(W, Wo, device_str, mode)[0]
+    if bw[1].shape[1] > FD_KW:
+        return None
+    rows = _fd_row_tiles(A)
+    if rows is None:
+        return None
+    dev = torch.device(device_str)
+    return (bw[0], bw[1], *(_native.table_to_device(t, dev) for t in rows))
+
+
 def resample_forward(x: torch.Tensor, Ho: int, Wo: int, out: torch.Tensor | None = None) -> torch.Tensor:
     H, W = x.shape[-2:]
     (fh, th), _ = _tables(H, Ho, str(x.device))
```

Measured after the change: 1523 samples/s (median of 6 runs). 1.8% higher.
